# danielzgtg/TTS.cpp

Hardware: AMD Instinct MI355X
Metric: audio-sec/wall-sec (RTF^-1), Parler-TTS-mini v1 Q4_K AR decode + DAC decode (higher is better)
Workload: dtype q4_K weights x q8_K activations (int dot, f32 combine); DAC f16 im2col x f32 weights, f64 accumulate

## Files before the change

include/tts_hip.h:

```cpp
#ifndef TTS_HIP_H
#define TTS_HIP_H

#include <stddef.h>
#include <stdint.h>

#ifdef __cplusplus
extern "C" {
#endif

#define TTS_MAX_DIMS 4
#define TTS_MAX_SRC 4
#define TTS_MAX_OP_PARAMS 16
#define TTS_MAX_NAME 64

enum tts_type {
    TTS_TYPE_F32 = 0,
    TTS_TYPE_F16 = 1,
    TTS_TYPE_Q4_0 = 2,
    TTS_TYPE_Q4_1 = 3,
    TTS_TYPE_Q5_0 = 6,
    TTS_TYPE_Q5_1 = 7,
    TTS_TYPE_Q8_0 = 8,
    TTS_TYPE_Q8_1 = 9,
    TTS_TYPE_Q4_K = 12,
// ... 49 lines not shown
    TTS_OP_COUNT
};

enum tts_custom_op {
    TTS_CUSTOM_NONE = 0,
    TTS_CUSTOM_UV_NOISE = 1,
    TTS_CUSTOM_CFG_SCALE = 2
};

enum tts_unary_op {
    TTS_UNARY_ABS = 0,
    TTS_UNARY_NEG,
    TTS_UNARY_TANH,
    TTS_UNARY_RELU,
    TTS_UNARY_SIGMOID,
    TTS_UNARY_GELU,
    TTS_UNARY_SILU,
    TTS_UNARY_EXP,
    TTS_UNARY_COUNT
};

enum tts_status {
    TTS_STATUS_SUCCESS = 0,
    TTS_STATUS_FAILED = -1,
    TTS_STATUS_ALLOC_FAILED = -2,
    TTS_STATUS_UNSUPPORTED = -3,
    TTS_STATUS_BAD_ARG = -4,
    TTS_STATUS_NO_DEVICE = -5
};

#define TTS_PROF_ATTN 39

#define TTS_FLAG_INPUT 1
#define TTS_FLAG_HOSTDATA 2
#define TTS_FLAG_OUTPUT 4
#define TTS_FLAG_PERSIST 8
#define TTS_FLAG_REPACKED 16
#define TTS_FLAG_TILED_COPY 64
#define TTS_FLAG_TILED 32

typedef struct tts_tensor {
    int32_t type;
    int32_t op;
    int64_t ne[TTS_MAX_DIMS];
    size_t nb[TTS_MAX_DIMS];
    int32_t op_params[TTS_MAX_OP_PARAMS];
    struct tts_tensor * src[TTS_MAX_SRC];
    struct tts_tensor * view_src;
    size_t view_offs;
    void * data;
    int32_t flags;
    int32_t pad_;
    char name[TTS_MAX_NAME];
} tts_tensor;

size_t tts_type_size(int type);
int64_t tts_blck_size(int type);
size_t tts_row_size(int type, int64_t ne0);
const char * tts_type_name(int type);
const char * tts_op_name(int op);

typedef struct tts_hip_backend * tts_hip_backend_t;

int tts_hip_device_count(void);
int tts_hip_device_memory(int device, size_t * free_bytes, size_t * total_bytes);
void * tts_hip_event_new(int device);
void tts_hip_event_free(void * event);
int tts_hip_event_record(tts_hip_backend_t backend, void * event);
int tts_hip_event_wait(tts_hip_backend_t backend, void * event);
int tts_hip_event_synchronize(void * event);
int tts_hip_is_device_pointer(const void * p);
tts_hip_backend_t tts_hip_backend_init(int device);
void tts_hip_backend_free(tts_hip_backend_t backend);
const char * tts_hip_backend_name(tts_hip_backend_t backend);

void * tts_hip_buffer_alloc(tts_hip_backend_t backend, size_t size);
void tts_hip_buffer_free(tts_hip_backend_t backend, void * ptr);
size_t tts_hip_buffer_alignment(void);

int tts_hip_tensor_set(tts_hip_backend_t backend, void * dst_dev, const void * src_host, size_t size);
int tts_hip_tensor_get(tts_hip_backend_t backend, void * dst_host, const void * src_dev, size_t size);
int tts_hip_tensor_copy(tts_hip_backend_t backend, void * dst_dev, const void * src_dev, size_t size);
int tts_hip_copy_stream(tts_hip_backend_t backend, void * dst_dev, const void * src_dev, size_t size);
int tts_hip_plan_stats(tts_tensor * const * nodes, int n_nodes, int mask, int32_t * counts);
int tts_hip_tensor_set_async(tts_hip_backend_t backend, void * dst_dev, const void * src_host, size_t size);
int tts_hip_memset(tts_hip_backend_t backend, void * dst_dev, int value, size_t size);
int tts_hip_synchronize(tts_hip_backend_t backend);

int tts_hip_weight_set(tts_hip_backend_t backend, tts_tensor * t, const void * src_host);
int tts_hip_weight_get(tts_hip_backend_t backend, const tts_tensor * t, void * dst_host);
int tts_hip_quantize(tts_hip_backend_t backend, int type, const float * x_dev, void * dst_dev, int64_t rows, int64_t K);
void tts_repack_q4_K(const void * src, void * dst, int64_t nblocks, int inverse);
void tts_repack_q4_K_tiled(const void * src, void * dst, int64_t nrows, int64_t nb, int inverse);

int tts_hip_supports_op(const tts_tensor * node);
int tts_hip_graph_compute(tts_hip_backend_t backend, tts_tensor * const * nodes, int n_nodes);
int tts_hip_graph_prepare(tts_hip_backend_t backend, tts_tensor * const * nodes, int n_nodes, int slot);
int tts_hip_graph_launch(tts_hip_backend_t backend, int slot);

enum tts_hip_option {
    TTS_HIP_OPT_FUSION = 0,
    TTS_HIP_OPT_PROFILE_GEMV = 1,
    TTS_HIP_OPT_GRAPHS = 2,
    TTS_HIP_OPT_CONV_F32ACC = 3,
    TTS_HIP_OPT_CONVT_LDS = 4,
    TTS_HIP_OPT_ATTN_SPLIT = 5,
    TTS_HIP_OPT_KV_PREFETCH = 6,
    TTS_HIP_OPT_KV_PREFETCH_BLOCKS = 7,
    TTS_HIP_OPT_Q4K_TILE_BYTES = 8,
    TTS_HIP_OPT_GEMV_DEBUG = 10,
    TTS_HIP_OPT_CONV_SPLIT = 12,
    TTS_HIP_OPT_GEMV_UNIQUE = 11,
    TTS_HIP_OPT_GEMV_KS = 13,
    TTS_HIP_OPT_ATTN_FUSED = 14,
    TTS_HIP_OPT_GEMM_Q8 = 18,
    TTS_HIP_OPT_BGEMM_F32 = 19,
    TTS_HIP_OPT_CU_PARTITION = 20,
    TTS_HIP_OPT_Q4K_DUAL_BYTES = 16,
    TTS_HIP_OPT_GEMV_RSPLIT = 17,
    TTS_HIP_OPT_ATTN_PV16 = 15,
    TTS_HIP_OPT_GEMV_PREQUANT = 21,
    TTS_HIP_OPT_GEMV_KRELAY = 22,
    TTS_HIP_OPT_ATTN_KS = 23,
    TTS_HIP_OPT_ATTN_PV8 = 24,
    TTS_HIP_OPT_GEMV_KRELAY_LOOP = 26,
    TTS_HIP_OPT_GEMV_Q80_PRO = 27,
    TTS_HIP_OPT_GEMV_Q80_SLAB = 28,
    TTS_HIP_OPT_GEMV_Q80_RW = 29,
    TTS_HIP_OPT_GEMM_Q8_STAGED = 30,
    TTS_HIP_OPT_GEMV_KR_INKERNEL = 31,
    TTS_HIP_OPT_GEMV_F32_WIDE = 32,
    TTS_HIP_OPT_ATTN_PV_MP = 33,
    TTS_HIP_OPT_GEMM_KR_INKERNEL = 35,
    TTS_HIP_OPT_GEMM_KR_CT2 = 36,
    TTS_HIP_OPT_GEMM_KR_NW = 34,
    TTS_HIP_OPT_GEMV_NW_MIN = 25,
    TTS_HIP_OPT_GEMM_KR_XCD = 38,
    TTS_HIP_OPT_GEMM_KR_CP = 39,
    TTS_HIP_OPT_GEMM_KR_WALK = 40,
    TTS_HIP_OPT_GEMM_PF = 41,
    TTS_HIP_OPT_GEMM_PF_NW = 42,
    TTS_HIP_OPT_ATTN_ONE = 43,
    TTS_HIP_OPT_GEMV_KR_TAIL = 44,
    TTS_HIP_OPT_GEMV_Q50_SLAB = 45,
    TTS_HIP_OPT_GEMV_Q50_RW = 46,
    TTS_HIP_OPT_GEMM_Q5 = 47,
    TTS_HIP_OPT_GEMM_Q5_STAGED = 48,
    TTS_HIP_OPT_GEMV_Q40_SLAB = 49,
    TTS_HIP_OPT_GEMV_Q40_RW = 50,
    TTS_HIP_OPT_GEMM_Q4_0 = 51,
    TTS_HIP_OPT_GEMM_Q4_0_STAGED = 52,
    TTS_HIP_OPT_CONV_VFMA = 53,
    TTS_HIP_OPT_CONV_TILE96 = 54,
    TTS_HIP_OPT_COALESCE = 37,
};
enum tts_fuse_bits {
    TTS_FUSE_LN = 1, TTS_FUSE_GROUP = 2, TTS_FUSE_KV = 4, TTS_FUSE_EPI = 8, TTS_FUSE_HEADS = 16, TTS_FUSE_ATTN = 32,
    TTS_FUSE_LSTM = 64,
    TTS_FUSE_SNAKE = 128,
    TTS_FUSE_EMBED = 256,
    TTS_FUSE_CONV = 512,
    TTS_FUSE_ADAIN = 1024,
    TTS_FUSE_XATTN = 2048,
    TTS_FUSE_MCPY = 4096,
    TTS_FUSE_CONTREAD = 8192
};
int tts_hip_set_option(tts_hip_backend_t backend, int option, int value);
int tts_hip_attn_decode(tts_hip_backend_t backend, const tts_tensor * q, const tts_tensor * k, const tts_tensor * v,
                        const float * mask, int64_t mbs, float scale, float * out, float * out2, const int64_t * koff,
                        const int64_t * voff, const int64_t * moff, const int32_t * pseq);
int tts_hip_coalesce_stats(int device, int64_t * out, int n);
void tts_hip_coalesce_set_wait(int us);
int tts_hip_coalesce_enable(int on);
#define TTS_HIP_HOOK_FAULT_WEIGHT_SET 1
int tts_hip_test_hook(int hook, int value);
int tts_hip_install_crash_handler(void);
int tts_hip_gemv_stats(tts_hip_backend_t backend, int type, double * ms, int64_t * launches, double * bytes, int reset);
int tts_hip_greedy_step(tts_hip_backend_t backend, const float * logits, int32_t B, int32_t NH, int32_t V, int32_t step,
                        int32_t bos, int32_t eos, int32_t * eos_seen, int32_t * hist, int32_t * next);
typedef struct tts_sampling {
    float temperature;
    float top_p;
    float repetition_penalty;
    int32_t top_k;
    int32_t do_sample;
    int32_t pad_;
    uint64_t seed;
} tts_sampling;
void tts_sampling_default(tts_sampling * cfg);
uint32_t tts_sampler_call_seed(uint64_t seed, int32_t stream, int64_t call);
int tts_sampler_sample(const tts_sampling * cfg, const float * logits, int32_t NH, int32_t V, uint32_t call_seed, int32_t * last,
                       int32_t * count, int32_t * out);
int tts_hip_sample_step(tts_hip_backend_t backend, const float * logits, int32_t B, int32_t NH, int32_t V, const tts_sampling * cfg,
                        int64_t call, int32_t * rep_state, int32_t step, int32_t bos, int32_t eos, int32_t * eos_seen, int32_t * hist,
                        int32_t * next);
int tts_sampling_device_ok(const tts_sampling * cfg, int32_t V);
int tts_hip_counters(tts_hip_backend_t backend, int64_t * out, int n);

int tts_hip_gemv(tts_hip_backend_t backend, int type, const void * w, const float * x, float * y,
                 int64_t K, int64_t N, int64_t M);
int tts_hip_gemv_ex(tts_hip_backend_t backend, int type, const void * w, const float * x, float * y,
                    int64_t K, int64_t N, int64_t M, int32_t wflags);
int tts_hip_gemv_res(tts_hip_backend_t backend, int type, const void * w, const float * x, float * y, const float * res,
                     int64_t K, int64_t N, int64_t M, int32_t wflags);

typedef struct tts_backend_iface {
    void * ctx;
    const char * name;
    void * (*alloc)(void * ctx, size_t size);
    void (*free)(void * ctx, void * ptr);
    int (*set)(void * ctx, void * dst, const void * src, size_t size);
    int (*set_tensor)(void * ctx, tts_tensor * t, const void * src);
    int (*get)(void * ctx, void * dst, const void * src, size_t size);
    int (*memset)(void * ctx, void * dst, int value, size_t size);
    int (*compute)(void * ctx, tts_tensor * const * nodes, int n_nodes);
    int (*synchronize)(void * ctx);
    int (*prepare)(void * ctx, tts_tensor * const * nodes, int n_nodes, int slot);
    int (*launch)(void * ctx, int slot);
    int (*set_async)(void * ctx, void * dst, const void * src, size_t size);
    int (*copy)(void * ctx, void * dst, const void * src, size_t size);
    int (*greedy_step)(void * ctx, const float * logits, int B, int NH, int V, int step, int bos, int eos, int32_t * eos_seen,
                       int32_t * hist, int32_t * next);
    int (*sample_step)(void * ctx, const float * logits, int B, int NH, int V, const tts_sampling * cfg, int64_t call, int32_t * rep_state,
                       int step, int bos, int eos, int32_t * eos_seen, int32_t * hist, int32_t * next);
} tts_backend_iface;

int tts_hip_backend_iface(tts_hip_backend_t backend, tts_backend_iface * out);

#ifdef __cplusplus
}
#endif

#endif
```

tts.cpp_amd/csrc/backend.hip:

```cpp
#include <cmath>
#include <atomic>
#include <cstring>
#include <map>
#include <mutex>
#include <thread>

#include "hip_internal.h"
#include <hip/hip_ext.h>

#include <dlfcn.h>
#include <execinfo.h>
#include <fcntl.h>
#include <signal.h>
#include <unistd.h>

using namespace tts;


static void build_gelu_table(uint16_t * t) {
    const float GELU_COEF_A = 0.044715f;
    const float SQRT_2_OVER_PI = 0.79788456080286535587989211986876f;
    for (int i = 0; i < 65536; ++i) {
        const float x = fp16_to_fp32_host((uint16_t)i);
        const float g = 0.5f * x * (1.0f + tanhf(SQRT_2_OVER_PI * x * (1.0f + GELU_COEF_A * x * x)));
        t[i] = fp32_to_fp16_host(g);
    }
}

static const size_t kScratchBytes = 64u << 20;
static const size_t kShadowBytes = 4u << 20;
static const size_t kLstmFloats = 4u << 20;
static const size_t kAttnFloats = 4u << 20;
static const size_t kVecScratchFloats = 1u << 18;
static const size_t kPinBytes = 16u << 20;

namespace {
std::mutex g_reg_mu;
struct BufRec {
    size_t size = 0;
};
std::map<const char *, BufRec> g_buffers;
std::unordered_map<const void *, uint8_t *> g_tiled;
std::atomic<size_t> g_tiled_n{0};
}

namespace tts {
const uint8_t * tiled_copy_find(const void * w) {
    std::lock_guard<std::mutex> lk(g_reg_mu);
    auto it = g_tiled.find(w);
    return it == g_tiled.end() ? nullptr : it->second;
}
static std::atomic<int> g_coalesce_on{[] {
    const char * e = getenv("TTS_HIP_COALESCE");
    return e && e[0] == '0' ? 0 : 1;
}()};
bool coalesce_enabled() { return g_coalesce_on.load(std::memory_order_relaxed) != 0; }
bool buffer_lookup(const void * p, const char ** base, size_t * size) {
    std::lock_guard<std::mutex> lk(g_reg_mu);
    auto it = g_buffers.upper_bound((const char *)p);
    if (it == g_buffers.begin()) return false;
    --it;
    if ((const char *)p >= it->first + it->second.size) return false;
    if (base) *base = it->first;
    if (size) *size = it->second.size;
    return true;
}
}

extern "C" {

int tts_hip_coalesce_enable(int on) { return tts::g_coalesce_on.exchange(on ? 1 : 0); }

int tts_hip_device_count(void) {
    int n = 0;
    if (hipGetDeviceCount(&n) != hipSuccess) return 0;
    return n;
}

tts_hip_backend_t tts_hip_backend_init(int device) {
    int n = tts_hip_device_count();
    if (device < 0 || device >= n) return nullptr;
    if (hipSetDevice(device) != hipSuccess) return nullptr;
    auto * be = new tts_hip_backend();
    be->device = device;
    TTS_HIP_CHECK(hipStreamCreateWithFlags(&be->stream, hipStreamNonBlocking));
    TTS_HIP_CHECK(hipStreamCreateWithFlags(&be->cap_stream, hipStreamNonBlocking));
    TTS_HIP_CHECK(hipStreamCreateWithFlags(&be->pf_stream, hipStreamNonBlocking));
    TTS_HIP_CHECK(hipEventCreateWithFlags(&be->co_ev, hipEventDisableTiming));
    TTS_HIP_CHECK(hipEventCreateWithFlags(&be->pf_fork, hipEventDisableTiming));
    TTS_HIP_CHECK(hipEventCreateWithFlags(&be->pf_join, hipEventDisableTiming));
    hipDeviceProp_t prop;
    TTS_HIP_CHECK(hipGetDeviceProperties(&prop, device));
    snprintf(be->name, sizeof(be->name), "HIP%d(%s)", device, prop.gcnArchName);
    be->cu_total = prop.multiProcessorCount > 0 ? prop.multiProcessorCount : 256;
    be->cus = be->cu_total;
    TTS_HIP_CHECK(hipMalloc((void **)&be->scratch, kScratchBytes));
    be->scratch_size = kScratchBytes;
    TTS_HIP_CHECK(hipMalloc((void **)&be->shadow, kShadowBytes));
    be->shadow_size = kShadowBytes;
    be->hoist_size = (size_t)8 << 20;
    TTS_HIP_CHECK(hipMalloc(&be->hoist, be->hoist_size));
    TTS_HIP_CHECK(hipMalloc((void **)&be->lstm_buf, kLstmFloats * sizeof(float)));
    TTS_HIP_CHECK(hipMalloc((void **)&be->attn_buf, kAttnFloats * sizeof(float)));
    be->attn_floats = kAttnFloats;
    TTS_HIP_CHECK(hipMalloc((void **)&be->vec_scratch, kVecScratchFloats * sizeof(float)));
    be->conv_stage_floats = (size_t)8 << 20;
    TTS_HIP_CHECK(hipMalloc((void **)&be->conv_stage, be->conv_stage_floats * sizeof(float)));
    if (const char * e = getenv("TTS_HIP_OPT_CONV_VFMA"))
        if (e[0] >= '0' && e[0] <= '2' && !e[1]) be->conv_vfma = e[0] - '0';
    be->conv_part_doubles = (size_t)8 << 20;
    TTS_HIP_CHECK(hipMalloc((void **)&be->conv_part, be->conv_part_doubles * sizeof(double)));
    be->lstm_floats = kLstmFloats;
    TTS_HIP_CHECK(hipMalloc((void **)&be->argmax_keys, kArgmaxRows * sizeof(unsigned long long)));
    TTS_HIP_CHECK(hipMalloc((void **)&be->argmax_counts, kArgmaxRows * sizeof(unsigned)));
    TTS_HIP_CHECK(hipMemset(be->argmax_keys, 0, kArgmaxRows * sizeof(unsigned long long)));
    TTS_HIP_CHECK(hipMemset(be->argmax_counts, 0, kArgmaxRows * sizeof(unsigned)));
    TTS_HIP_CHECK(hipHostMalloc((void **)&be->pin, kPinBytes, hipHostMallocDefault));
    be->pin_size = kPinBytes;
    for (auto & e : be->plan_ev) TTS_HIP_CHECK(hipEventCreateWithFlags(&e, hipEventDisableTiming));
    std::vector<uint16_t> tab(65536);
    build_gelu_table(tab.data());
    TTS_HIP_CHECK(hipMalloc((void **)&be->gelu_table, 65536 * sizeof(uint16_t)));
    TTS_HIP_CHECK(hipMemcpy(be->gelu_table, tab.data(), 65536 * sizeof(uint16_t), hipMemcpyHostToDevice));
    return be;
}

void tts_hip_backend_free(tts_hip_backend_t be) {
    if (!be) return;
    tts::coalesce_backend_gone(be);
    hipSetDevice(be->device);
    hipStreamSynchronize(be->stream);
    for (auto & p : be->ev_pending) {
        hipEventDestroy(p.first);
        hipEventDestroy(p.second);
    }
    for (auto e : be->ev_free) hipEventDestroy(e);
    for (auto & r : be->pin_pending) hipEventDestroy(r.ev);
    for (auto e : be->pin_events) hipEventDestroy(e);
    for (auto e : be->plan_ev) hipEventDestroy(e);
    hipHostFree(be->pin);
    if (be->rb_host) hipHostFree(be->rb_host);
    hipFree(be->scratch);
    hipFree(be->shadow);
    hipFree(be->argmax_keys);
    hipFree(be->argmax_counts);
    hipFree(be->lstm_buf);
    hipFree(be->hoist);
    hipFree(be->attn_buf);
    hipFree(be->vec_scratch);
    hipFree(be->conv_stage);
    hipFree(be->conv_part);
    hipFree(be->gelu_table);
    if (be->sample_cand) hipFree(be->sample_cand);
    if (be->repack_tmp) hipFree(be->repack_tmp);
    for (char * r : be->repack_retired) hipFree(r);
    if (be->attn_stage) hipFree(be->attn_stage);
    for (auto & ex : be->gsig_exec)
        if (ex) hipGraphExecDestroy(ex);
    for (auto & ex : be->pexec)
        if (ex) hipGraphExecDestroy(ex);
    hipStreamDestroy(be->stream);
    hipStreamDestroy(be->cap_stream);
    hipStreamDestroy(be->pf_stream);
    hipEventDestroy(be->pf_fork);
    hipEventDestroy(be->pf_join);
    hipEventDestroy(be->co_ev);
    delete be;
}

const char * tts_hip_backend_name(tts_hip_backend_t be) { return be ? be->name : "HIP(null)"; }

int tts_hip_device_memory(int device, size_t * free_bytes, size_t * total_bytes) {
    if (device < 0 || device >= tts_hip_device_count()) return TTS_STATUS_NO_DEVICE;
    int prev = 0;
    hipGetDevice(&prev);
    hipSetDevice(device);
    size_t f = 0, t = 0;
    const hipError_t e = hipMemGetInfo(&f, &t);
    hipSetDevice(prev);
    if (e != hipSuccess) return TTS_STATUS_FAILED;
    if (free_bytes) *free_bytes = f;
    if (total_bytes) *total_bytes = t;
    return 0;
}

void * tts_hip_event_new(int device) {
    if (device < 0 || device >= tts_hip_device_count()) return nullptr;
    hipSetDevice(device);
    hipEvent_t ev = nullptr;
    if (hipEventCreateWithFlags(&ev, hipEventDisableTiming) != hipSuccess) return nullptr;
    return (void *)ev;
}
void tts_hip_event_free(void * event) {
    if (event) hipEventDestroy((hipEvent_t)event);
}
int tts_hip_event_record(tts_hip_backend_t be, void * event) {
    if (!be || !event) return TTS_STATUS_BAD_ARG;
    hipSetDevice(be->device);
    return hipEventRecord((hipEvent_t)event, be->stream) == hipSuccess ? 0 : TTS_STATUS_FAILED;
}
int tts_hip_event_wait(tts_hip_backend_t be, void * event) {
    if (!be || !event) return TTS_STATUS_BAD_ARG;
    hipSetDevice(be->device);
    return hipStreamWaitEvent(be->stream, (hipEvent_t)event, 0) == hipSuccess ? 0 : TTS_STATUS_FAILED;
}
int tts_hip_event_synchronize(void * event) {
    if (!event) return TTS_STATUS_BAD_ARG;
    return hipEventSynchronize((hipEvent_t)event) == hipSuccess ? 0 : TTS_STATUS_FAILED;
}
int tts_hip_is_device_pointer(const void * p) {
    if (!p) return 0;
    hipPointerAttribute_t a;
    if (hipPointerGetAttributes(&a, p) != hipSuccess) {
        (void)hipGetLastError();
        return 0;
    }
    return a.type == hipMemoryTypeDevice ? 1 : 0;
}

size_t tts_hip_buffer_alignment(void) { return 256; }

void * tts_hip_buffer_alloc(tts_hip_backend_t be, size_t size) {
    if (!be) return nullptr;
    hipSetDevice(be->device);
    void * p = nullptr;
    BufRec r;
    r.size = size ? size : 256;
    if (hipMalloc(&p, r.size) != hipSuccess) return nullptr;
    std::lock_guard<std::mutex> lk(g_reg_mu);
    g_buffers[(const char *)p] = r;
    return p;
}

static void drop_tiled_copies(const void * p, size_t n) {
    if (g_tiled_n.load(std::memory_order_acquire) == 0) return;
    const char * a = (const char *)p;
    std::vector<uint8_t *> dead;
    {
        std::lock_guard<std::mutex> lk(g_reg_mu);
        for (auto it = g_tiled.begin(); it != g_tiled.end();) {
            const char * k = (const char *)it->first;
            if (k >= a && k < a + n) {
                dead.push_back(it->second);
                it = g_tiled.erase(it);
            } else {
                ++it;
            }
        }
        g_tiled_n.store(g_tiled.size(), std::memory_order_release);
    }
    if (dead.empty()) return;
    hipDeviceSynchronize();
    for (uint8_t * c : dead) hipFree(c);
}

void tts_hip_buffer_free(tts_hip_backend_t be, void * ptr) {
    if (!be || !ptr) return;
    hipSetDevice(be->device);
    hipStreamSynchronize(be->stream);
    BufRec r;
    bool known = false;
    {
        std::lock_guard<std::mutex> lk(g_reg_mu);
        auto b = g_buffers.find((const char *)ptr);
        if (b != g_buffers.end()) {
            r = b->second;
            known = true;
            g_buffers.erase(b);
        }
    }
    if (known) {
        drop_tiled_copies(ptr, r.size);
        tts::coalesce_written(ptr, r.size);
    }
    hipFree(ptr);
}

int tts_hip_tensor_set(tts_hip_backend_t be, void * dst, const void * src, size_t size) {
    if (!be) return TTS_STATUS_BAD_ARG;
    hipSetDevice(be->device);
    be->rb_clear();
    drop_tiled_copies(dst, size);
    tts::coalesce_written(dst, size);
    if (size > 0 && size <= be->pin_size / 4) {
        const int st = tts_hip_tensor_set_async(be, dst, src, size);
        if (st != 0) return st;
    } else if (hipMemcpyAsync(dst, src, size, hipMemcpyHostToDevice, be->stream) != hipSuccess) {
        return TTS_STATUS_FAILED;
    }
    if (hipStreamSynchronize(be->stream) != hipSuccess) return TTS_STATUS_FAILED;
    return 0;
}

int tts_hip_tensor_set_async(tts_hip_backend_t be, void * dst, const void * src, size_t size) {
    if (!be) return TTS_STATUS_BAD_ARG;
    if (size == 0) return 0;
    hipSetDevice(be->device);
    be->rb_clear();
    if (size > be->pin_size / 2) return tts_hip_tensor_set(be, dst, src, size);
    tts::coalesce_written(dst, size);
    std::lock_guard<std::mutex> pl(be->pin_mu);
    while (!be->pin_pending.empty() && hipEventQuery(be->pin_pending.front().ev) == hipSuccess) {
        be->pin_events.push_back(be->pin_pending.front().ev);
        be->pin_pending.pop_front();
    }
    size_t off = (be->pin_head + 255) & ~(size_t)255;
    if (off + size > be->pin_size) off = 0;
    int last = -1;
    for (int i = 0; i < (int)be->pin_pending.size(); ++i) {
        const auto & r = be->pin_pending[i];
        if (r.off < off + size && off < r.off + r.size) last = i;
    }
    if (last >= 0) {
        if (hipEventSynchronize(be->pin_pending[last].ev) != hipSuccess) return TTS_STATUS_FAILED;
        for (int i = 0; i <= last; ++i) {
            be->pin_events.push_back(be->pin_pending.front().ev);
            be->pin_pending.pop_front();
        }
    }
    memcpy(be->pin + off, src, size);
    if (hipMemcpyAsync(dst, be->pin + off, size, hipMemcpyHostToDevice, be->stream) != hipSuccess) return TTS_STATUS_FAILED;
    hipEvent_t ev;
    if (be->pin_events.empty()) {
        if (hipEventCreateWithFlags(&ev, hipEventDisableTiming) != hipSuccess) return TTS_STATUS_FAILED;
    } else {
        ev = be->pin_events.back();
        be->pin_events.pop_back();
    }
    if (hipEventRecord(ev, be->stream) != hipSuccess) return TTS_STATUS_FAILED;
    be->pin_pending.push_back({off, size, ev});
    be->pin_head = off + size;
    return 0;
}

int tts_hip_greedy_step(tts_hip_backend_t be, const float * logits, int32_t B, int32_t NH, int32_t V, int32_t step, int32_t bos,
                        int32_t eos, int32_t * eos_seen, int32_t * hist, int32_t * next) {
    if (!be || !logits || B <= 0 || NH <= 0 || V <= 0) return TTS_STATUS_BAD_ARG;
    hipSetDevice(be->device);
    be->rb_clear();
    launch_greedy_step(be, logits, B, NH, V, step, bos, eos, eos_seen, hist, next);
    return 0;
}

int tts_hip_sample_step(tts_hip_backend_t be, const float * logits, int32_t B, int32_t NH, int32_t V, const tts_sampling * cfg, int64_t call,
                        int32_t * rep_state, int32_t step, int32_t bos, int32_t eos, int32_t * eos_seen, int32_t * hist, int32_t * next) {
    if (!be || !logits || !cfg || B <= 0 || NH <= 0 || V <= 0) return TTS_STATUS_BAD_ARG;
    hipSetDevice(be->device);
    be->rb_clear();
    return launch_sample_step(be, logits, B, NH, V, cfg, call, rep_state, step, bos, eos, eos_seen, hist, next);
}

int tts_hip_tensor_get(tts_hip_backend_t be, void * dst, const void * src, size_t size) {
    if (!be) return TTS_STATUS_BAD_ARG;
    hipSetDevice(be->device);
    if (be->rb_any.load(std::memory_order_acquire)) {
        std::lock_guard<std::mutex> l(be->rb_mu);
        for (const auto & r : be->rb) {
            const char * s = (const char *)src;
            if (s >= r.dev && s + size <= r.dev + r.bytes) {
                if (hipStreamSynchronize(be->stream) != hipSuccess) return TTS_STATUS_FAILED;
                memcpy(dst, be->rb_host + r.off + (s - r.dev), size);
                return 0;
            }
        }
    }
    if (hipMemcpyAsync(dst, src, size, hipMemcpyDeviceToHost, be->stream) != hipSuccess) return TTS_STATUS_FAILED;
    if (hipStreamSynchronize(be->stream) != hipSuccess) return TTS_STATUS_FAILED;
    return 0;
}

int tts_hip_copy_stream(tts_hip_backend_t be, void * dst, const void * src, size_t size) {
    if (!be || !dst || !src || size % 16 || ((uintptr_t)dst | (uintptr_t)src) % 16) return TTS_STATUS_BAD_ARG;
    if (size == 0) return 0;
    hipSetDevice(be->device);
    be->rb_clear();
    tts::launch_copy_stream(be, dst, src, (int64_t)(size / 16));
    return hipGetLastError() == hipSuccess ? 0 : TTS_STATUS_FAILED;
}

int tts_hip_tensor_copy(tts_hip_backend_t be, void * dst, const void * src, size_t size) {
    if (!be) return TTS_STATUS_BAD_ARG;
    hipSetDevice(be->device);
    be->rb_clear();
    tts::coalesce_written(dst, size);
    tts::launch_copy_bytes(be, dst, src, size);
    return hipGetLastError() == hipSuccess ? 0 : TTS_STATUS_FAILED;
}

int tts_hip_memset(tts_hip_backend_t be, void * dst, int value, size_t size) {
    if (!be) return TTS_STATUS_BAD_ARG;
    hipSetDevice(be->device);
    be->rb_clear();
    tts::coalesce_written(dst, size);
    return hipMemsetAsync(dst, value, size, be->stream) == hipSuccess ? 0 : TTS_STATUS_FAILED;
}

int tts_hip_synchronize(tts_hip_backend_t be) {
    if (!be) return TTS_STATUS_BAD_ARG;
    hipSetDevice(be->device);
    return hipStreamSynchronize(be->stream) == hipSuccess ? 0 : TTS_STATUS_FAILED;
}

void tts_repack_q4_K(const void * src, void * dst, int64_t nblocks, int inverse) {
    const uint8_t * s = (const uint8_t *)src;
    uint8_t * d = (uint8_t *)dst;
    for (int64_t b = 0; b < nblocks; ++b) {
        const uint8_t * sb = s + b * 144;
        uint8_t * db = d + b * 144;
        memcpy(db, sb, 16);
        for (int i = 0; i < 128; ++i) {
            const int l = i >> 4, c = (i >> 2) & 3, k = i & 3;
            const int nat = 32 * c + 8 * k + l;
            if (!inverse) db[16 + i] = sb[16 + nat];
            else db[16 + nat] = sb[16 + i];
        }
    }
}

static void repack_tiled_rows(const uint8_t * s, uint8_t * d, int64_t r0, int64_t r1, int64_t nb, int inverse) {
    const int64_t rb = nb * 144;
    for (int64_t row = r0; row < r1; ++row) {
        const int64_t t = row >> 2, i = row & 3;
        for (int64_t b = 0; b < nb; ++b) {
            const int64_t nat = row * rb + b * 144;
            const int64_t til = (t * nb + b) * 576;
            const uint8_t * a = inverse ? s + til : s + nat;
            uint8_t * o = inverse ? d + nat : d + til;
            if (!inverse) memcpy(o + i * 16, a, 16);
            else memcpy(o, a + i * 16, 16);
            for (int c = 0; c < 4; ++c)
                for (int h = 0; h < 2; ++h)
                    for (int lp = 0; lp < 4; ++lp)
                        for (int kk = 0; kk < 4; ++kk) {
                            const int64_t tpos = 64 + ((c * 2 + h) * 4 + i) * 16 + lp * 4 + kk;
                            const int64_t npos = 16 + 32 * c + 8 * kk + 4 * h + lp;
                            if (!inverse) o[tpos] = a[npos];
                            else o[npos] = a[tpos];
                        }
        }
    }
}

void tts_repack_q4_K_tiled(const void * src, void * dst, int64_t nrows, int64_t nb, int inverse) {
    const uint8_t * s = (const uint8_t *)src;
    uint8_t * d = (uint8_t *)dst;
    unsigned nt = std::thread::hardware_concurrency();
    nt = nt < 1 ? 1 : nt > 16 ? 16 : nt;
    if (nrows * nb < 4096 || nt == 1) {
        repack_tiled_rows(s, d, 0, nrows, nb, inverse);
        return;
    }
    std::vector<std::thread> th;
    const int64_t chunk = ((nrows + nt - 1) / nt + 3) & ~(int64_t)3;
    for (int64_t r0 = 0; r0 < nrows; r0 += chunk)
        th.emplace_back(repack_tiled_rows, s, d, r0, r0 + chunk < nrows ? r0 + chunk : nrows, nb, inverse);
    for (auto & t : th) t.join();
}

static size_t tensor_bytes(const tts_tensor * t) {
    size_t n = tts_row_size(t->type, t->ne[0]);
    for (int i = 1; i < 4; ++i) n *= (size_t)t->ne[i];
    return n;
}

static int weight_set_impl(tts_hip_backend_t be, tts_tensor * t, const void * src);
static std::atomic<bool> g_fault_weight_set{false};

static struct sigaction g_prev_segv, g_prev_bus;
static void crash_write(const char * s, int n) {
    while (n > 0) {
        const ssize_t w = write(2, s, (size_t)n);
        if (w <= 0) return;
        s += w, n -= (int)w;
    }
}
static char g_crash_maps[1 << 20];
static int crash_hex(char * o, unsigned long v) {
    char t[16];
    int n = 0;
    do t[n++] = "0123456789abcdef"[v & 15], v >>= 4; while (v);
    o[0] = '0', o[1] = 'x';
    for (int i = 0; i < n; ++i) o[2 + i] = t[n - 1 - i];
    return n + 2;
}
static int crash_dec(char * o, int v) {
    char t[12];
    int n = 0;
    do t[n++] = (char)('0' + v % 10), v /= 10; while (v);
    for (int i = 0; i < n; ++i) o[i] = t[n - 1 - i];
    return n;
}
static const char * crash_parse_hex(const char * p, unsigned long * v) {
    unsigned long x = 0;
    for (;; ++p) {
        const char c = *p;
        const int d = c >= '0' && c <= '9' ? c - '0' : c >= 'a' && c <= 'f' ? c - 'a' + 10 : -1;
        if (d < 0) break;
        x = x * 16 + (unsigned long)d;
    }
    *v = x;
    return p;
}
static bool crash_map_line(const char * l, const char * e, unsigned long * a, unsigned long * b, unsigned long * off, const char ** path, int * plen) {
    const char * p = crash_parse_hex(l, a);
    if (*p != '-') return false;
    p = crash_parse_hex(p + 1, b);
    while (p < e && *p == ' ') ++p;
    while (p < e && *p != ' ') ++p;
    while (p < e && *p == ' ') ++p;
    p = crash_parse_hex(p, off);
    for (int f = 0; f < 2; ++f) {
        while (p < e && *p == ' ') ++p;
        while (p < e && *p != ' ') ++p;
    }
    while (p < e && *p == ' ') ++p;
    *path = p, *plen = (int)(e - p);
    return true;
}
static void crash_handler(int sig, siginfo_t * si, void * uc) {
    char buf[640];
    int n = 0;
    const char h1[] = "tts_hip: signal ";
    for (const char * c = h1; *c; ++c) buf[n++] = *c;
    n += crash_dec(buf + n, sig);
    const char h2[] = ", fault address ";
    for (const char * c = h2; *c; ++c) buf[n++] = *c;
    const uintptr_t fa = si ? (uintptr_t)si->si_addr : 0;
    n += crash_hex(buf + n, fa);
    buf[n++] = '\n';
    crash_write(buf, n);
    int mlen = 0;
    {
        const int fd = open("/proc/self/maps", O_RDONLY);
        if (fd >= 0) {
            ssize_t r;
            while (mlen < (int)sizeof g_crash_maps - 1 && (r = read(fd, g_crash_maps + mlen, sizeof g_crash_maps - 1 - mlen)) > 0) mlen += (int)r;
            close(fd);
        }
    }
    void * fr[64];
    const int nf = backtrace(fr, 64);
    for (int i = 0; i < nf; ++i) {
        n = 0;
        buf[n++] = ' ', buf[n++] = ' ', buf[n++] = '#';
        n += crash_dec(buf + n, i);
        buf[n++] = ' ';
        n += crash_hex(buf + n, (unsigned long)(uintptr_t)fr[i]);
// ... 28 lines not shown
        if (crash_map_line(g_crash_maps + l0, g_crash_maps + l1, &a, &b, &off, &path, &plen) && fa + (64ul << 20) >= a && fa <= b + (64ul << 20))
            crash_write(g_crash_maps + l0, l1 - l0 + (l1 < mlen ? 1 : 0));
        l0 = l1 + 1;
    }
    const struct sigaction & prev = sig == SIGBUS ? g_prev_bus : g_prev_segv;
    if (prev.sa_flags & SA_SIGINFO) {
        if (prev.sa_sigaction) prev.sa_sigaction(sig, si, uc);
    } else if (prev.sa_handler != SIG_DFL && prev.sa_handler != SIG_IGN && prev.sa_handler) {
        prev.sa_handler(sig);
    }
    signal(sig, SIG_DFL);
    raise(sig);
}

int tts_hip_install_crash_handler(void) {
    void * warm[2];
    (void)backtrace(warm, 2);
    struct sigaction sa;
    memset(&sa, 0, sizeof sa);
    sa.sa_sigaction = crash_handler;
    sa.sa_flags = SA_SIGINFO | SA_RESETHAND;
    sigemptyset(&sa.sa_mask);
    if (sigaction(SIGSEGV, &sa, &g_prev_segv) != 0 || sigaction(SIGBUS, &sa, &g_prev_bus) != 0) return TTS_STATUS_FAILED;
    return 0;
}

int tts_hip_test_hook(int hook, int value) {
    if (hook == TTS_HIP_HOOK_FAULT_WEIGHT_SET) {
        g_fault_weight_set.store(value != 0);
        return 0;
    }
    return TTS_STATUS_BAD_ARG;
}

int tts_hip_weight_set(tts_hip_backend_t be, tts_tensor * t, const void * src) {
    if (!be || !t) return TTS_STATUS_BAD_ARG;
    if (t->type == TTS_TYPE_Q4_K && g_fault_weight_set.load(std::memory_order_relaxed)) return TTS_STATUS_ALLOC_FAILED;
    return weight_set_impl(be, t, src);
}

static int weight_set_impl(tts_hip_backend_t be, tts_tensor * t, const void * src) {
    const size_t n = tensor_bytes(t);
    if (t->type == TTS_TYPE_Q4_K && t->ne[0] % 256 == 0 && t->ne[1] % 4 == 0 && t->ne[2] == 1 && t->ne[3] == 1 &&
        be->q4k_tile_bytes > 0 && (int64_t)n >= be->q4k_tile_bytes) {
        std::vector<uint8_t> tmp(n);
        tts_repack_q4_K_tiled(src, tmp.data(), t->ne[1], t->ne[0] / 256, 0);
        int st = tts_hip_tensor_set(be, t->data, tmp.data(), n);
        if (st == 0) t->flags |= TTS_FLAG_REPACKED | TTS_FLAG_TILED;
        return st;
    }
    if (t->type == TTS_TYPE_Q4_K && t->ne[0] % 256 == 0) {
        std::vector<uint8_t> tmp(n);
        tts_repack_q4_K(src, tmp.data(), (int64_t)(n / 144), 0);
        t->flags &= ~TTS_FLAG_TILED_COPY;
        int st = tts_hip_tensor_set(be, t->data, tmp.data(), n);
        if (st == 0) t->flags |= TTS_FLAG_REPACKED;
        if (st == 0 && be->q4k_dual_bytes > 0 && (int64_t)n >= be->q4k_dual_bytes && t->ne[0] >= 2048 && t->ne[1] % 16 == 0 &&
            t->ne[2] == 1 && t->ne[3] == 1) {
            tts_repack_q4_K_tiled(src, tmp.data(), t->ne[1], t->ne[0] / 256, 0);
            uint8_t * cp = nullptr;
            if (hipMalloc((void **)&cp, n) != hipSuccess) return TTS_STATUS_ALLOC_FAILED;
            if (hipMemcpy(cp, tmp.data(), n, hipMemcpyHostToDevice) != hipSuccess) {
                hipFree(cp);
                return TTS_STATUS_FAILED;
            }
            {
                std::lock_guard<std::mutex> lk(g_reg_mu);
                g_tiled[t->data] = cp;
                g_tiled_n.store(g_tiled.size(), std::memory_order_release);
            }
            t->flags |= TTS_FLAG_TILED_COPY;
        }
        return st;
    }
    return tts_hip_tensor_set(be, t->data, src, n);
}

int tts_hip_weight_get(tts_hip_backend_t be, const tts_tensor * t, void * dst) {
    if (!be || !t) return TTS_STATUS_BAD_ARG;
    const size_t n = tensor_bytes(t);
    if (t->type == TTS_TYPE_Q4_K && (t->flags & TTS_FLAG_TILED)) {
        std::vector<uint8_t> tmp(n);
        int st = tts_hip_tensor_get(be, tmp.data(), t->data, n);
        if (st == 0) tts_repack_q4_K_tiled(tmp.data(), dst, t->ne[1], t->ne[0] / 256, 1);
        return st;
    }
    if (t->type == TTS_TYPE_Q4_K && (t->flags & TTS_FLAG_REPACKED)) {
        std::vector<uint8_t> tmp(n);
        int st = tts_hip_tensor_get(be, tmp.data(), t->data, n);
        if (st == 0) tts_repack_q4_K(tmp.data(), dst, (int64_t)(n / 144), 1);
        return st;
    }
    return tts_hip_tensor_get(be, dst, t->data, n);
}

static bool is_f32(const tts_tensor * t) { return t && t->type == TTS_TYPE_F32; }

int tts_hip_supports_op(const tts_tensor * n) {
    if (!n) return 0;
    for (int i = 0; i < TTS_MAX_SRC; ++i)
        if (n->src[i] && (n->src[i]->flags & 2)) return 0;
    switch (n->op) {
        case TTS_OP_NONE: case TTS_OP_VIEW: case TTS_OP_RESHAPE: case TTS_OP_PERMUTE: case TTS_OP_TRANSPOSE:
            return 1;
        case TTS_OP_DUP: case TTS_OP_CONT: case TTS_OP_CPY:
            return (n->type == TTS_TYPE_F32 || n->type == TTS_TYPE_F16 || n->type == TTS_TYPE_I32) &&
                   (n->src[0]->type == TTS_TYPE_F32 || n->src[0]->type == TTS_TYPE_F16 || n->src[0]->type == TTS_TYPE_I32);
        case TTS_OP_ADD: case TTS_OP_SUB: case TTS_OP_MUL: case TTS_OP_DIV:
        case TTS_OP_SQR: case TTS_OP_SQRT: case TTS_OP_SIN: case TTS_OP_COS: case TTS_OP_SCALE: case TTS_OP_CLAMP:
        case TTS_OP_LEAKY_RELU: case TTS_OP_ROUND: case TTS_OP_MOD: case TTS_OP_UNARY: case TTS_OP_CONCAT:
        case TTS_OP_REPEAT: case TTS_OP_SUM_ROWS:
            return 1;
        case TTS_OP_NORM: case TTS_OP_RMS_NORM:
            return is_f32(n->src[0]) && n->src[0]->nb[0] == 4;
        case TTS_OP_SOFT_MAX:
            return is_f32(n->src[0]);
        case TTS_OP_ROPE:
            return is_f32(n->src[0]);
        case TTS_OP_IM2COL:
            return is_f32(n->src[1]) && n->op_params[6] == 0 && (n->type == TTS_TYPE_F16 || n->type == TTS_TYPE_F32);
        case TTS_OP_CONV_TRANSPOSE_1D:
            return is_f32(n->src[0]) && is_f32(n->src[1]) && n->op_params[4] >= 1;
        case TTS_OP_CUMSUM: case TTS_OP_UPSCALE: case TTS_OP_STFT: case TTS_OP_ISTFT: case TTS_OP_MAP_CUSTOM3: case TTS_OP_MAP_CUSTOM2:
            return tts::audio_op_supported(n);
        case TTS_OP_GET_ROWS:
            return n->src[1]->type == TTS_TYPE_I32 &&
                   (n->src[0]->type == TTS_TYPE_F32 || n->src[0]->type == TTS_TYPE_F16 || n->src[0]->type == TTS_TYPE_Q4_K ||
                    n->src[0]->type == TTS_TYPE_Q8_0 || n->src[0]->type == TTS_TYPE_Q5_0 || n->src[0]->type == TTS_TYPE_Q4_0);
        case TTS_OP_MUL_MAT: {
            const tts_tensor * a = n->src[0];
            const tts_tensor * b = n->src[1];
            if (!is_f32(b)) return 0;
            if (a->ne[0] != b->ne[0] || b->ne[2] % a->ne[2] || b->ne[3] % a->ne[3]) return 0;
            if (a->type == TTS_TYPE_F32 || a->type == TTS_TYPE_F16) return 1;
            if (a->type == TTS_TYPE_Q4_K) return a->ne[0] % 256 == 0;
            if (a->type == TTS_TYPE_Q8_0 || a->type == TTS_TYPE_Q5_0 || a->type == TTS_TYPE_Q4_0) return a->ne[0] % 32 == 0;
            return 0;
        }
        default:
            return 0;
    }
}

}

extern "C" int tts_hip_set_option(tts_hip_backend_t be, int option, int value) {
    if (!be) return TTS_STATUS_BAD_ARG;
    switch (option) {
        case TTS_HIP_OPT_FUSION: be->fusion = value; return 0;
        case TTS_HIP_OPT_CONVT_LDS: be->convt_lds = value != 0; return 0;
        case TTS_HIP_OPT_CONV_SPLIT: be->conv_split = value < 0 ? 1 : value; return 0;
        case TTS_HIP_OPT_CONV_VFMA: be->conv_vfma = value < 0 || value > 2 ? 1 : value; return 0;
        case TTS_HIP_OPT_CONV_TILE96: be->conv_tile96 = value != 0; return 0;
        case TTS_HIP_OPT_PROFILE_GEMV: be->profile_gemv = value != 0; return 0;
        case TTS_HIP_OPT_GRAPHS: be->use_graphs = value != 0; return 0;
        case TTS_HIP_OPT_CONV_F32ACC:
            be->conv_f32acc = value == 1;
            be->conv_acc_mode = value == 2 ? 2 : 0;
            return 0;
        case TTS_HIP_OPT_ATTN_SPLIT: be->attn_split_minp = value; return 0;
        case TTS_HIP_OPT_ATTN_FUSED: be->attn_fused_minp = value; return 0;
        case TTS_HIP_OPT_ATTN_PV16: be->attn_pv_uv16 = value != 0; return 0;
        case TTS_HIP_OPT_KV_PREFETCH: be->kv_prefetch_minp = value; return 0;
        case TTS_HIP_OPT_Q4K_TILE_BYTES: be->q4k_tile_bytes = value; return 0;
        case TTS_HIP_OPT_Q4K_DUAL_BYTES: be->q4k_dual_bytes = value; return 0;
        case TTS_HIP_OPT_GEMV_RSPLIT: be->gemv_mf_rsplit = value != 0; return 0;
        case TTS_HIP_OPT_GEMV_PREQUANT: be->gemv_mf_prequant = value != 0; return 0;
        case TTS_HIP_OPT_GEMV_KRELAY: be->gemv_kr = value != 0; return 0;
        case TTS_HIP_OPT_GEMV_KRELAY_LOOP: be->gemv_kr_loop = value != 0; return 0;
        case TTS_HIP_OPT_GEMV_Q80_PRO: be->gemv_q80_pro = value != 0; return 0;
        case TTS_HIP_OPT_GEMV_Q80_SLAB: be->gemv_q80_slab = value != 0; return 0;
        case TTS_HIP_OPT_GEMV_KR_INKERNEL:
            if (value < 0) return TTS_STATUS_BAD_ARG;
            be->gemv_kr_ink = value;
            return 0;
        case TTS_HIP_OPT_GEMM_Q8_STAGED:
            if (value < 0 || value > 2) return TTS_STATUS_BAD_ARG;
            be->gemm_q8_staged = value;
            return 0;
        case TTS_HIP_OPT_GEMV_Q80_RW:
            if (value < 0 || value > 32 || (value & (value - 1))) return TTS_STATUS_BAD_ARG;
            be->gemv_q80_rw = value;
            return 0;
        case TTS_HIP_OPT_GEMV_Q50_SLAB: be->gemv_q50_slab = value != 0; return 0;
        case TTS_HIP_OPT_GEMV_Q50_RW:
            if (value < 0 || value > 32 || (value & (value - 1))) return TTS_STATUS_BAD_ARG;
            be->gemv_q50_rw = value;
            return 0;
        case TTS_HIP_OPT_GEMM_Q5: be->gemm_q5 = value != 0; return 0;
        case TTS_HIP_OPT_GEMM_Q5_STAGED:
            if (value < 0 || value > 2) return TTS_STATUS_BAD_ARG;
            be->gemm_q5_staged = value;
            return 0;
        case TTS_HIP_OPT_GEMV_Q40_SLAB: be->gemv_q40_slab = value != 0; return 0;
        case TTS_HIP_OPT_GEMV_Q40_RW:
            if (value < 0 || value > 32 || (value & (value - 1))) return TTS_STATUS_BAD_ARG;
            be->gemv_q40_rw = value;
            return 0;
        case TTS_HIP_OPT_GEMM_Q4_0: be->gemm_q4_0 = value != 0; return 0;
        case TTS_HIP_OPT_GEMM_Q4_0_STAGED:
            if (value < 0 || value > 2) return TTS_STATUS_BAD_ARG;
            be->gemm_q4_0_staged = value;
            return 0;
        case TTS_HIP_OPT_ATTN_KS: be->attn_ks = value; return 0;
        case TTS_HIP_OPT_GEMV_NW_MIN: be->gemv_nw_min = value; return 0;
        case TTS_HIP_OPT_ATTN_PV8: be->attn_pv8 = value != 0; return 0;
        case TTS_HIP_OPT_GEMM_KR_CT2: be->gemm_kr_ct2 = value != 0; return 0;
        case TTS_HIP_OPT_GEMM_KR_INKERNEL: be->gemm_kr_ink = value < 0 ? 0 : value; return 0;
        case TTS_HIP_OPT_ATTN_PV_MP: be->attn_pv_mp = value == 2 ? 2 : value != 0; return 0;
        case TTS_HIP_OPT_ATTN_ONE:
            if (value < 0 || value > 2) return TTS_STATUS_BAD_ARG;
            be->attn_one = value;
            return 0;
        case TTS_HIP_OPT_GEMV_KR_TAIL:
            if (value < 0 || value > 4) return TTS_STATUS_BAD_ARG;
            be->gemv_kr_tail = value;
            return 0;
        case TTS_HIP_OPT_GEMM_KR_NW: be->gemm_kr_nw = value == 8 ? 8 : 4; return 0;
        case TTS_HIP_OPT_GEMM_Q8: be->gemm_q8 = value != 0; return 0;
        case TTS_HIP_OPT_CU_PARTITION: {
            const int count = value & 0xFF, index = (value >> 8) & 0xFF;
            const bool inter = (value >> 16) & 1;
            hipSetDevice(be->device);
            TTS_HIP_CHECK(hipStreamSynchronize(be->stream));
            hipStream_t ns = nullptr;
            if (count <= 1) {
                TTS_HIP_CHECK(hipStreamCreateWithFlags(&ns, hipStreamNonBlocking));
                be->cus = be->cu_total;
            } else {
                if (index >= count) return TTS_STATUS_BAD_ARG;
                std::vector<uint32_t> mask((be->cu_total + 31) / 32, 0u);
                const int per = be->cu_total / count;
                int n = 0;
                for (int c = 0; c < be->cu_total; ++c) {
                    const bool on = inter ? (c % count == index) : (c / per == index && c < per * count);
                    if (on) mask[c / 32] |= 1u << (c % 32), ++n;
                }
                if (hipExtStreamCreateWithCUMask(&ns, (uint32_t)mask.size(), mask.data()) != hipSuccess) return TTS_STATUS_FAILED;
                be->cus = n;
            }
            TTS_HIP_CHECK(hipStreamDestroy(be->stream));
            be->stream = ns;
            for (auto & ex : be->gsig_exec)
                if (ex) hipGraphExecDestroy(ex), ex = nullptr;
            for (auto & g : be->gsig) g = 0;
            return 0;
        }
        case TTS_HIP_OPT_BGEMM_F32: be->bgemm_f32 = value != 0; return 0;
        case TTS_HIP_OPT_GEMV_F32_WIDE: be->gemv_f32_wide = value != 0; return 0;
        case TTS_HIP_OPT_GEMV_DEBUG: be->gemv_dbg = value; return 0;
        case TTS_HIP_OPT_GEMV_UNIQUE: be->gemv_unique = value != 0; return 0;
        case TTS_HIP_OPT_GEMV_KS: be->gemv_ks_tiles = value > 0 ? value : 0; return 0;
        case TTS_HIP_OPT_COALESCE: be->co_member = value != 0; return 0;
        case TTS_HIP_OPT_GEMM_KR_XCD: be->gemm_kr_xcd = value != 0; return 0;
        case TTS_HIP_OPT_GEMM_KR_CP: be->gemm_kr_cp = value != 0; return 0;
        case TTS_HIP_OPT_GEMM_KR_WALK: be->gemm_kr_walk = value < 0 ? 0 : value; return 0;
        case TTS_HIP_OPT_GEMM_PF: be->gemm_pf = value < 0 ? 0 : value; return 0;
        case TTS_HIP_OPT_GEMM_PF_NW: be->gemm_pf_nw = value == 8 ? 8 : 4; return 0;
        case TTS_HIP_OPT_KV_PREFETCH_BLOCKS: be->kv_prefetch_blocks = value > 0 ? value : 1; return 0;
        default: return TTS_STATUS_BAD_ARG;
    }
}

extern "C" int tts_hip_counters(tts_hip_backend_t be, int64_t * out, int n) {
    if (!be || !out) return TTS_STATUS_BAD_ARG;
    const int64_t v[8] = {be->graph_updates, be->graph_instantiations, be->lstm_chains, be->lstm_steps, be->plan_wait_ns,
                          be->cap_plan_ns, be->cap_launch_ns, be->cap_update_ns};
    int k = 0;
    for (; k < n && k < 8; ++k) out[k] = v[k];
    return k;
}

extern "C" int tts_hip_gemv_stats(tts_hip_backend_t be, int type, double * ms, int64_t * launches, double * bytes, int reset) {
    if (!be) return TTS_STATUS_BAD_ARG;
    hipSetDevice(be->device);
    TTS_HIP_CHECK(hipStreamSynchronize(be->stream));
    for (size_t i = 0; i < be->ev_pending.size(); ++i) {
        float t = 0;
        TTS_HIP_CHECK(hipEventElapsedTime(&t, be->ev_pending[i].first, be->ev_pending[i].second));
        const int ty = be->ev_type[i];
        be->gemv_ms[ty] += t;
        be->gemv_launches[ty] += 1;
        be->gemv_bytes[ty] += be->ev_bytes[i];
        be->ev_free.push_back(be->ev_pending[i].first);
        be->ev_free.push_back(be->ev_pending[i].second);
    }
    be->ev_pending.clear();
    be->ev_bytes.clear();
    be->ev_type.clear();
    double a = 0, c = 0;
    int64_t b = 0;
    for (int ty = 0; ty < TTS_TYPE_COUNT; ++ty) {
        if (type >= 0 && ty != type) continue;
        a += be->gemv_ms[ty];
        b += be->gemv_launches[ty];
        c += be->gemv_bytes[ty];
    }
    if (ms) *ms = a;
    if (launches) *launches = b;
    if (bytes) *bytes = c;
    if (reset) {
        for (int ty = 0; ty < TTS_TYPE_COUNT; ++ty) {
            be->gemv_ms[ty] = 0;
            be->gemv_launches[ty] = 0;
            be->gemv_bytes[ty] = 0;
        }
    }
    return 0;
}

static void * hb_alloc(void * c, size_t n) { return tts_hip_buffer_alloc((tts_hip_backend_t)c, n); }
static void hb_free(void * c, void * p) { tts_hip_buffer_free((tts_hip_backend_t)c, p); }
static int hb_set(void * c, void * d, const void * s, size_t n) { return tts_hip_tensor_set((tts_hip_backend_t)c, d, s, n); }
static int hb_set_tensor(void * c, tts_tensor * t, const void * s) { return tts_hip_weight_set((tts_hip_backend_t)c, t, s); }
static int hb_get(void * c, void * d, const void * s, size_t n) { return tts_hip_tensor_get((tts_hip_backend_t)c, d, s, n); }
static int hb_memset(void * c, void * d, int v, size_t n) { return tts_hip_memset((tts_hip_backend_t)c, d, v, n); }
static int hb_compute(void * c, tts_tensor * const * nodes, int n) { return tts_hip_graph_compute((tts_hip_backend_t)c, nodes, n); }
static int hb_sync(void * c) { return tts_hip_synchronize((tts_hip_backend_t)c); }
static int hb_prepare(void * c, tts_tensor * const * nodes, int n, int slot) {
    return tts_hip_graph_prepare((tts_hip_backend_t)c, nodes, n, slot);
}
static int hb_launch(void * c, int slot) { return tts_hip_graph_launch((tts_hip_backend_t)c, slot); }
static int hb_set_async(void * c, void * d, const void * s, size_t n) { return tts_hip_tensor_set_async((tts_hip_backend_t)c, d, s, n); }
static int hb_copy(void * c, void * d, const void * s, size_t n) { return tts_hip_tensor_copy((tts_hip_backend_t)c, d, s, n); }
static int hb_greedy(void * c, const float * l, int B, int NH, int V, int step, int bos, int eos, int32_t * seen, int32_t * hist, int32_t * next) {
    return tts_hip_greedy_step((tts_hip_backend_t)c, l, B, NH, V, step, bos, eos, seen, hist, next);
}
static int hb_sample(void * c, const float * l, int B, int NH, int V, const tts_sampling * cfg, int64_t call, int32_t * rep, int step, int bos,
                     int eos, int32_t * seen, int32_t * hist, int32_t * next) {
    return tts_hip_sample_step((tts_hip_backend_t)c, l, B, NH, V, cfg, call, rep, step, bos, eos, seen, hist, next);
}

extern "C" int tts_hip_backend_iface(tts_hip_backend_t be, tts_backend_iface * out) {
    if (!be || !out) return TTS_STATUS_BAD_ARG;
    out->ctx = be;
    out->name = be->name;
    out->alloc = hb_alloc;
    out->free = hb_free;
    out->set = hb_set;
    out->set_tensor = hb_set_tensor;
    out->get = hb_get;
    out->memset = hb_memset;
    out->compute = hb_compute;
    out->synchronize = hb_sync;
    out->prepare = hb_prepare;
    out->launch = hb_launch;
    out->set_async = hb_set_async;
    out->copy = hb_copy;
    out->greedy_step = hb_greedy;
    out->sample_step = hb_sample;
    return 0;
}
```

tts.cpp_amd/csrc/graph_exec.hip:

```cpp
#include <algorithm>
#include <cstring>
#include <deque>
#include <unordered_map>
#include <vector>

#include <array>

#include "hip_internal.h"
#include <chrono>

using namespace tts;

namespace tts {
void launch_kv_prefetch(tts_hip_backend * be, hipStream_t st, const TD & t, int pdim, int blocks);
void launch_gemv_q4K_xattn(tts_hip_backend * be, const GemvJob & j, const XAttnArgs & a);
void launch_attn_decode(tts_hip_backend * be, const TD & q, const TD & k, const TD & v, const float * mask, float scale,
                        float * out, int hd, int P, int H, int n, int B, float * out2, int64_t obs = -1, int64_t mbs = 0,
                        const int64_t * koff = nullptr, const int64_t * voff = nullptr, const int64_t * moff = nullptr,
                        const int * pseq = nullptr);
void launch_attn_bias(tts_hip_backend * be, const TD & q, const TD & k, const TD & v, const float * bias, const float * mask,
                      float scale, float * out, int P, int H, int n);
void launch_layernorm(tts_hip_backend * be, const tts_tensor * dst, const tts_tensor * x, const float * w, const float * b,
                      float eps, bool rms);
}
// ... 1156 lines not shown
                m->ne[1] * m->ne[2] * m->ne[3] == 1 && !overlap(A, m) && !(overlap(A, x0) && A->data != x0->data)) {
                it.x = x0;
                it.snake_mask = m;
                act[index[x]] = -1;
            }
        }
        act[index[M1]] = act[index[S]] = act[index[Q]] = act[index[M2]] = -1;
        if (rfuse) {
            it.b = nullptr;
            it.snake_one = O;
            act[index[R]] = -1;
        }
        act[i] = add_item(std::move(it));
    }

    static bool vec_c(const tts_tensor * t, int64_t C) {
        if (!t || t->type != TTS_TYPE_F32 || t->ne[2] * t->ne[3] != 1 || t->nb[0] != 4) return false;
        return (t->ne[0] == C && t->ne[1] == 1) || (t->ne[0] == 1 && t->ne[1] == C && t->nb[1] == 4);
    }
    static bool same_shape(const tts_tensor * a, int64_t n0, int64_t n1) {
        return a->type == TTS_TYPE_F32 && a->ne[0] == n0 && a->ne[1] == n1 && a->ne[2] * a->ne[3] == 1;
    }
    static bool plan_debug() {
        static const bool dbg = getenv("TTS_PLAN_DEBUG") != nullptr;
        return dbg;
    }
    static void plan_reject(const char * what, int code) {
        if (plan_debug()) fprintf(stderr, "plan: %s not fused (check %d)\n", what, code);
    }
    static bool adain_fail(int code) {
        plan_reject("adain", code);
        return false;
    }
    bool try_adain(int i) {
        const tts_tensor * N = nodes[i];
        const tts_tensor * X = N->src[0];
        if (!X || X->type != TTS_TYPE_F32 || N->type != TTS_TYPE_F32 || X->nb[0] != 4 || N->ne[2] * N->ne[3] != 1) return adain_fail(1);
        const int64_t T = N->ne[0], C = N->ne[1];
        if (!adain_supported(T)) return adain_fail(2);
        const tts_tensor * T1 = sole_consumer(N);
        if (!T1 || T1->op != TTS_OP_TRANSPOSE) return adain_fail(3);
        const tts_tensor * C1 = sole_consumer(T1);
        if (!C1 || C1->op != TTS_OP_CONT || !same_shape(C1, C, T) || uses[C1] != 2) return adain_fail(4);
        const auto & cc = consumers[C1];
        if (cc.size() != 2) return adain_fail(5);
        const tts_tensor *M = nodes[cc[0]], *A1 = nodes[cc[1]];
        if (M->op != TTS_OP_MUL || M->src[0] != C1 || !vec_c(M->src[1], C) || sole_consumer(M) != A1) return adain_fail(6);
        if (A1->op != TTS_OP_ADD || A1->src[0] != C1 || A1->src[1] != M || !same_shape(A1, C, T)) return adain_fail(7);
        const tts_tensor * A2 = sole_consumer(A1);
        if (!A2 || A2->op != TTS_OP_ADD || A2->src[0] != A1 || !vec_c(A2->src[1], C) || !same_shape(A2, C, T)) return adain_fail(8);
        const tts_tensor * T2 = sole_consumer(A2);
        if (!T2 || T2->op != TTS_OP_TRANSPOSE) return adain_fail(9);
        const tts_tensor * C2 = sole_consumer(T2);
        if (!C2 || C2->op != TTS_OP_CONT || !same_shape(C2, T, C) || !contiguous(C2)) return adain_fail(10);
        const tts_tensor *gamma = M->src[1], *beta = A2->src[1];
        std::vector<int> absorbed = {i, index[C1], index[M], index[A1], index[A2], index[C2]};
        auto affine_src = [&](const tts_tensor * v, const tts_tensor * user, const tts_tensor *& W, const tts_tensor *& B,
                              const tts_tensor *& st) {
            if (!v || v->op != TTS_OP_ADD || sole_consumer(v) != user) return false;
            const tts_tensor * mm = v->src[0];
            if (!mm || mm->op != TTS_OP_MUL_MAT || sole_consumer(mm) != v || !vec_c(v->src[1], C) || v->src[1]->ne[0] != C) return false;
            W = mm->src[0], st = mm->src[1], B = v->src[1];
            const int64_t S = W->ne[0];
            return W->type == TTS_TYPE_F32 && contiguous(W) && W->ne[1] == C && W->ne[2] * W->ne[3] == 1 && S % 4 == 0 &&
                   ((uintptr_t)W->data % 16) == 0 && st->type == TTS_TYPE_F32 && contiguous(st) && st->ne[0] == S &&
                   st->ne[1] * st->ne[2] * st->ne[3] == 1 && ((uintptr_t)st->data % 16) == 0;
        };
        const tts_tensor *gW = nullptr, *gB = nullptr, *gS = nullptr, *bW = nullptr, *bB = nullptr, *bS = nullptr;
        const bool inline_gb = affine_src(gamma, M, gW, gB, gS) && affine_src(beta, A2, bW, bB, bS) && gS == bS;
        if (inline_gb) {
            for (const tts_tensor * t : {gamma, (const tts_tensor *)gamma->src[0], beta, (const tts_tensor *)beta->src[0]}) absorbed.push_back(index[t]);
            gamma = beta = nullptr;
        }
        const tts_tensor * out = C2;
        const tts_tensor *alpha = nullptr, *recip = nullptr, *one = nullptr;
        if ((mask & TTS_FUSE_SNAKE) && uses[C2] == 2) {
            const auto & sc = consumers[C2];
            const tts_tensor *M1 = nodes[sc[0]], *SA = nodes[sc[1]];
            const tts_tensor *S = sole_consumer(M1), *Q = S ? sole_consumer(S) : nullptr, *M2 = Q ? sole_consumer(Q) : nullptr;
            const tts_tensor * R = M2 ? M2->src[1] : nullptr;
            const tts_tensor * O = R ? R->src[0] : nullptr;
            const bool r_inline = R && R->op == TTS_OP_DIV && O && R->src[1] == M1->src[1] && sole_consumer(R) == M2 &&
                                  O->type == TTS_TYPE_F32 && O->nb[1] == 0 && O->ne[0] == 1 && O->ne[2] * O->ne[3] == 1 &&
                                  same_shape(R, 1, C);
            if (M1->op == TTS_OP_MUL && M1->src[0] == C2 && S && S->op == TTS_OP_SIN && Q && Q->op == TTS_OP_SQR && M2 &&
                M2->op == TTS_OP_MUL && M2->src[0] == Q && sole_consumer(M2) == SA && SA->op == TTS_OP_ADD && SA->src[0] == C2 &&
                SA->src[1] == M2 && vec_c(M1->src[1], C) && vec_c(M2->src[1], C) && same_shape(SA, T, C) && contiguous(SA) &&
                same_shape(M1, T, C) && same_shape(S, T, C) && same_shape(Q, T, C) && same_shape(M2, T, C)) {
                alpha = M1->src[1];
                recip = M2->src[1];
                out = SA;
                for (const tts_tensor * t : {M1, S, Q, M2, SA}) absorbed.push_back(index[t]);
                if (r_inline) {
                    absorbed.push_back(index[R]);
                    recip = nullptr;
                    one = O;
                }
            }
        }
        const bool in_place = out->data == X->data && out->nb[1] == X->nb[1];
        if (overlap(out, X) && !in_place) return adain_fail(11);
        bool stage = false;
        for (const tts_tensor * t : {gamma, beta, alpha, recip, one})
            if (t && overlap(out, t)) stage = true;
        if (inline_gb)
            for (const tts_tensor * t : {gW, gB, bW, bB, gS})
                if (overlap(out, t)) return adain_fail(14);
        if (stage && 4 * C + 1 > (int64_t)vec_cap) return adain_fail(12);
        const int last = *std::max_element(absorbed.begin(), absorbed.end());
        std::vector<bool> is_abs(n, false);
        for (int k : absorbed) is_abs[k] = true;
        for (int k = i + 1; k < last; ++k) {
            if (is_abs[k] || is_view(nodes[k]->op)) continue;
            const tts_tensor * w = nodes[k];
            for (const tts_tensor * t : {X, gamma, beta, alpha, recip, one, gW, gB, bW, bB, gS})
                if (t && t != w && overlap(w, t)) {
                    if (plan_debug()) fprintf(stderr, "plan: adain node %d (%s) between %d..%d overlaps an input\n", k, tts_op_name(w->op), i, last);
                    return adain_fail(13);
                }
        }
        AdainArgs a;
        a.x = (const float *)X->data;
        a.xcs = (int64_t)(X->nb[1] / 4);
        a.y = (float *)out->data;
        a.ycs = (int64_t)(out->nb[1] / 4);
        auto vstride = [](const tts_tensor * t) { return t->ne[0] == 1 ? (int64_t)(t->nb[1] / 4) : (int64_t)1; };
        if (inline_gb) {
            a.gw = (const float *)gW->data, a.gb = (const float *)gB->data;
            a.bw = (const float *)bW->data, a.bb = (const float *)bB->data;
            a.style = (const float *)gS->data, a.S = gW->ne[0];
        } else {
            a.gamma = (const float *)gamma->data, a.gcs = vstride(gamma);
            a.beta = (const float *)beta->data, a.bcs = vstride(beta);
        }
        if (alpha) {
            a.alpha = (const float *)alpha->data, a.acs = vstride(alpha);
            if (recip) a.recip = (const float *)recip->data, a.rcs = vstride(recip);
            else a.one = (const float *)one->data;
        }
        a.T = T, a.C = C;
        a.stage = stage;
        memcpy(&a.eps, &N->op_params[0], 4);
        Item it;
        it.kind = Item::ADAIN;
        it.adain = a;
        it.dst = out;
        for (int k : absorbed)
            if (k != last) act[k] = -1;
        act[last] = add_item(std::move(it));
        return true;
    }

    static const tts_tensor * through_view(const tts_tensor * t) { return t && t->op == TTS_OP_RESHAPE ? t->src[0] : t; }
    void try_conv(int i) {
        const tts_tensor * col = nodes[i];
        const tts_tensor *kern = col->src[0], *x = col->src[1];
        if (col->type != TTS_TYPE_F16 || col->op_params[6] != 0 || col->ne[2] * col->ne[3] != 1) return plan_reject("conv", 1);
        if (!x || x->type != TTS_TYPE_F32 || x->ne[2] * x->ne[3] != 1) return plan_reject("conv", 2);
        if (!kern || (kern->type != TTS_TYPE_F32 && kern->type != TTS_TYPE_F16) || kern->ne[3] != 1) return plan_reject("conv", 3);
        const tts_tensor * cv = sole_consumer(col);
        if (!cv || cv->op != TTS_OP_RESHAPE || !contiguous(col)) return plan_reject("conv", 4);
        const tts_tensor * mm = sole_consumer(cv);
        if (!mm || mm->op != TTS_OP_MUL_MAT || mm->src[0] != cv || mm->type != TTS_TYPE_F32) return plan_reject("conv", 5);
        const tts_tensor * wv = mm->src[1];
        if (!wv || through_view(wv) != kern) return plan_reject("conv", 6);
        const int K = (int)kern->ne[0];
        const int64_t IC = kern->ne[1], OC = kern->ne[2], L = x->ne[0], OL = col->ne[1];
        if (x->ne[1] != IC || mm->ne[0] != OL || mm->ne[1] != OC || !contiguous(mm)) return plan_reject("conv", 7);
        const int s = col->op_params[0], p = col->op_params[2], d = col->op_params[4];
        if (!conv1d_fused_ok(IC, K, s, d, nullptr)) return plan_reject("conv", 8);
        if (kern->nb[0] != tts_type_size(kern->type)) return plan_reject("conv", 9);
        const tts_tensor * out = mm;
        std::vector<int> absorbed = {i, (int)index[mm]};
        const tts_tensor * r3 = sole_consumer(mm);
        const tts_tensor * cur = mm;
        if (r3 && r3->op == TTS_OP_RESHAPE && r3->ne[0] == OL && r3->ne[1] == OC) cur = r3;
        Conv1dArgs a;
        const tts_tensor * bias = nullptr;
        const tts_tensor * res = nullptr;
        const tts_tensor * nb = sole_consumer(cur);
        if (nb && nb->op == TTS_OP_ADD && nb->src[0] == cur && nb->type == TTS_TYPE_F32 && contiguous(nb) && nb->ne[0] == OL &&
            nb->ne[1] == OC && nb->ne[2] * nb->ne[3] == 1 && chan_vec(nb->src[1], OC) && nb->src[1]->ne[1] == OC) {
            bias = nb->src[1];
            out = nb;
            absorbed.push_back(index[nb]);
            const tts_tensor * nr = sole_consumer(nb);
            if (nr && nr->op == TTS_OP_ADD && nr->type == TTS_TYPE_F32 && contiguous(nr) && nr->ne[0] == OL && nr->ne[1] == OC &&
                nr->ne[2] * nr->ne[3] == 1) {
                const tts_tensor * other = nr->src[0] == nb ? nr->src[1] : nr->src[0];
                if (other && other != nb && other->type == TTS_TYPE_F32 && contiguous(other) && other->ne[0] == OL && other->ne[1] == OC &&
                    other->ne[2] * other->ne[3] == 1 && (!overlap(nr, other) || nr->data == other->data)) {
                    res = other;
                    out = nr;
                    absorbed.push_back(index[nr]);
                }
            }
        }
        float * stage = nullptr;
        for (;;) {
            if (overlap(out, kern) || (bias && overlap(out, bias))) return plan_reject("conv", 10);
            stage = nullptr;
            bool ok = true;
            bool in_col = false;
            if (overlap(out, x)) {
                const size_t need = (size_t)OL * (size_t)OC * 4;
                if (tbytes(col) >= need && !overlap(col, x) && !overlap(col, out) && !(res && overlap(col, res)) && !overlap(col, kern) &&
                    !(bias && overlap(col, bias))) {
                    stage = (float *)col->data;
                    in_col = true;
                } else if (conv_stage && need <= 4 * conv_stage_cap) {
                    stage = conv_stage;
                } else {
                    ok = false;
                }
            }
            for (int j = i + 1; ok && j < absorbed.back(); ++j) {
                if (std::find(absorbed.begin(), absorbed.end(), j) != absorbed.end() || is_view(nodes[j]->op)) continue;
                if (overlap(nodes[j], x) || (in_col && overlap(nodes[j], col))) ok = false;
            }
            if (ok) break;
            if (!res) return plan_reject("conv", 11);
            res = nullptr;
            absorbed.pop_back();
            out = bias ? nb : mm;
        }
        a.x = make_td(x);
        a.w = kern->data;
        a.w16 = kern->type == TTS_TYPE_F16;
        const size_t es = tts_type_size(kern->type);
        a.wk = (int64_t)(kern->nb[0] / es), a.wic = (int64_t)(kern->nb[1] / es), a.woc = (int64_t)(kern->nb[2] / es);
        a.y = (float *)out->data;
        a.ycs = (int64_t)(out->nb[1] / 4);
        if (stage) {
            a.copy_dst = a.y;
            a.y = stage;
            a.ycs = OL;
        }
        if (bias) a.bias = (const float *)bias->data, a.bcs = bias->ne[1] == 1 ? 0 : (int64_t)(bias->nb[1] / 4);
        if (res) a.res = (const float *)res->data, a.rcs = (int64_t)(res->nb[1] / 4);
        a.L = L, a.IC = IC, a.OL = OL, a.OC = OC;
        a.K = K, a.s = s, a.p = p, a.d = d;
        const size_t xb = (size_t)((x->ne[0] - 1) * x->nb[0] + (x->ne[1] - 1) * x->nb[1]) + 4;
        const size_t wb = tbytes(kern);
        if (xb >= 0x80000000u || wb >= 0x80000000u) return plan_reject("conv", 12);
        a.x_bytes = (uint32_t)xb, a.w_bytes = (uint32_t)wb;
        Item it;
        it.kind = Item::CONV;
        it.conv = a;
        it.dst = out;
        for (size_t k = 0; k + 1 < absorbed.size(); ++k) act[absorbed[k]] = -1;
        act[absorbed.back()] = add_item(std::move(it));
    }

    bool embed_terms(const tts_tensor * a, const tts_tensor * root, std::vector<const tts_tensor *> & terms, std::vector<int> & members) {
        if (a->op != TTS_OP_ADD || a->type != TTS_TYPE_F32) return false;
        for (int d = 0; d < 4; ++d)
            if (a->ne[d] != root->ne[d]) return false;
        const tts_tensor *l = a->src[0], *r = a->src[1];
        if (!l || !r) return false;
        const bool la = l->op == TTS_OP_ADD, ra = r->op == TTS_OP_ADD;
        if (la && ra) return false;
        auto leaf_ok = [&](const tts_tensor * g) {
            if (g->op != TTS_OP_GET_ROWS || sole_consumer(g) != a || g->type != TTS_TYPE_F32) return false;
            const tts_tensor *tab = g->src[0], *idx = g->src[1];
            if (tab->type != TTS_TYPE_F32 && tab->type != TTS_TYPE_F16 && tab->type != TTS_TYPE_Q8_0 && tab->type != TTS_TYPE_Q5_0 && tab->type != TTS_TYPE_Q4_0 && tab->type != TTS_TYPE_Q4_K) return false;
            if (idx->type != TTS_TYPE_I32 || idx->ne[1] * idx->ne[2] * idx->ne[3] != 1 || (idx->nb[0] % 4)) return false;
            if (tab->ne[0] != root->ne[0] || g->ne[0] != root->ne[0] || tab->ne[2] * tab->ne[3] != 1) return false;
            const int64_t rows = g->ne[1] * g->ne[2] * g->ne[3], M = root->ne[1] * root->ne[2] * root->ne[3];
            return idx->ne[0] == rows && (rows == 1 || rows == M);
        };
        if (la || ra) {
            const tts_tensor * inner = la ? l : r;
            const tts_tensor * leaf = la ? r : l;
            if (sole_consumer(inner) != a || !leaf_ok(leaf)) return false;
            if (!embed_terms(inner, root, terms, members)) return false;
            terms.push_back(leaf);
            members.push_back(index[leaf]);
            members.push_back(index[inner]);
            return true;
        }
        if (!leaf_ok(l) || !leaf_ok(r)) return false;
        terms.push_back(l);
        terms.push_back(r);
        members.push_back(index[l]);
        members.push_back(index[r]);
        return true;
    }
    void try_rint(int i) {
        const tts_tensor * R = nodes[i];
        if (R->type != TTS_TYPE_F32 || R->op_params[0] != 1 || !contiguous(R)) return;
        std::vector<const tts_tensor *> leaves;
        std::vector<int> members{i};
        const tts_tensor * t = R;
        while (t->op == TTS_OP_CONCAT && t->op_params[0] == 1) {
            leaves.push_back(t->src[1]);
            t = t->src[0];
            if (t->op == TTS_OP_CONCAT) {
                if (uses[t] != 1 || !index.count(t)) return;
                members.push_back(index[t]);
            }
        }
        leaves.push_back(t);
        std::reverse(leaves.begin(), leaves.end());
        const tts_tensor * a = nullptr;
        int64_t r = 0;
        for (size_t k = 0; k < leaves.size(); ++k) {
            const tts_tensor * rp = leaves[k];
            if (rp->op != TTS_OP_REPEAT || uses[rp] != 1 || !index.count(rp)) return;
            const tts_tensor * c = rp->src[0];
            if (!c || c->op != TTS_OP_CONT || uses[c] != 1 || !index.count(c)) return;
            const tts_tensor * v = c->src[0];
            if (!v || v->op != TTS_OP_VIEW || !v->view_src || v->ne[1] != 1) return;
            const tts_tensor * base = v->view_src;
            if (k == 0) {
                a = base;
                r = rp->ne[1];
                if (a->type != TTS_TYPE_F32 || (int64_t)leaves.size() != a->ne[1]) return;
            }
            if (base != a || rp->ne[1] != r || (const char *)v->data != (const char *)a->data + k * a->nb[1]) return;
            for (int d = 0; d < 4; ++d)
                if (d != 1 && (v->ne[d] != a->ne[d] || v->nb[d] != a->nb[d] || rp->ne[d] != a->ne[d])) return;
            members.push_back(index[rp]);
            members.push_back(index[c]);
        }
        if (!a || R->ne[1] != a->ne[1] * r || overlap(R, a)) return;
        for (int m : members)
            if (act[m] != 0) return;
        const int first = *std::min_element(members.begin(), members.end());
        for (int j = first + 1; j < i; ++j) {
            if (is_view(nodes[j]->op) || std::find(members.begin(), members.end(), j) != members.end()) continue;
            if (overlap(nodes[j], a)) return;
        }
        Item it;
        it.kind = Item::RINT;
        it.x = a;
        it.dst = R;
        it.rint = (int)r;
        for (int m : members) act[m] = -1;
        if (a->op == TTS_OP_CONT && a->src[0] && index.count(a) && act[index[a]] == 0) {
            const tts_tensor * s0 = a->src[0];
            bool ok = s0->type == TTS_TYPE_F32 && !overlap(R, s0);
            for (int d = 0; d < 4; ++d) ok &= s0->ne[d] == a->ne[d];
            auto ca = consumers.find(a);
            ok &= ca != consumers.end();
            if (ok)
                for (int k : ca->second) {
                    const tts_tensor * v = nodes[k];
                    const tts_tensor * u = sole_consumer(v);
                    ok &= v->op == TTS_OP_VIEW && u && std::find(members.begin(), members.end(), index[u]) != members.end();
                }
            const int ia = ok ? index[a] : 0;
            for (int j = ia + 1; ok && j < i; ++j) {
                if (is_view(nodes[j]->op) || std::find(members.begin(), members.end(), j) != members.end()) continue;
                if (overlap(nodes[j], s0)) ok = false;
            }
            if (ok) {
                it.x = s0;
                act[ia] = -1;
            }
        }
        rint_to_cpy(i, R, it);
        act[i] = add_item(std::move(it));
    }

    void rint_to_cpy(int i, const tts_tensor * R, Item & it) {
        const tts_tensor * X = sole_consumer(R);
        std::vector<int> skip;
        while (X && X->op == TTS_OP_RESHAPE && X->src[0] && contiguous(X)) X = sole_consumer(X);
        if (X && X->op == TTS_OP_CONT && contiguous(X) && index.count(X) && act[index[X]] == 0) {
            skip.push_back(index[X]);
            X = sole_consumer(X);
        }
        if (!X || X->op != TTS_OP_CPY || !index.count(X) || act[index[X]] != 0) return;
        const int iP = index[X];
        skip.push_back(iP);
        const tts_tensor * D = X;
        if (D->type != TTS_TYPE_F32 || D->nb[0] != 4 || D->ne[0] != R->ne[0] * R->ne[1] * R->ne[2] || D->ne[1] != R->ne[3] ||
            D->ne[2] != 1 || D->ne[3] != 1 || overlap(D, it.x))
            return;
        for (int j = i + 1; j < iP; ++j)
            if (!is_view(nodes[j]->op) && std::find(skip.begin(), skip.end(), j) == skip.end()) return;
        tts_tensor t = *R;
        t.data = D->data;
        t.nb[0] = 4;
        t.nb[1] = 4 * R->ne[0];
        t.nb[2] = t.nb[1] * R->ne[1];
        t.nb[3] = D->nb[1];
        it.node = t;
        it.rint_cpy = true;
        for (int k : skip) act[k] = -1;
    }

    void try_gather_t(int i) {
        const tts_tensor * C2 = nodes[i];
        const tts_tensor * Tv = C2->src[0];
        if (!Tv || Tv->op != TTS_OP_TRANSPOSE || C2->type != TTS_TYPE_F32 || !contiguous(C2) || uses[Tv] != 1) return;
        const tts_tensor * G = Tv->view_src ? Tv->view_src : Tv->src[0];
        if (!G || G->op != TTS_OP_GET_ROWS || !index.count(G) || act[index[G]] != 0 || uses[G] != 1 || G->type != TTS_TYPE_F32 ||
// ... 925 lines not shown
                    if (!mk || !mv || mk->ne[0] != it.k->ne[0] || mk->ne[2] != it.k->ne[2] || mk->ne[3] != 1 || mv->ne[1] != it.v->ne[1] ||
                        mv->ne[2] != it.v->ne[2] || mv->ne[3] != 1 || mv->ne[0] != mk->ne[1] || mk->nb[1] != it.k->nb[1] ||
                        mk->nb[2] != it.k->nb[2] || mv->nb[1] != it.v->nb[1] || mv->nb[2] != it.v->nb[2] || mk->nb[0] != it.k->nb[0] ||
                        mv->nb[0] != it.v->nb[0])
                        CO_NO();
                    pseq = (int *)&tab[of[3]];
                    pseq[k] = (int)mk->ne[1];
                    pmax = std::max(pmax, (int)mk->ne[1]);
                    ragged |= mk->ne[1] != it.k->ne[1];
                    if (it.mask) {
                        const tts_tensor * mm = cm.member(bc, it.mask, k);
                        if (!mm || mm->ne[0] != mk->ne[1] || mm->ne[1] < it.q->ne[1]) CO_NO();
                    }
                }
                tb.pmax = pmax;
                bc.ragged |= ragged;
                for (int w = 0; w < 2; ++w) {
                    const tts_tensor * kv = w ? it.v : it.k;
                    if (inter(kv)) {
                        if (ragged) CO_NO();
                        continue;
                    }
                    if (bc.stride(kv->data)) CO_NO();
                    of[1 + w] = alloc(N);
                    if (!offsets(kv, of[1 + w], 16)) CO_NO();
                    for (int k = 0; k < N; ++k) tab[of[1 + w] + k] *= 16;
                }
                if (it.mask) {
                    if (inter(it.mask)) {
                        if (ragged) CO_NO();
                    } else {
                        of[4] = alloc(N);
                        if (!offsets(it.mask, of[4], 4)) CO_NO();
                    }
                }
                break;
            }
            case Item::LN:
                if (it.dst->ne[3] != 1 || it.x->ne[3] != 1 || !inter(it.dst) || !inter(it.x) || !equal_all(it.dst) || !equal_all(it.x)) CO_NO();
                if (!share(it.w) || !share(it.b)) CO_NO();
                break;
            case Item::EMBED:
                if (it.gather_t || it.dst->ne[1] * it.dst->ne[2] * it.dst->ne[3] != 1 || !inter(it.dst) || !equal_all(it.dst)) CO_NO();
                if (it.terms.size() > (size_t)EMBED_MAX_TERMS) CO_NO();
                for (size_t t = 0; t < it.terms.size(); ++t) {
                    const tts_tensor * g = it.terms[t];
                    if (g->ne[1] * g->ne[2] * g->ne[3] != 1 || !equal_all(g) || !share(g->src[0])) CO_NO();
                    const tts_tensor * idx = g->src[1];
                    if (inter(idx)) continue;
                    if (!input_mem(idx) || !equal_all(idx)) CO_NO();
                    ioffs[a - 1][t] = alloc(N);
                    if (!offsets(idx, ioffs[a - 1][t], 4)) CO_NO();
                }
                break;
            case Item::NODE: {
                auto * e = cm.pos.find(nd);
                if (!e) CO_NO();
                cm.pos[&it.node] = e->second;
                if (!equal_all(nd)) CO_NO();
                for (int s2 = 0; s2 < TTS_MAX_SRC; ++s2) {
                    const tts_tensor * x = it.node.src[s2];
                    if (!x) continue;
                    if (!cm.pos.find(x) && owned_mem(x)) CO_NO();
                    if (cm.pos.find(x) && !equal_all(x)) CO_NO();
                }
                if (co_per_slice(bc, &it.node))
                    for (int s2 = 0; s2 < TTS_MAX_SRC; ++s2)
                        if (it.node.src[s2] && owned_mem(it.node.src[s2]) && !share(it.node.src[s2])) CO_NO();
                break;
            }
            default: CO_NO();
        }
    }
    *n_scatter = 0;
    std::vector<const tts_tensor *> outs;
    for (int i = 0; i < n_nodes; ++i)
        if ((nodes[i]->flags & TTS_FLAG_OUTPUT) || i == n_nodes - 1) outs.push_back(nodes[i]);
    std::vector<std::array<int64_t, 3>> sc;
    for (const tts_tensor * o : outs) {
        if (owned_mem(o) || is_view(o->op)) continue;
        if (!inter(o) || !contiguous(o) || (tbytes(o) & 3) || !equal_all(o)) CO_NO();
        for (int k = 0; k < N; ++k) {
            const tts_tensor * m = cm.member(bc, o, k);
            if (!m || !m->data || !contiguous(m)) CO_NO();
            sc.push_back({(int64_t)(uintptr_t)bc.reloc(o->data, k), (int64_t)(uintptr_t)m->data, (int64_t)tbytes(o)});
        }
    }
    if (!sc.empty()) {
        *scatter = alloc(3 * sc.size());
        for (size_t e = 0; e < sc.size(); ++e)
            for (int c = 0; c < 3; ++c) tab[*scatter + 3 * (int64_t)e + c] = sc[e][c];
        *n_scatter = (int)sc.size();
    }
    for (size_t a = 0; a < pl.items.size(); ++a)
        for (int t = 0; t < EMBED_MAX_TERMS; ++t)
            if (ioffs[a][t] >= 0) bc.tabs[a].ioff[t] = (const int64_t *)(intptr_t)(ioffs[a][t] + 1);
    return true;
}

static void co_readback(tts_hip_backend * be, const std::vector<int64_t> & sc, int n_sc) {
    BatchCtx & bc = *be->bat;
    const int N = bc.N;
    if ((int)bc.mbe.size() != N) return;
    std::vector<size_t> need(N, 0), off(N, 0);
    for (int e = 0; e < n_sc; ++e) need[e % N] += ((size_t)sc[3 * e + 2] + 255) & ~(size_t)255;
    for (int k = 0; k < N; ++k) {
        tts_hip_backend * m = bc.mbe[k];
        m->rb_clear();
        if (need[k] <= m->rb_cap) continue;
        if (m->rb_host) {
            TTS_HIP_CHECK(hipStreamSynchronize(be->stream));
            TTS_HIP_CHECK(hipHostFree(m->rb_host));
            m->rb_host = nullptr;
            m->rb_cap = 0;
        }
        if (hipHostMalloc((void **)&m->rb_host, need[k], hipHostMallocDefault) != hipSuccess) {
            (void)hipGetLastError();
            m->rb_host = nullptr;
            continue;
        }
        m->rb_cap = need[k];
    }
    for (int e = 0; e < n_sc; ++e) {
        const int k = e % N;
        tts_hip_backend * m = bc.mbe[k];
        if (!m->rb_host) continue;
        const size_t bytes = (size_t)sc[3 * e + 2];
        TTS_HIP_CHECK(hipMemcpyAsync(m->rb_host + off[k], (const void *)(uintptr_t)sc[3 * e], bytes, hipMemcpyDeviceToHost, be->stream));
        std::lock_guard<std::mutex> l(m->rb_mu);
        m->rb.push_back({(const char *)(uintptr_t)sc[3 * e + 1], bytes, off[k]});
        m->rb_any.store(true, std::memory_order_release);
        off[k] += (bytes + 255) & ~(size_t)255;
    }
}

__global__ void k_co_scatter(const int64_t * __restrict__ tab, int n) {
    const int e = blockIdx.y;
    if (e >= n) return;
    const uint32_t * src = (const uint32_t *)(uintptr_t)tab[3 * e];
    uint32_t * dst = (uint32_t *)(uintptr_t)tab[3 * e + 1];
    const int64_t w = tab[3 * e + 2] / 4;
    for (int64_t i = (int64_t)blockIdx.x * blockDim.x + threadIdx.x; i < w; i += (int64_t)gridDim.x * blockDim.x) dst[i] = src[i];
}

static bool capture_worthy(tts_hip_backend * be, tts_tensor * const * nodes, int n_nodes) {
    if (!be->use_graphs || be->profile_gemv) return false;
    for (int i = 0; i < n_nodes; ++i) {
        const tts_tensor * t = nodes[i];
        if (t->op == TTS_OP_MUL_MAT && t->src[1] && t->src[1]->ne[1] > 64) return false;
    }
    return true;
}

static int capture_into(tts_hip_backend * be, tts_tensor * const * nodes, int n_nodes, hipGraphExec_t & ex) {
    hipStream_t run = be->stream;
    be->stream = be->cap_stream;
    const auto t0 = std::chrono::steady_clock::now();
    TTS_HIP_CHECK(hipStreamBeginCapture(be->stream, hipStreamCaptureModeThreadLocal));
    const int st = graph_compute_launches(be, nodes, n_nodes);
    hipGraph_t graph = nullptr;
    TTS_HIP_CHECK(hipStreamEndCapture(be->stream, &graph));
    be->stream = run;
    const auto t1 = std::chrono::steady_clock::now();
    be->cap_launch_ns += std::chrono::duration_cast<std::chrono::nanoseconds>(t1 - t0).count();
    if (st != 0) {
        if (graph) hipGraphDestroy(graph);
        return st;
    }
    bool ok = false;
    if (ex) {
        hipGraphNode_t err_node = nullptr;
        hipGraphExecUpdateResult res;
        ok = hipGraphExecUpdate(ex, graph, &err_node, &res) == hipSuccess && res == hipGraphExecUpdateSuccess;
        if (ok) be->graph_updates++;
        else {
            (void)hipGetLastError();
            TTS_HIP_CHECK(hipGraphExecDestroy(ex));
            ex = nullptr;
        }
    }
    if (!ok) {
        TTS_HIP_CHECK(hipGraphInstantiate(&ex, graph, nullptr, nullptr, 0));
        be->graph_instantiations++;
    }
    TTS_HIP_CHECK(hipGraphDestroy(graph));
    be->cap_update_ns += std::chrono::duration_cast<std::chrono::nanoseconds>(std::chrono::steady_clock::now() - t1).count();
    return 0;
}

extern "C" int tts_hip_graph_compute(tts_hip_backend_t be, tts_tensor * const * nodes, int n_nodes) {
    if (!be) return TTS_STATUS_BAD_ARG;
    hipSetDevice(be->device);
    be->rb_clear();
    const int cs = coalesce_submit(be, nodes, n_nodes);
    if (cs != kCoalesceNotTaken) return cs;
    uint64_t sig = 0x9E3779B97F4A7C15ull ^ (uint64_t)n_nodes;
    for (int i = 0; i < n_nodes; ++i) sig = (sig ^ (uint64_t)nodes[i]->op) * 0x100000001B3ull;
    if (n_nodes > 0)
        for (int d = 0; d < 4; ++d)
            sig = (sig ^ (uint64_t)nodes[0]->ne[d] ^ ((uint64_t)nodes[n_nodes - 1]->ne[d] << 32)) * 0x100000001B3ull;
    sig |= 1;
    int slot = -1;
    for (int k = 0; k < tts_hip_backend::N_GSIG; ++k)
        if (be->gsig[k] == sig) slot = k;
    if (slot < 0) {
        slot = be->gsig_next;
        be->gsig_next = (be->gsig_next + 1) % tts_hip_backend::N_GSIG;
        be->gsig[slot] = sig;
        if (be->gsig_exec[slot]) {
            TTS_HIP_CHECK(hipGraphExecDestroy(be->gsig_exec[slot]));
            be->gsig_exec[slot] = nullptr;
        }
        return graph_compute_launches(be, nodes, n_nodes);
    }
    if (!capture_worthy(be, nodes, n_nodes)) return graph_compute_launches(be, nodes, n_nodes);
    const int st = capture_into(be, nodes, n_nodes, be->gsig_exec[slot]);
    if (st != 0) return st;
    TTS_HIP_CHECK(hipGraphLaunch(be->gsig_exec[slot], be->stream));
    return 0;
}

extern "C" int tts_hip_graph_prepare(tts_hip_backend_t be, tts_tensor * const * nodes, int n_nodes, int slot) {
    if (!be || slot < 0 || slot > 1) return TTS_STATUS_BAD_ARG;
    hipSetDevice(be->device);
    be->rb_clear();
    if (be->plan_ev_pending[slot]) {
        const auto t0 = std::chrono::steady_clock::now();
        TTS_HIP_CHECK(hipEventSynchronize(be->plan_ev[slot]));
        be->plan_wait_ns += std::chrono::duration_cast<std::chrono::nanoseconds>(std::chrono::steady_clock::now() - t0).count();
        be->plan_ev_pending[slot] = false;
    }
    be->plan_nodes[slot] = nodes;
    be->plan_n[slot] = n_nodes;
    be->plan_eager[slot] = !capture_worthy(be, nodes, n_nodes);
    if (be->plan_eager[slot]) return 0;
    const int st = capture_into(be, nodes, n_nodes, be->pexec[slot]);
    be->plan_prepared[slot] = st == 0;
    return st;
}

extern "C" int tts_hip_graph_launch(tts_hip_backend_t be, int slot) {
    if (!be || slot < 0 || slot > 1) return TTS_STATUS_BAD_ARG;
    hipSetDevice(be->device);
    be->rb_clear();
    if (be->plan_eager[slot]) {
        const int st = graph_compute_launches(be, be->plan_nodes[slot], be->plan_n[slot]);
        if (st != 0) return st;
    } else {
        if (!be->pexec[slot]) return TTS_STATUS_BAD_ARG;
        TTS_HIP_CHECK(hipGraphLaunch(be->pexec[slot], be->stream));
        be->plan_prepared[slot] = false;
    }
    TTS_HIP_CHECK(hipEventRecord(be->plan_ev[slot], be->stream));
    be->plan_ev_pending[slot] = true;
    return 0;
}

extern "C" int tts_hip_plan_stats(tts_tensor * const * nodes, int n_nodes, int mask, int32_t * counts) {
    Planner pl;
    pl.mask = mask;
    pl.vec_cap = 1u << 18;
    static float lstm_stand_in alignas(256);
    pl.lstm_buf = &lstm_stand_in;
    pl.lstm_cap = (size_t)4 << 20;
    static float conv_stand_in alignas(256);
    pl.conv_stage = &conv_stand_in;
    pl.conv_stage_cap = (size_t)8 << 20;
    static char hoist_stand_in alignas(256);
    pl.hoist_buf = &hoist_stand_in;
    pl.hoist_cap = (size_t)8 << 20;
    if (mask) pl.build(nodes, n_nodes);
    else pl.act.assign(n_nodes, 0);
    for (int k = 0; k < 16; ++k) counts[k] = 0;
    for (const Item & it : pl.items) {
        counts[(int)it.kind]++;
        if (it.xattn >= 0) counts[14]++;
        if (it.kind == Item::GEMV) {
            counts[12] += (int32_t)it.mms.size();
            if ((int32_t)it.mms.size() > counts[13]) counts[13] = (int32_t)it.mms.size();
        }
    }
    static const bool dump = getenv("TTS_PLAN_DUMP") != nullptr;
    if (dump)
        for (int i = 0; i < n_nodes; ++i)
            if (pl.act[i] > 0) {
                const Item & it = pl.items[pl.act[i] - 1];
                fprintf(stderr, "item %d kind %d", i, (int)it.kind);
                if (it.kind == Item::GEMV)
                    fprintf(stderr, " mms %d K %lld N %lld M %lld epi %d ln %d", (int)it.mms.size(), (long long)it.mms[0]->src[0]->ne[0],
                            (long long)it.mms[0]->src[0]->ne[1], (long long)(nel(it.mms[0]->src[1]) / it.mms[0]->src[1]->ne[0]), it.epi, (int)it.ln);
                if (it.kind == Item::COPY) fprintf(stderr, " bytes %zu", it.cp_bytes);
                fprintf(stderr, "\n");
            }
    for (int i = 0; i < n_nodes; ++i)
        if (pl.act[i] == 0 && !is_view(nodes[i]->op)) {
            counts[15]++;
            if (dump)
                fprintf(stderr, "unfused %d op %d [%lld %lld %lld %lld] %s <- %s\n", i, (int)nodes[i]->op, (long long)nodes[i]->ne[0],
                        (long long)nodes[i]->ne[1], (long long)nodes[i]->ne[2], (long long)nodes[i]->ne[3], nodes[i]->name,
                        nodes[i]->src[0] ? nodes[i]->src[0]->name : "");
        }
    return (int)pl.items.size();
}

namespace tts {
static void plan_setup(Planner & pl, const tts_hip_backend * be) {
    pl.mask = be->fusion;
    pl.q80pro = be->gemv_q80_pro != 0;
    pl.lstm_buf = be->lstm_buf;
    pl.lstm_cap = be->lstm_floats;
    pl.vec_cap = be->vec_scratch ? (1u << 18) : 0;
    pl.conv_stage = be->conv_stage;
    pl.conv_stage_cap = be->conv_stage_floats;
    pl.hoist_buf = (char *)be->hoist;
    pl.hoist_cap = be->hoist_size;
// ... 198 lines not shown
```

tts.cpp_amd/csrc/hip_internal.h:

```cpp
#pragma once

#include <hip/hip_fp16.h>
#include <hip/hip_runtime.h>

#include <cstdio>
#include <cstdlib>
#include <atomic>
#include <deque>
#include <mutex>
#include <unordered_map>
#include <tuple>
#include <vector>

#include "common.h"

#define TTS_HIP_CHECK(expr)                                                                          \
    do {                                                                                             \
        hipError_t err_ = (expr);                                                                    \
        if (err_ != hipSuccess) {                                                                    \
            fprintf(stderr, "%s:%d: HIP error %s: %s\n", __FILE__, __LINE__, #expr, hipGetErrorString(err_)); \
            abort();                                                                                 \
        }                                                                                            \
    } while (0)

// ... 252 lines not shown
    const int64_t * koff = nullptr;
    const int64_t * voff = nullptr;
    const int64_t * moff = nullptr;
    const int * pseq = nullptr;
};

constexpr int EMBED_MAX_TERMS = 16;
struct BatchCls {
    const char * b0 = nullptr;
    size_t size = 0;
    char * win = nullptr;
    int64_t stride = 0;
};
struct ItemTab {
    const int64_t * yoff = nullptr;
    int32_t yoff_mats = 0;
    const int64_t *koff = nullptr, *voff = nullptr;
    const int64_t * moff = nullptr;
    const int * pseq = nullptr;
    int pmax = 0;
    const int64_t * ioff[EMBED_MAX_TERMS] = {};
};
struct BatchCtx {
    int N = 0;
    uint64_t key = 0;
    std::vector<BatchCls> cls;
    std::vector<tts_tensor * const *> mnodes;
    std::vector<tts_hip_backend *> mbe;
    int n_nodes = 0;
    bool checked = false;
    int canon = 0;
    bool ragged = false;
    bool differs = false;
    std::vector<ItemTab> tabs;
    void * comap = nullptr;
    const BatchCls * find(const void * p) const {
        const char * c = (const char *)p;
        size_t lo = 0, hi = cls.size();
        while (lo < hi) {
            const size_t m = (lo + hi) / 2;
            if (cls[m].b0 <= c) lo = m + 1;
            else hi = m;
        }
        if (lo == 0) return nullptr;
        const BatchCls & b = cls[lo - 1];
        return c < b.b0 + b.size ? &b : nullptr;
    }
    template <typename T>
    T * win(T * p) const {
        const BatchCls * b = p ? find(p) : nullptr;
        return b ? (T *)(b->win + ((const char *)p - b->b0)) : p;
    }
    int64_t stride(const void * p) const {
        const BatchCls * b = p ? find(p) : nullptr;
        return b ? b->stride : 0;
    }
    template <typename T>
    T * reloc(T * p, int k) const {
        const BatchCls * b = p ? find(p) : nullptr;
        return b ? (T *)(b->win + k * b->stride + ((const char *)p - b->b0)) : p;
    }
};

}

struct tts_hip_backend {
    int device = 0;
    hipStream_t stream = nullptr;
    char name[64] = {0};
    char * scratch = nullptr;
    size_t scratch_size = 0;
    float * shadow = nullptr;
    size_t shadow_size = 0;
    void * hoist = nullptr;
    size_t hoist_size = 0;
    float * attn_buf = nullptr;
    size_t attn_floats = 0;
    int attn_split_minp = 128;
    int attn_ks = 2;
    int attn_pv_mp = 1;
    int attn_one = 1;
    int attn_pv8 = 0;
    int attn_pv_uv16 = 0;
    int attn_fused_minp = 0;
    unsigned long long * argmax_keys = nullptr;
    unsigned * argmax_counts = nullptr;
    int64_t q4k_tile_bytes = 4 << 20;
    int gemv_dbg = 0;
    int gemv_unique = 1;
    int gemm_q8 = 1;
    int64_t cus = 256;
    int cu_total = 256;
    int bgemm_f32 = 1;
    int gemv_f32_wide = 1;
    int gemm_kr_nw = 4;
    int64_t gemv_ks_tiles = 256;
    int gemv_mf_prequant = 1;
    int gemv_kr = 1;
    int gemv_kr_loop = 1;
    int gemv_kr_tail = 1;
    int gemv_q80_pro = 1;
    int gemv_q80_slab = 1;
    int gemv_q80_rw = 0;
    int gemm_q8_staged = 2;
    int gemv_q50_slab = 1;
    int gemv_q50_rw = 0;
    int gemm_q5 = 1;
    int gemm_q5_staged = 2;
    int gemv_q40_slab = 1;
    int gemv_q40_rw = 0;
    int gemm_q4_0 = 1;
    int gemm_q4_0_staged = 2;
    int64_t gemv_kr_ink = 0;
    int gemm_kr_walk = 0;
    int gemm_pf = 64;
    int gemm_pf_nw = 4;
    int gemm_kr_cp = 0;
    int gemm_kr_xcd = 0;
    int gemm_kr_ct2 = 0;
    int64_t gemm_kr_ink = 0;
    int gemv_nw_min = 0;
    int gemv_mf_rsplit = 1;
    int64_t q4k_dual_bytes = 1 << 20;
    void * sample_cand = nullptr;
    size_t sample_cand_size = 0;
    int kv_prefetch_minp = 0;
    int kv_prefetch_blocks = 128;
    hipStream_t pf_stream = nullptr;
    hipEvent_t pf_fork = nullptr, pf_join = nullptr;
    uint8_t * pin = nullptr;
    size_t pin_size = 0, pin_head = 0;
    struct PinRec {
        size_t off, size;
        hipEvent_t ev;
    };
    std::deque<PinRec> pin_pending;
    std::vector<hipEvent_t> pin_events;
    std::mutex pin_mu;
    hipEvent_t plan_ev[2] = {nullptr, nullptr};
    bool plan_ev_pending[2] = {false, false};
    float * lstm_buf = nullptr;
    float * conv_stage = nullptr;
    size_t conv_stage_floats = 0;
    float * vec_scratch = nullptr;
    size_t lstm_floats = 0;
    tts::ActQuant aq;
    int64_t graph_epoch = 0;
    uint16_t * gelu_table = nullptr;
    bool convt_lds = true;
    double * conv_part = nullptr;
    size_t conv_part_doubles = 0;
    int conv_vfma = 1;
    int conv_tile96 = 1;
    int conv_split = 1;
    int fusion = 0x3FFF;
    bool profile_gemv = false;
    double gemv_ms[TTS_TYPE_COUNT] = {0};
    int64_t gemv_launches[TTS_TYPE_COUNT] = {0};
    double gemv_bytes[TTS_TYPE_COUNT] = {0};
    std::vector<std::pair<hipEvent_t, hipEvent_t>> ev_pending;
    std::vector<double> ev_bytes;
    std::vector<int> ev_type;
    std::vector<hipEvent_t> ev_free;
    char * repack_tmp = nullptr;
    size_t repack_tmp_size = 0;
    std::vector<char *> repack_retired;
    float * attn_stage = nullptr;
    size_t attn_stage_size = 0;
    bool use_graphs = false;
    static constexpr int N_GSIG = 4;
    uint64_t gsig[N_GSIG] = {};
    hipGraphExec_t gsig_exec[N_GSIG] = {};
    int gsig_next = 0;
    bool conv_f32acc = false;
    int conv_acc_mode = 0;
    hipStream_t cap_stream = nullptr;
    int64_t graph_updates = 0, graph_instantiations = 0;
    int64_t lstm_chains = 0, lstm_steps = 0;
    int64_t plan_wait_ns = 0;
    int64_t cap_plan_ns = 0, cap_launch_ns = 0, cap_update_ns = 0;
    hipGraphExec_t pexec[2] = {nullptr, nullptr};
    tts_tensor * const * plan_nodes[2] = {nullptr, nullptr};
    int plan_n[2] = {0, 0};
    bool plan_eager[2] = {true, true};
    bool plan_prepared[2] = {false, false};
    tts::BatchCtx * bat = nullptr;
    hipEvent_t co_ev = nullptr;
    int64_t * co_tab = nullptr;
    size_t co_tab_bytes = 0;
    int64_t co_prep_ns = 0;
    bool co_member = true;
    struct RbEnt {
        const char * dev;
        size_t bytes, off;
    };
    char * rb_host = nullptr;
    size_t rb_cap = 0;
    std::vector<RbEnt> rb;
    std::mutex rb_mu;
    std::atomic<bool> rb_any{false};
    void rb_clear() {
        if (!rb_any.load(std::memory_order_acquire)) return;
        std::lock_guard<std::mutex> l(rb_mu);
        rb.clear();
        rb_any.store(false, std::memory_order_release);
    }
};

namespace tts {

const uint8_t * tiled_copy_find(const void * weight);

void profile_pair(tts_hip_backend * be, hipEvent_t & e0, hipEvent_t & e1);
void profile_push(tts_hip_backend * be, hipEvent_t e0, hipEvent_t e1, double bytes, int type);

void launch_quantize_act(tts_hip_backend * be, int wtype, const float * x, int64_t xcs, int64_t K, int64_t M, ActQuant & aq);
void launch_gemv_job(tts_hip_backend * be, const GemvJob & job);
bool launch_bgemm_f32(tts_hip_backend * be, const tts_tensor * node);
bool gemm_f32_ok(const GemvJob & j);
void launch_gemm_f32(tts_hip_backend * be, const GemvJob & j);
void launch_copy_cols(tts_hip_backend * be, float * dst, const float * src, int64_t K, int64_t scs, int64_t M);
void launch_profile_spin(tts_hip_backend * be, double us);
void launch_im2col(tts_hip_backend * be, const tts_tensor * node);
constexpr int kLstmQMaxK = 512;
struct LstmStepArgs {
    const float * pre[4];
    const void * w[4];
    int64_t w_rs[4];
    const float * bias[4];
    const float * hprev;
    const float * cprev;
    float * h;
    float * c;
    int Hd, K, wtype;
};
void launch_lstm_step(tts_hip_backend * be, const LstmStepArgs & a, const LstmStepArgs * b = nullptr);
void launch_repeat_interleave1(tts_hip_backend * be, const tts_tensor * dst, const tts_tensor * a, int r);
void launch_copy_bytes(tts_hip_backend * be, void * dst, const void * src, size_t bytes);
void launch_cpy_multi(tts_hip_backend * be, const tts_tensor * src, const tts_tensor * const * dsts, int nd);
void launch_rope_multi(tts_hip_backend * be, const tts_tensor * rope, const tts_tensor * src, const tts_tensor * const * dsts, int nd);
void launch_greedy_step(tts_hip_backend * be, const float * logits, int B, int NH, int V, int step, int bos, int eos, int32_t * eos_seen,
                        int32_t * hist, int32_t * next);
int launch_sample_step(tts_hip_backend * be, const float * logits, int B, int NH, int V, const tts_sampling * c, int64_t call,
                       int32_t * rep_state, int step, int bos, int eos, int32_t * eos_seen, int32_t * hist, int32_t * next);
struct BatchCtx;
void launch_embed_sum(tts_hip_backend * be, const tts_tensor * out, const tts_tensor * const * gr, int n, const BatchCtx * bat = nullptr,
                      const ItemTab * tab = nullptr);
void launch_snake(tts_hip_backend * be, const tts_tensor * dst, const tts_tensor * x, const tts_tensor * alpha, const tts_tensor * recip,
                  const tts_tensor * one = nullptr, const tts_tensor * mask = nullptr);
void launch_lstm_finish(tts_hip_backend * be, const tts_tensor * final_out, const float * hist, int64_t Hd, int64_t T);
bool audio_op_supported(const tts_tensor * n);
int launch_audio_op(tts_hip_backend * be, const tts_tensor * n);
void launch_conv_transpose_1d(tts_hip_backend * be, const tts_tensor * node);
constexpr int CONV1D_MAX_R = 128;
struct Conv1dArgs {
    TD x;
    const void * w = nullptr;
    int w16 = 0;
    int64_t wk = 0, wic = 0, woc = 0;
    float * y = nullptr;
    int64_t ycs = 0;
    const float * bias = nullptr;
    int64_t bcs = 0;
    const float * res = nullptr;
    int64_t rcs = 0;
    int64_t L = 0, IC = 0, OL = 0, OC = 0;
    int K = 1, s = 1, p = 0, d = 1;
    int icc = 0, xw = 0, rs = 0;
    float * copy_dst = nullptr;
    uint32_t x_bytes = 0, w_bytes = 0;
    double * part = nullptr;
    int ic_per_split = 0;
};
constexpr int CONV1D_XN = 16, CONV1D_WN = 16;
inline int conv1d_icc(int64_t IC, int K, int xw) {
    int best = 0;
    double best_eff = -1.0;
    const int top = (int)(IC < 64 ? IC : 64);
    for (int c = 1; c <= top; ++c) {
        const int r = c * K, rp = (r + 31) & ~31;
        if (rp > 64 || c * xw > 256 * CONV1D_XN) break;
        const double eff = (double)r / rp + 1e-4 * c;
        if (eff > best_eff) best_eff = eff, best = c;
    }
    return best;
}
bool conv1d_fused_ok(int64_t IC, int K, int s, int d, size_t * lds);
struct AdainArgs {
    const float * x = nullptr;
    int64_t xcs = 0;
    float * y = nullptr;
    int64_t ycs = 0;
    const float *gamma = nullptr, *beta = nullptr, *alpha = nullptr, *recip = nullptr;
    const float * one = nullptr;
    int stage = 0;
    const float *gw = nullptr, *gb = nullptr, *bw = nullptr, *bb = nullptr, *style = nullptr;
    int64_t S = 0;
    int64_t gcs = 1, bcs = 1, acs = 1, rcs = 1;
    int64_t T = 0, C = 0;
    float eps = 0.f;
};
bool adain_supported(int64_t T);
void launch_adain_snake(tts_hip_backend * be, const AdainArgs & a);
void launch_conv1d_fused(tts_hip_backend * be, Conv1dArgs a);
bool launch_gemm_f16(tts_hip_backend * be, const tts_tensor * node);
size_t act_quant_bytes(int wtype, int64_t K, int64_t M);
void act_quant_layout(int wtype, char * base, int64_t K, int64_t M, ActQuant & aq);

void launch_repack_q4_K(tts_hip_backend * be, const void * src, void * dst, int64_t nblocks, int inverse);

int launch_op(tts_hip_backend * be, const tts_tensor * node);
void launch_copy_stream(tts_hip_backend * be, void * dst, const void * src, int64_t n16);

int graph_compute_launches(tts_hip_backend * be, tts_tensor * const * nodes, int n_nodes);
constexpr int kCoalesceNotTaken = 1 << 20;
int coalesce_submit(tts_hip_backend * be, tts_tensor * const * nodes, int n_nodes);
bool buffer_lookup(const void * p, const char ** base, size_t * size);
bool coalesce_check_shared(tts_hip_backend * ex, const std::vector<std::tuple<const void *, const void *, size_t>> & pairs);
void coalesce_backend_gone(const tts_hip_backend * be);
void coalesce_written(const void * p, size_t size);
bool coalesce_enabled();
bool co_debug();

}
```

tts.cpp_amd/csrc/k_conv.hip:

```cpp
#include "hip_internal.h"

namespace tts {

template <bool F16OUT>
__global__ void k_im2col(TD dst, TD x, int K, int s0, int p0, int d0, int64_t n) {
    const int64_t KW = dst.ne[0];
    const int64_t OL = dst.ne[1];
    const int64_t L = x.ne[0];
    for (int64_t e = (int64_t)blockIdx.x * blockDim.x + threadIdx.x; e < n; e += (int64_t)gridDim.x * blockDim.x) {
        const int64_t kk = e % KW;
        const int64_t ol = (e / KW) % OL;
        const int64_t nn = e / (KW * OL);
        const int64_t ic = kk / K, k = kk % K;
        const int64_t il = ol * s0 + k * d0 - p0;
        float v = 0.f;
        if (il >= 0 && il < L) v = *(const float *)(x.data + il * x.nb[0] + ic * x.nb[1] + nn * x.nb[2]);
        char * o = dst.data + kk * dst.nb[0] + ol * dst.nb[1] + nn * dst.nb[2];
        if (F16OUT) *(__half *)o = __float2half_rn(v);
        else *(float *)o = v;
    }
}

void launch_im2col(tts_hip_backend * be, const tts_tensor * node) {
    const tts_tensor * a = node->src[0];
// ... 75 lines not shown
            if (j >= N) continue;
            float * dp = D + j * ldd + i;
#pragma unroll
            for (int e = 0; e < 4; ++e)
                if (i + e < M) dp[e] = acc[ti][tj][e];
        }
    }
}

typedef double f64x4_t __attribute__((ext_vector_type(4)));

template <bool BF16>
__global__ __launch_bounds__(256) void k_gemm_f16_f64acc(const __half * __restrict__ A, int64_t lda, const void * __restrict__ B, int64_t ldb,
                                                         float * __restrict__ D, int64_t ldd, int64_t M, int64_t N, int64_t K,
                                                         double * __restrict__ part = nullptr, int64_t kps = 0) {
    const int64_t kb = part ? (int64_t)blockIdx.z * kps : 0;
    const int64_t ke = part ? min(K, kb + kps) : K;
    const int lane = threadIdx.x & 63, wave = threadIdx.x >> 6;
    const int64_t i0 = (int64_t)blockIdx.x * 64 + (wave & 1) * 32;
    const int64_t j0 = (int64_t)blockIdx.y * 64 + (wave >> 1) * 32;
    const int r16 = lane & 15, kq = lane >> 4;
    int64_t ia[2], jb[2];
#pragma unroll
    for (int t = 0; t < 2; ++t) {
        ia[t] = min(i0 + 16 * t + r16, M - 1);
        jb[t] = min(j0 + 16 * t + r16, N - 1);
    }
    f64x4_t acc[2][2] = {};
    half8_t a[2], b[2], an[2], bn[2];
    auto load = [&](int64_t k0, half8_t (&fa)[2], half8_t (&fb)[2]) {
        const int64_t k = k0 + 8 * kq;
        const bool kin = k < ke;
        const int64_t kc = kin ? k : 0;
#pragma unroll
        for (int t = 0; t < 2; ++t) {
            half8_t va = __builtin_bit_cast(half8_t, *(const uint4 *)(A + ia[t] * lda + kc));
            half8_t vb = load_b_frag<BF16>(B, ldb, jb[t], kc);
            const half8_t z = {};
            fa[t] = kin ? va : z;
            fb[t] = kin ? vb : z;
        }
    };
    load(kb, a, b);
    for (int64_t k0 = kb; k0 < ke; k0 += 32) {
        if (k0 + 32 < ke) load(k0 + 32, an, bn);
#pragma unroll
        for (int t = 0; t < 8; ++t) {
            double ad[2], bd[2];
#pragma unroll
            for (int u = 0; u < 2; ++u) ad[u] = (double)(float)a[u][t], bd[u] = (double)(float)b[u][t];
#pragma unroll
            for (int ti = 0; ti < 2; ++ti)
#pragma unroll
                for (int tj = 0; tj < 2; ++tj) acc[ti][tj] = __builtin_amdgcn_mfma_f64_16x16x4f64(ad[ti], bd[tj], acc[ti][tj], 0, 0, 0);
        }
#pragma unroll
        for (int t = 0; t < 2; ++t) a[t] = an[t], b[t] = bn[t];
    }
#pragma unroll
    for (int ti = 0; ti < 2; ++ti) {
#pragma unroll
        for (int tj = 0; tj < 2; ++tj) {
            const int64_t j = j0 + 16 * tj + r16;
            if (j >= N) continue;
#pragma unroll
            for (int e = 0; e < 4; ++e) {
                const int64_t i = i0 + 16 * ti + kq + 4 * e;
                if (i >= M) continue;
                if (part) part[((int64_t)blockIdx.z * N + j) * M + i] = acc[ti][tj][e];
                else D[j * ldd + i] = (float)acc[ti][tj][e];
            }
        }
    }
}

__global__ __launch_bounds__(256) void k_split_reduce(const double * __restrict__ part, int nz, int64_t M, int64_t N, float * __restrict__ y,
                                                      int64_t ldy, const float * __restrict__ bias, int64_t bcs, const float * __restrict__ res,
                                                      int64_t rcs) {
    const int64_t e = (int64_t)blockIdx.x * 256 + threadIdx.x;
    if (e >= M * N) return;
    const int64_t j = e / M, i = e - j * M;
    double s = 0.0;
    for (int z = 0; z < nz; ++z) s += part[((int64_t)z * N + j) * M + i];
    float v = (float)s;
    if (bias) v = v + bias[j * bcs];
    if (res) v = res[i + j * rcs] + v;
    y[i + j * ldy] = v;
}

static int split_count(const tts_hip_backend * be, int64_t tiles, int64_t K, int64_t minlen, int64_t outs) {
    const int64_t target = be->conv_split > 1 ? be->conv_split : 512;
    if (!be->conv_split || 2 * tiles >= target) return 1;
    int64_t z = (target + tiles - 1) / tiles;
    const int64_t zk = K / minlen;
    if (z > zk) z = zk;
    const int64_t zm = outs > 0 ? (int64_t)(be->conv_part_doubles / (size_t)outs) : 1;
    if (z > zm) z = zm;
    return z < 2 ? 1 : (int)z;
}

static void launch_split_reduce(tts_hip_backend * be, int nz, int64_t M, int64_t N, float * y, int64_t ldy, const float * bias, int64_t bcs,
                                const float * res, int64_t rcs) {
    const int64_t n = M * N;
    hipLaunchKernelGGL(k_split_reduce, dim3((unsigned)((n + 255) / 256)), dim3(256), 0, be->stream, (const double *)be->conv_part, nz, M, N, y, ldy,
                       bias, bcs, res, rcs);
}

bool launch_gemm_f16(tts_hip_backend * be, const tts_tensor * node) {
    const tts_tensor * a = node->src[0];
    const tts_tensor * b = node->src[1];
    if (a->type != TTS_TYPE_F16 || (b->type != TTS_TYPE_F32 && b->type != TTS_TYPE_F16)) return false;
    if (a->ne[2] * a->ne[3] != 1 || b->ne[2] * b->ne[3] != 1 || node->type != TTS_TYPE_F32) return false;
    const int64_t K = a->ne[0], M = a->ne[1], N = b->ne[1];
    const size_t bes = tts_type_size(b->type);
    if (K % 8 || a->nb[0] != 2 || b->nb[0] != bes || node->nb[0] != 4) return false;
    if (a->nb[1] % 16 || b->nb[1] % 16 || ((uintptr_t)a->data % 16) || ((uintptr_t)b->data % 16)) return false;
    dim3 grid((unsigned)((M + 63) / 64), (unsigned)((N + 63) / 64));
    if (!be->conv_f32acc) {
        const int nz = split_count(be, (int64_t)grid.x * grid.y, K, 256, M * N);
        const int64_t kps = nz > 1 ? (((K + nz - 1) / nz + 31) & ~(int64_t)31) : K;
        const int nzr = nz > 1 ? (int)((K + kps - 1) / kps) : 1;
        double * part = nzr > 1 ? be->conv_part : nullptr;
        grid.z = (unsigned)nzr;
        if (b->type == TTS_TYPE_F16)
            hipLaunchKernelGGL(k_gemm_f16_f64acc<true>, grid, dim3(256), 0, be->stream, (const __half *)a->data, (int64_t)(a->nb[1] / 2), b->data,
                               (int64_t)(b->nb[1] / 2), (float *)node->data, (int64_t)(node->nb[1] / 4), M, N, K, part, kps);
        else
            hipLaunchKernelGGL(k_gemm_f16_f64acc<false>, grid, dim3(256), 0, be->stream, (const __half *)a->data, (int64_t)(a->nb[1] / 2), b->data,
                               (int64_t)(b->nb[1] / 4), (float *)node->data, (int64_t)(node->nb[1] / 4), M, N, K, part, kps);
        TTS_HIP_CHECK(hipGetLastError());
        if (part) launch_split_reduce(be, nzr, M, N, (float *)node->data, (int64_t)(node->nb[1] / 4), nullptr, 0, nullptr, 0);
        return true;
    }
    if (b->type == TTS_TYPE_F16)
        hipLaunchKernelGGL(k_gemm_f16_mfma<true>, grid, dim3(256), 0, be->stream, (const __half *)a->data, (int64_t)(a->nb[1] / 2), b->data,
                           (int64_t)(b->nb[1] / 2), (float *)node->data, (int64_t)(node->nb[1] / 4), M, N, K);
    else
        hipLaunchKernelGGL(k_gemm_f16_mfma<false>, grid, dim3(256), 0, be->stream, (const __half *)a->data, (int64_t)(a->nb[1] / 2), b->data,
                           (int64_t)(b->nb[1] / 4), (float *)node->data, (int64_t)(node->nb[1] / 4), M, N, K);
    TTS_HIP_CHECK(hipGetLastError());
    return true;
}

typedef _Float16 h16x8_t __attribute__((ext_vector_type(8)));

template <bool BIAS, bool RES>
__device__ __forceinline__ float conv1d_epilogue(double acc, float bias, float res) {
    float v = (float)acc;
    if (BIAS) v = v + bias;
    if (RES) v = res + v;
    return v;
}

template <bool W16, bool BIAS, bool RES, bool H32 = false, int MT = 2>
__global__ __launch_bounds__(256) __attribute__((amdgpu_waves_per_eu(MT == 2 ? 1 : 2))) void k_conv1d_f64(Conv1dArgs a) {
    constexpr int OCT = 32 * MT, WN = CONV1D_WN * MT / 2;
    extern __shared__ float sm[];
    __shared__ int xoff[CONV1D_MAX_R];
    __shared__ int wofs[CONV1D_MAX_R];
    const int lane = threadIdx.x & 63, wave = threadIdx.x >> 6;
    const int c16 = lane & 15, kq = lane >> 4;
    const int64_t ol0 = (int64_t)blockIdx.x * 64;
    const int oc0 = blockIdx.y * OCT;
    const int K = a.K, s = a.s, icc = a.icc, xw = a.xw, rs = a.rs;
    const int R = icc * K, Rp = (R + 31) & ~31;
    float * xs = sm;
    float * ws = sm + icc * xw + 1;
    const int zslot = icc * xw;
    for (int r = threadIdx.x; r < Rp; r += 256) {
        const int ic = r / K, k = r - ic * K;
        xoff[r] = r < R ? ic * xw + k * a.d : zslot;
        wofs[r] = r < R ? (int)(k * a.wk + ic * a.wic) : -1;
    }
    if (threadIdx.x == 0) xs[zslot] = 0.f;
    __syncthreads();
    const int wr0 = (wave >> 1) * 16 * MT, wc0 = (wave & 1) * 32;
    const bool wave_live = oc0 + wr0 < a.OC && ol0 + wc0 < a.OL;
    f64x4_t acc[MT][2] = {};
    const int64_t base = ol0 * s - a.p;
    const int EX = icc * xw, EW = OCT * Rp;
    constexpr int esz = W16 ? 2 : 4;
    const uint32_t OOB = 0x80000000u;
    const auto xr = __builtin_amdgcn_make_buffer_rsrc(a.x.data, 0, a.x_bytes, 0x00020000);
    const auto wr = __builtin_amdgcn_make_buffer_rsrc(const_cast<void *>(a.w), 0, a.w_bytes, 0x00020000);
    const int rsh = Rp == 64 ? 6 : 5;
    uint32_t xrel[CONV1D_XN], wrel[WN];
#pragma unroll
    for (int u = 0; u < CONV1D_XN; ++u) {
        const int e = (int)threadIdx.x + 256 * u;
        const int ic = e / xw, q = e - ic * xw;
        const int64_t pos = base + q;
        const bool ok = e < EX && pos >= 0 && pos < a.L;
        xrel[u] = ok ? (uint32_t)(pos * a.x.nb[0] + (int64_t)ic * a.x.nb[1]) : OOB;
    }
#pragma unroll
    for (int u = 0; u < WN; ++u) {
        const int e = (int)threadIdx.x + 256 * u;
        const int oc = e >> rsh, r = e & (Rp - 1);
        const int wo = e < EW ? wofs[r] : -1;
        const bool ok = wo >= 0 && oc0 + oc < a.OC;
        wrel[u] = ok ? (uint32_t)(((int64_t)(oc0 + oc) * a.woc + wo) * esz) : OOB;
    }
    float xv[CONV1D_XN], wv[WN];
    auto fetch = [&](int ic0) {
        const int nic = min(icc, (int)(a.IC - ic0));
        const uint32_t xc = (uint32_t)((int64_t)ic0 * a.x.nb[1]);
        const uint32_t wc = (uint32_t)((int64_t)ic0 * a.wic * esz);
#pragma unroll
        for (int u = 0; u < CONV1D_XN; ++u) {
            const uint32_t off = (xrel[u] == OOB || (int)threadIdx.x + 256 * u >= nic * xw) ? OOB : xrel[u] + xc;
            xv[u] = __builtin_bit_cast(float, __builtin_amdgcn_raw_buffer_load_b32(xr, off, 0, 0));
        }
#pragma unroll
        for (int u = 0; u < WN; ++u) {
            const uint32_t off = (wrel[u] == OOB || (((int)threadIdx.x + 256 * u) & (Rp - 1)) >= nic * K) ? OOB : wrel[u] + wc;
            if (W16) wv[u] = __half2float(__builtin_bit_cast(__half, __builtin_amdgcn_raw_buffer_load_b16(wr, off, 0, 0)));
            else wv[u] = __builtin_bit_cast(float, __builtin_amdgcn_raw_buffer_load_b32(wr, off, 0, 0));
        }
    };
    const int ic_lo = a.part ? (int)blockIdx.z * a.ic_per_split : 0;
    const int ic_hi = a.part ? (int)min((int64_t)(ic_lo + a.ic_per_split), a.IC) : (int)a.IC;
    fetch(ic_lo);
    for (int ic0 = ic_lo; ic0 < ic_hi; ic0 += icc) {
#pragma unroll
        for (int u = 0; u < CONV1D_XN; ++u)
            if ((int)threadIdx.x + 256 * u < EX) xs[(int)threadIdx.x + 256 * u] = __half2float(__float2half_rn(xv[u]));
#pragma unroll
        for (int u = 0; u < WN; ++u) {
            const int e = (int)threadIdx.x + 256 * u;
            if (e < EW) ws[e + (e >> rsh)] = W16 ? wv[u] : __half2float(__float2half_rn(wv[u]));
        }
        __syncthreads();
        if (ic0 + icc < ic_hi) fetch(ic0 + icc);
        if (!wave_live) {
            __syncthreads();
            continue;
        }
        if (H32) {
            for (int r0 = 0; r0 < Rp; r0 += 32) {
                int xo[8];
#pragma unroll
                for (int u = 0; u < 8; ++u) xo[u] = xoff[r0 + 8 * kq + u];
                h16x8_t A[MT], B[2];
#pragma unroll
                for (int u = 0; u < 8; ++u) {
                    const bool z = xo[u] == zslot;
#pragma unroll
                    for (int t = 0; t < MT; ++t) A[t][u] = (_Float16)ws[(wr0 + 16 * t + c16) * rs + r0 + 8 * kq + u];
#pragma unroll
                    for (int t = 0; t < 2; ++t) B[t][u] = (_Float16)xs[z ? zslot : xo[u] + (wc0 + 16 * t + c16) * s];
                }
#pragma unroll
                for (int ti = 0; ti < MT; ++ti)
#pragma unroll
                    for (int tj = 0; tj < 2; ++tj) {
                        const f32x4 pr = __builtin_amdgcn_mfma_f32_16x16x32_f16(A[ti], B[tj], f32x4{0.f, 0.f, 0.f, 0.f}, 0, 0, 0);
#pragma unroll
                        for (int e = 0; e < 4; ++e) acc[ti][tj][e] += (double)pr[e];
                    }
            }
        } else
        for (int r0 = 0; r0 < Rp; r0 += 32) {
            int xo[8];
#pragma unroll
            for (int u = 0; u < 8; ++u) xo[u] = xoff[r0 + 4 * u + kq];
            float af[8][MT], bf[8][2];
#pragma unroll
            for (int u = 0; u < 8; ++u) {
                const int r = r0 + 4 * u + kq;
                const bool z = xo[u] == zslot;
#pragma unroll
                for (int t = 0; t < MT; ++t) af[u][t] = ws[(wr0 + 16 * t + c16) * rs + r];
#pragma unroll
                for (int t = 0; t < 2; ++t) bf[u][t] = xs[z ? zslot : xo[u] + (wc0 + 16 * t + c16) * s];
            }
#pragma unroll
            for (int u = 0; u < 8; ++u)
#pragma unroll
                for (int ti = 0; ti < MT; ++ti)
#pragma unroll
                    for (int tj = 0; tj < 2; ++tj)
                        acc[ti][tj] = __builtin_amdgcn_mfma_f64_16x16x4f64((double)af[u][ti], (double)bf[u][tj], acc[ti][tj], 0, 0, 0);
        }
        __syncthreads();
    }
    if (a.part) {
#pragma unroll
        for (int tj = 0; tj < 2; ++tj) {
            const int64_t ol = ol0 + wc0 + 16 * tj + c16;
            if (ol >= a.OL) continue;
#pragma unroll
            for (int ti = 0; ti < MT; ++ti)
#pragma unroll
                for (int e = 0; e < 4; ++e) {
                    const int oc = oc0 + wr0 + 16 * ti + (H32 ? 4 * kq + e : kq + 4 * e);
                    if (oc < a.OC) a.part[((int64_t)blockIdx.z * a.OC + oc) * a.OL + ol] = acc[ti][tj][e];
                }
        }
        return;
    }
    float bv[MT][4], rv[2][MT][4];
#pragma unroll
    for (int ti = 0; ti < MT; ++ti)
#pragma unroll
        for (int e = 0; e < 4; ++e) {
            const int oc = min(oc0 + wr0 + 16 * ti + (H32 ? 4 * kq + e : kq + 4 * e), (int)a.OC - 1);
            bv[ti][e] = BIAS ? a.bias[(int64_t)oc * a.bcs] : 0.f;
#pragma unroll
            for (int tj = 0; tj < 2; ++tj) {
                const int64_t ol = min(ol0 + wc0 + 16 * tj + c16, a.OL - 1);
                rv[tj][ti][e] = RES ? a.res[ol + (int64_t)oc * a.rcs] : 0.f;
            }
        }
#pragma unroll
    for (int tj = 0; tj < 2; ++tj) {
        const int64_t ol = ol0 + wc0 + 16 * tj + c16;
        if (ol >= a.OL) continue;
#pragma unroll
        for (int ti = 0; ti < MT; ++ti)
#pragma unroll
            for (int e = 0; e < 4; ++e) {
                const int oc = oc0 + wr0 + 16 * ti + (H32 ? 4 * kq + e : kq + 4 * e);
                if (oc >= a.OC) continue;
                a.y[ol + (int64_t)oc * a.ycs] = conv1d_epilogue<BIAS, RES>(acc[ti][tj][e], bv[ti][e], rv[tj][ti][e]);
            }
    }
}

constexpr int CONV1DV_NP = 4;
template <bool W16, bool BIAS, bool RES>
__global__ __launch_bounds__(256) void k_conv1d_f64v(Conv1dArgs a) {
    constexpr int NP = CONV1DV_NP;
    extern __shared__ double smd[];
    const int K = a.K, d = a.d, icc = a.icc, xw = a.xw, R = icc * K;
    double * xs = smd;
    double * ws = smd + icc * xw;
    const int tid = threadIdx.x;
    const int64_t ol0 = (int64_t)blockIdx.x * (256 * NP);
    const int oc = blockIdx.y;
    const int64_t base = ol0 - a.p;
    const int EX = icc * xw;
    constexpr int esz = W16 ? 2 : 4;
    const uint32_t OOB = 0x80000000u;
    const auto xr = __builtin_amdgcn_make_buffer_rsrc(a.x.data, 0, a.x_bytes, 0x00020000);
    const auto wr = __builtin_amdgcn_make_buffer_rsrc(const_cast<void *>(a.w), 0, a.w_bytes, 0x00020000);
    uint32_t xrel[CONV1D_XN];
#pragma unroll
    for (int u = 0; u < CONV1D_XN; ++u) {
        const int e = tid + 256 * u;
        const int ic = e / xw, q = e - ic * xw;
        const int64_t pos = base + q;
        const bool ok = e < EX && pos >= 0 && pos < a.L;
        xrel[u] = ok ? (uint32_t)(pos * a.x.nb[0] + (int64_t)ic * a.x.nb[1]) : OOB;
    }
    const int wicl = tid < R ? tid / K : -1;
    const uint32_t wrel = tid < R ? (uint32_t)(((int64_t)oc * a.woc + (int64_t)(tid - wicl * K) * a.wk + (int64_t)wicl * a.wic) * esz) : OOB;
    float xv[CONV1D_XN], wv;
    auto fetch = [&](int ic0) {
        const int nic = min(icc, (int)(a.IC - ic0));
        const uint32_t xc = (uint32_t)((int64_t)ic0 * a.x.nb[1]);
        const uint32_t wc = (uint32_t)((int64_t)ic0 * a.wic * esz);
#pragma unroll
        for (int u = 0; u < CONV1D_XN; ++u) {
            const uint32_t off = (xrel[u] == OOB || tid + 256 * u >= nic * xw) ? OOB : xrel[u] + xc;
            xv[u] = __builtin_bit_cast(float, __builtin_amdgcn_raw_buffer_load_b32(xr, off, 0, 0));
        }
        const uint32_t off = (wrel == OOB || wicl >= nic) ? OOB : wrel + wc;
        if (W16) wv = __half2float(__builtin_bit_cast(__half, __builtin_amdgcn_raw_buffer_load_b16(wr, off, 0, 0)));
        else wv = __builtin_bit_cast(float, __builtin_amdgcn_raw_buffer_load_b32(wr, off, 0, 0));
    };
    double acc[NP];
#pragma unroll
    for (int j = 0; j < NP; ++j) acc[j] = 0.0;
    fetch(0);
    for (int ic0 = 0; ic0 < a.IC; ic0 += icc) {
        const int nic = min(icc, (int)(a.IC - ic0));
#pragma unroll
        for (int u = 0; u < CONV1D_XN; ++u)
            if (tid + 256 * u < EX) xs[tid + 256 * u] = (double)__half2float(__float2half_rn(xv[u]));
        if (wicl >= 0) ws[tid] = (double)(W16 ? wv : __half2float(__float2half_rn(wv)));
        __syncthreads();
        if (ic0 + icc < a.IC) fetch(ic0 + icc);
        const double * xp = xs + tid;
        for (int icl = 0; icl < nic; ++icl, xp += xw)
            for (int k = 0; k < K; ++k) {
                const double w = ws[icl * K + k];
#pragma unroll
                for (int j = 0; j < NP; ++j) acc[j] = __builtin_fma(xp[k * d + 256 * j], w, acc[j]);
            }
        __syncthreads();
    }
    const float bias = BIAS ? a.bias[(int64_t)oc * a.bcs] : 0.f;
#pragma unroll
    for (int j = 0; j < NP; ++j) {
        const int64_t ol = ol0 + tid + 256 * j;
        if (ol >= a.OL) continue;
        const float res = RES ? a.res[ol + (int64_t)oc * a.rcs] : 0.f;
        a.y[ol + (int64_t)oc * a.ycs] = conv1d_epilogue<BIAS, RES>(acc[j], bias, res);
    }
}

static bool conv1d_vfma_geometry(const Conv1dArgs & a, int * xw, int * icc, size_t * lds) {
    if (a.s != 1 || a.K < 1 || a.K > 64 || a.OC > 65535) return false;
    const int64_t w = 256 * CONV1DV_NP + (int64_t)(a.K - 1) * a.d;
    if (w > 256 * CONV1D_XN) return false;
    int c = (int)std::min<int64_t>(std::min<int64_t>(a.IC, 256 * CONV1D_XN / w), 256 / a.K);
    if (c < 1) return false;
    *xw = (int)w, *icc = c, *lds = ((size_t)c * (size_t)w + (size_t)c * a.K) * sizeof(double);
    return true;
}

bool conv1d_fused_ok(int64_t IC, int K, int s, int d, size_t * lds) {
    if (K < 1 || K > 64 || s < 1 || d < 1 || IC < 1) return false;
    const int xw = 63 * s + (K - 1) * d + 1;
    const int icc = conv1d_icc(IC, K, xw);
    if (icc < 1) return false;
    const int rs = ((icc * K + 31) & ~31) + 1;
    const size_t bytes = ((size_t)icc * xw + 1 + 64 * (size_t)rs) * 4;
    if (lds) *lds = bytes;
    return bytes <= 64 * 1024;
}

void launch_conv1d_fused(tts_hip_backend * be, Conv1dArgs a) {
    a.xw = 63 * a.s + (a.K - 1) * a.d + 1;
    a.icc = conv1d_icc(a.IC, a.K, a.xw);
    a.rs = ((a.icc * a.K + 31) & ~31) + 1;
    size_t lds = 0;
    if (!conv1d_fused_ok(a.IC, a.K, a.s, a.d, &lds)) {
        fprintf(stderr, "tts_hip: conv1d_fused shape unsupported\n");
        abort();
    }
    dim3 grid((unsigned)((a.OL + 63) / 64), (unsigned)((a.OC + 63) / 64));
    Conv1dArgs e = a;
    const int64_t nchunk = (a.IC + a.icc - 1) / a.icc;
    const int nz = be->conv_acc_mode == 2 ? 1 : split_count(be, (int64_t)grid.x * grid.y, nchunk, 2, a.OL * a.OC);
    if (nz > 1) {
        a.ic_per_split = (int)(((nchunk + nz - 1) / nz) * a.icc);
        grid.z = (unsigned)((a.IC + a.ic_per_split - 1) / a.ic_per_split);
        a.part = be->conv_part;
        a.bias = nullptr;
        a.res = nullptr;
    }
    const int sel = (a.w16 ? 4 : 0) | (a.bias ? 2 : 0) | (a.res ? 1 : 0);
#define TTS_CONV1D_SEL(KERNEL, GRID, LDS, ...)                                                                           \
    switch (sel) {                                                                                                        \
        case 0: hipLaunchKernelGGL((KERNEL<false, false, false __VA_ARGS__>), GRID, dim3(256), LDS, be->stream, a); break; \
        case 1: hipLaunchKernelGGL((KERNEL<false, false, true __VA_ARGS__>), GRID, dim3(256), LDS, be->stream, a); break;  \
        case 2: hipLaunchKernelGGL((KERNEL<false, true, false __VA_ARGS__>), GRID, dim3(256), LDS, be->stream, a); break;  \
        case 3: hipLaunchKernelGGL((KERNEL<false, true, true __VA_ARGS__>), GRID, dim3(256), LDS, be->stream, a); break;   \
        case 4: hipLaunchKernelGGL((KERNEL<true, false, false __VA_ARGS__>), GRID, dim3(256), LDS, be->stream, a); break;  \
        case 5: hipLaunchKernelGGL((KERNEL<true, false, true __VA_ARGS__>), GRID, dim3(256), LDS, be->stream, a); break;   \
        case 6: hipLaunchKernelGGL((KERNEL<true, true, false __VA_ARGS__>), GRID, dim3(256), LDS, be->stream, a); break;   \
        default: hipLaunchKernelGGL((KERNEL<true, true, true __VA_ARGS__>), GRID, dim3(256), LDS, be->stream, a); break;   \
    }
#define TTS_COMMA ,
    int vxw = 0, vicc = 0;
    size_t vlds = 0;
    if (nz == 1 && be->conv_acc_mode != 2 && be->conv_vfma && (be->conv_vfma == 2 || a.OC < 8) && conv1d_vfma_geometry(a, &vxw, &vicc, &vlds)) {
        a.xw = vxw, a.icc = vicc;
        const dim3 vgrid((unsigned)((a.OL + 256 * CONV1DV_NP - 1) / (256 * CONV1DV_NP)), (unsigned)a.OC);
        TTS_CONV1D_SEL(k_conv1d_f64v, vgrid, vlds)
    } else if (nz == 1 && be->conv_acc_mode != 2 && be->conv_tile96 && a.OC % 96 == 0) {
        grid.y = (unsigned)(a.OC / 96);
        lds += 32 * (size_t)a.rs * 4;
        TTS_CONV1D_SEL(k_conv1d_f64, grid, lds, TTS_COMMA false TTS_COMMA 3)
    } else if (be->conv_acc_mode == 2) {
        TTS_CONV1D_SEL(k_conv1d_f64, grid, lds, TTS_COMMA true)
    } else {
        TTS_CONV1D_SEL(k_conv1d_f64, grid, lds)
    }
#undef TTS_COMMA
#undef TTS_CONV1D_SEL
    TTS_HIP_CHECK(hipGetLastError());
    if (a.part) launch_split_reduce(be, (int)grid.z, a.OL, a.OC, e.y, e.ycs, e.bias, e.bcs, e.res, e.rcs);
    if (a.copy_dst)
        launch_copy_bytes(be, a.copy_dst, a.y, (size_t)a.OL * (size_t)a.OC * 4);
}

__global__ __launch_bounds__(256) void k_conv_transpose_1d(TD y, TD x, TD w, int s, int p, int d, int g) {
    const int64_t OL = y.ne[0];
    const int64_t o = (int64_t)blockIdx.x * blockDim.x + threadIdx.x;
    const int oc = blockIdx.y;
    if (o >= OL) return;
    const int K = (int)w.ne[0], OCg = (int)w.ne[1];
    const int64_t L = x.ne[0];
    const int IC = (int)x.ne[1], ICg = IC / g;
    const int grp = oc / OCg, ocl = oc % OCg;
    double acc = 0.0;
    const int64_t num0 = o + p;
    for (int k = (d == 1 ? (int)(num0 % s) : 0); k < K; k += (d == 1 ? s : 1)) {
        const int64_t num = num0 - (int64_t)k * d;
        if (num < 0) break;
        if (num % s) continue;
        const int64_t i = num / s;
        if (i >= L) continue;
        const char * xp = x.data + i * x.nb[0] + (int64_t)grp * ICg * x.nb[1];
        const char * wp = w.data + (int64_t)k * w.nb[0] + (int64_t)ocl * w.nb[1] + (int64_t)grp * ICg * w.nb[2];
        if (w.type == TTS_TYPE_F16) {
            for (int icl = 0; icl < ICg; ++icl)
                acc = __fma_rn((double)__half2float(__float2half_rn(*(const float *)(xp + icl * x.nb[1]))),
                               (double)__half2float(*(const __half *)(wp + icl * w.nb[2])), acc);
        } else {
            for (int icl = 0; icl < ICg; ++icl)
                acc = __fma_rn((double)*(const float *)(xp + icl * x.nb[1]), (double)*(const float *)(wp + icl * w.nb[2]), acc);
        }
    }
    *(float *)(y.data + o * y.nb[0] + (int64_t)oc * y.nb[1]) = (float)acc;
}

__global__ __launch_bounds__(64) void k_conv_transpose_1d_mfma(TD y, TD x, TD w, int s, int p) {
    const int lane = threadIdx.x, r16 = lane & 15, kq = lane >> 4;
    const int rr = blockIdx.z;
    const int64_t q0 = (int64_t)blockIdx.x * 16;
    const int oc0 = blockIdx.y * 16;
    const int K = (int)w.ne[0], OC = (int)w.ne[1], IC = (int)w.ne[2];
    const int64_t L = x.ne[0], OL = y.ne[0];
    const int J = (K - rr + s - 1) / s;
    const int oca = min(oc0 + r16, OC - 1);
    const int64_t qb = q0 + r16;
    f64x4_t acc = {};
    for (int j = 0; j < J; ++j) {
        const int k = rr + s * j;
        const int64_t i = qb - j;
        const bool iin = i >= 0 && i < L;
        const char * wp = w.data + (int64_t)k * w.nb[0] + (int64_t)oca * w.nb[1];
        const char * xp = x.data + (iin ? i : 0) * x.nb[0];
        for (int ic0 = 0; ic0 < IC; ic0 += 16) {
            double av[4], bv[4];
#pragma unroll
            for (int u = 0; u < 4; ++u) {
                const int ic = ic0 + 4 * u + kq;
                const int icc = min(ic, IC - 1);
                const bool w16 = w.type == TTS_TYPE_F16;
                const float wa = w16 ? __half2float(*(const __half *)(wp + (int64_t)icc * w.nb[2])) : *(const float *)(wp + (int64_t)icc * w.nb[2]);
                float xb = *(const float *)(xp + (int64_t)icc * x.nb[1]);
                if (w16) xb = __half2float(__float2half_rn(xb));
                av[u] = ic < IC ? (double)wa : 0.0;
                bv[u] = (ic < IC && iin) ? (double)xb : 0.0;
            }
#pragma unroll
            for (int u = 0; u < 4; ++u) acc = __builtin_amdgcn_mfma_f64_16x16x4f64(av[u], bv[u], acc, 0, 0, 0);
        }
    }
    const int64_t o = qb * s + rr - p;
    if (o < 0 || o >= OL) return;
#pragma unroll
    for (int e = 0; e < 4; ++e) {
        const int oc = oc0 + kq + 4 * e;
        if (oc < OC) *(float *)(y.data + o * y.nb[0] + (int64_t)oc * y.nb[1]) = (float)acc[e];
    }
}

template <int S, bool W16>
__global__ __launch_bounds__(256) void k_convt_f64_lds(TD y, TD x, TD w, int p, double * __restrict__ part = nullptr, int icps = 0) {
    constexpr int JM = 2, K = 2 * S;
    constexpr int QT = 64, OCT = 32, ICC = 16, XW = QT + JM - 1;
    constexpr int NX = ICC * XW, NW4 = ICC * K * OCT / 4;
    constexpr int XR = (NX + 255) / 256, WR = (NW4 + 255) / 256;
    constexpr int XWP = 80;
    constexpr int WK = S == 8 ? 34 : S == 4 ? 36 : OCT + 1;
    constexpr int WIC0 = K * WK, WIC = WIC0 + ((16 - WIC0 % 32) + 32) % 32;
    __shared__ float xs[ICC][XWP];
    __shared__ float ws[ICC * WIC];
    const int lane = threadIdx.x & 63, qw = threadIdx.x >> 6;
    const int c16 = lane & 15, kq = lane >> 4;
    const int OC = (int)w.ne[1], IC = (int)w.ne[2];
    const int64_t L = x.ne[0], OL = y.ne[0];
    const int64_t q0 = (int64_t)blockIdx.x * QT;
    const int oc0 = blockIdx.y * OCT;
    f64x4_t acc[S][2];
#pragma unroll
    for (int r = 0; r < S; ++r) acc[r][0] = acc[r][1] = (f64x4_t){0.0, 0.0, 0.0, 0.0};
    float xr[XR];
    float4 wr[WR];
    auto fetch = [&](int ic0) {
#pragma unroll
        for (int u = 0; u < XR; ++u) {
            const int t = threadIdx.x + 256 * u;
            const int ic = t / XW, qq = t - ic * XW;
            const int64_t pos = q0 - (JM - 1) + qq;
            const bool ok = t < NX && pos >= 0 && pos < L && ic0 + ic < IC;
            xr[u] = ok ? *(const float *)(x.data + pos * x.nb[0] + (int64_t)(ic0 + ic) * x.nb[1]) : 0.f;
            if (W16) xr[u] = __half2float(__float2half_rn(xr[u]));
        }
#pragma unroll
        for (int u = 0; u < WR; ++u) {
            const int t = threadIdx.x + 256 * u;
            const int ic = t / (K * OCT / 4), rem = (t - ic * (K * OCT / 4)) * 4;
            const int oc = rem / K;
            const bool ok = t < NW4 && oc0 + oc < OC && ic0 + ic < IC;
            const char * src = w.data + (int64_t)(oc0 + oc) * w.nb[1] + (int64_t)(ic0 + ic) * w.nb[2] + (rem - oc * K) * (W16 ? 2 : 4);
            if (W16) {
                const uint2 h = ok ? *(const uint2 *)src : make_uint2(0u, 0u);
                wr[u] = make_float4(__half2float(__ushort_as_half((unsigned short)(h.x & 0xFFFF))), __half2float(__ushort_as_half((unsigned short)(h.x >> 16))),
                                    __half2float(__ushort_as_half((unsigned short)(h.y & 0xFFFF))), __half2float(__ushort_as_half((unsigned short)(h.y >> 16))));
            } else {
                wr[u] = ok ? *(const float4 *)src : make_float4(0.f, 0.f, 0.f, 0.f);
            }
        }
    };
    auto stage = [&]() {
#pragma unroll
        for (int u = 0; u < XR; ++u) {
            const int t = threadIdx.x + 256 * u;
            if (t < NX) xs[t / XW][t % XW] = xr[u];
        }
#pragma unroll
        for (int u = 0; u < WR; ++u) {
            const int t = threadIdx.x + 256 * u;
            if (t >= NW4) continue;
            const int ic = t / (K * OCT / 4), rem = (t - ic * (K * OCT / 4)) * 4;
            const int oc = rem / K, k = rem - oc * K;
            float * o = ws + ic * WIC + k * WK + oc;
            o[0] = wr[u].x, o[WK] = wr[u].y, o[2 * WK] = wr[u].z, o[3 * WK] = wr[u].w;
// ... 97 lines not shown
```

tts.cpp_amd/ttship/__init__.py:

```python
import ctypes
import os
import pathlib

_HERE = pathlib.Path(__file__).resolve().parent
PKG_ROOT = _HERE.parent
REPO_ROOT = PKG_ROOT.parent
LIB_PATH = PKG_ROOT / "lib" / "libtts_hip.so"

F32, F16, Q4_0, Q5_0, Q8_0, Q4_K, Q8_K, I32 = 0, 1, 2, 6, 8, 12, 15, 26
PROF_ATTN = 39

OPS = ["NONE", "DUP", "ADD", "SUB", "MUL", "DIV", "SQR", "SQRT", "SIN", "COS", "SUM_ROWS", "REPEAT",
       "CONCAT", "NORM", "RMS_NORM", "MUL_MAT", "SCALE", "CPY", "CONT", "RESHAPE", "VIEW", "PERMUTE",
       "TRANSPOSE", "GET_ROWS", "SOFT_MAX", "ROPE", "CLAMP", "CONV_TRANSPOSE_1D", "IM2COL", "UPSCALE",
       "PAD", "LEAKY_RELU", "UNARY", "CUMSUM", "MOD", "ROUND", "STFT", "ISTFT", "MAP_CUSTOM3", "MAP_CUSTOM2"]
OP = {n: i for i, n in enumerate(OPS)}
FUSE = {"LN": 1, "GROUP": 2, "KV": 4, "EPI": 8, "HEADS": 16, "ATTN": 32, "LSTM": 64, "SNAKE": 128, "EMBED": 256, "CONV": 512, "ADAIN": 1024, "XATTN": 2048, "MCPY": 4096, "CONTREAD": 8192}
FUSE_ALL = sum(FUSE.values())
UNARY = {"ABS": 0, "NEG": 1, "TANH": 2, "RELU": 3, "SIGMOID": 4, "GELU": 5, "SILU": 6, "EXP": 7}

OPT = {"FUSION": 0, "PROFILE_GEMV": 1, "GRAPHS": 2, "CONV_F32ACC": 3, "CONVT_LDS": 4, "ATTN_SPLIT": 5, "KV_PREFETCH": 6, "KV_PREFETCH_BLOCKS": 7, "Q4K_TILE_BYTES": 8, "GEMV_DEBUG": 10, "GEMV_UNIQUE": 11, "CONV_SPLIT": 12, "GEMV_KS": 13, "ATTN_FUSED": 14, "ATTN_PV16": 15, "Q4K_DUAL_BYTES": 16, "GEMV_RSPLIT": 17, "GEMM_Q8": 18, "BGEMM_F32": 19, "CU_PARTITION": 20, "GEMV_PREQUANT": 21, "GEMV_KRELAY": 22, "ATTN_KS": 23, "ATTN_PV8": 24, "GEMV_NW_MIN": 25, "GEMV_KRELAY_LOOP": 26, "GEMV_Q80_PRO": 27, "GEMV_Q80_SLAB": 28, "GEMV_Q80_RW": 29, "GEMM_Q8_STAGED": 30, "GEMV_KR_INKERNEL": 31, "GEMV_F32_WIDE": 32, "ATTN_PV_MP": 33, "GEMM_KR_NW": 34, "GEMM_KR_INKERNEL": 35, "GEMM_KR_CT2": 36, "COALESCE": 37, "GEMM_KR_XCD": 38, "GEMM_KR_CP": 39, "GEMM_KR_WALK": 40, "GEMM_PF": 41, "GEMM_PF_NW": 42, "ATTN_ONE": 43, "GEMV_KR_TAIL": 44, "GEMV_Q50_SLAB": 45, "GEMV_Q50_RW": 46, "GEMM_Q5": 47, "GEMM_Q5_STAGED": 48, "GEMV_Q40_SLAB": 49, "GEMV_Q40_RW": 50, "GEMM_Q4_0": 51, "GEMM_Q4_0_STAGED": 52, "CONV_VFMA": 53, "CONV_TILE96": 54}
ATTN_SPLIT_DEFAULT = 128
ATTN_ONE_DEFAULT = 1
GEMV_KR_TAIL_DEFAULT = 1
ATTN_FUSED_ON = 128

TYPE_SIZE = {F32: 4, F16: 2, Q4_K: 144, Q8_0: 34, Q5_0: 22, Q4_0: 18, I32: 4}
BLCK_SIZE = {F32: 1, F16: 1, Q4_K: 256, Q8_0: 32, Q5_0: 32, Q4_0: 32, I32: 1}


class TtsTensor(ctypes.Structure):
    pass


TtsTensor._fields_ = [
    ("type", ctypes.c_int32),
    ("op", ctypes.c_int32),
    ("ne", ctypes.c_int64 * 4),
    ("nb", ctypes.c_uint64 * 4),
    ("op_params", ctypes.c_int32 * 16),
    ("src", ctypes.POINTER(TtsTensor) * 4),
    ("view_src", ctypes.POINTER(TtsTensor)),
    ("view_offs", ctypes.c_uint64),
    ("data", ctypes.c_void_p),
    ("flags", ctypes.c_int32),
    ("pad_", ctypes.c_int32),
    ("name", ctypes.c_char * 64),
]


class BackendIface(ctypes.Structure):
    _fields_ = [
        ("ctx", ctypes.c_void_p),
        ("name", ctypes.c_char_p),
        ("alloc", ctypes.c_void_p),
        ("free", ctypes.c_void_p),
        ("set", ctypes.c_void_p),
        ("set_tensor", ctypes.c_void_p),
        ("get", ctypes.c_void_p),
        ("memset", ctypes.c_void_p),
        ("compute", ctypes.c_void_p),
        ("synchronize", ctypes.c_void_p),
        ("prepare", ctypes.c_void_p),
        ("launch", ctypes.c_void_p),
        ("set_async", ctypes.c_void_p),
        ("copy", ctypes.c_void_p),
        ("greedy_step", ctypes.c_void_p),
        ("sample_step", ctypes.c_void_p),
    ]


class Sampling(ctypes.Structure):
    _fields_ = [
        ("temperature", ctypes.c_float),
        ("top_p", ctypes.c_float),
        ("repetition_penalty", ctypes.c_float),
        ("top_k", ctypes.c_int32),
        ("do_sample", ctypes.c_int32),
        ("pad_", ctypes.c_int32),
        ("seed", ctypes.c_uint64),
    ]


def sampling(**kw):
    c = Sampling()
    lib().tts_sampling_default(ctypes.byref(c))
    for k, v in kw.items():
        setattr(c, k, v)
    return c


def call_seed(seed, stream, call):
    return int(lib().tts_sampler_call_seed(seed, stream, call))


def host_sample(cfg, logits, call_seed_, last=None, count=None):
    import numpy as np
    lg = np.ascontiguousarray(logits, dtype=np.float32)
    NH, V = lg.shape
    out = np.zeros(NH, dtype=np.int32)
    if last is None:
        last = np.full(NH, -1, dtype=np.int32)
    if count is None:
        count = np.zeros(NH, dtype=np.int32)
    st = lib().tts_sampler_sample(ctypes.byref(cfg), lg.ctypes.data, NH, V, call_seed_, last.ctypes.data, count.ctypes.data, out.ctypes.data)
    if st != 0:
        raise RuntimeError(f"tts_sampler_sample failed {st}")
    return out


class ParlerConfig(ctypes.Structure):
    _fields_ = [
        ("n_layers", ctypes.c_int32),
        ("hidden_size", ctypes.c_int32),
        ("n_attn_heads", ctypes.c_int32),
        ("ffn_size", ctypes.c_int32),
        ("n_output_heads", ctypes.c_int32),
        ("output_vocab", ctypes.c_int32),
        ("audio_vocab", ctypes.c_int32),
        ("max_ctx", ctypes.c_int32),
        ("n_encode", ctypes.c_int32),
        ("prompt_vocab", ctypes.c_int32),
        ("max_positions", ctypes.c_int32),
        ("weight_type", ctypes.c_int32),
        ("head_type", ctypes.c_int32),
        ("use_cross_attn", ctypes.c_int32),
        ("batch", ctypes.c_int32),
        ("eos_token", ctypes.c_int32),
        ("bos_token", ctypes.c_int32),
        ("seed", ctypes.c_uint64),
        ("arena_bytes", ctypes.c_uint64),
        ("debug_no_reuse", ctypes.c_int32),
        ("pad_", ctypes.c_int32),
    ]


class T5Config(ctypes.Structure):
    _fields_ = [
        ("n_layers", ctypes.c_int32),
        ("hidden_size", ctypes.c_int32),
        ("n_attn_heads", ctypes.c_int32),
        ("head_size", ctypes.c_int32),
        ("ffn_size", ctypes.c_int32),
        ("relative_attn_buckets", ctypes.c_int32),
        ("vocab_size", ctypes.c_int32),
        ("max_context_length", ctypes.c_int32),
        ("output_size", ctypes.c_int32),
        ("has_down_proj", ctypes.c_int32),
        ("weight_type", ctypes.c_int32),
        ("eos_token_id", ctypes.c_int32),
        ("seed", ctypes.c_uint64),
        ("arena_bytes", ctypes.c_uint64),
        ("debug_no_reuse", ctypes.c_int32),
        ("pad_", ctypes.c_int32),
    ]


class OrpheusConfig(ctypes.Structure):
    _fields_ = [
        ("n_layers", ctypes.c_int32),
        ("hidden_size", ctypes.c_int32),
        ("n_attn_heads", ctypes.c_int32),
        ("n_kv_attn_heads", ctypes.c_int32),
        ("head_size", ctypes.c_int32),
        ("ffn_size", ctypes.c_int32),
        ("vocab_size", ctypes.c_int32),
        ("max_ctx", ctypes.c_int32),
        ("weight_type", ctypes.c_int32),
        ("batch", ctypes.c_int32),
        ("seed", ctypes.c_uint64),
        ("arena_bytes", ctypes.c_uint64),
        ("rope_theta", ctypes.c_float),
        ("rope_factor", ctypes.c_float),
        ("rope_low_freq_factor", ctypes.c_float),
# ... 308 lines not shown
        "tts_gguf_arr_n": (i64, [vp, i64]),
        "tts_gguf_arr_data": (vp, [vp, i64]),
        "tts_gguf_arr_str": (ctypes.c_char_p, [vp, i64, i64]),
        "tts_gguf_n_tensors": (i64, [vp]),
        "tts_gguf_find_tensor": (i64, [vp, ctypes.c_char_p]),
        "tts_gguf_tensor_name": (ctypes.c_char_p, [vp, i64]),
        "tts_gguf_tensor_type": (i32, [vp, i64]),
        "tts_gguf_tensor_ndims": (i32, [vp, i64, ctypes.POINTER(i64)]),
        "tts_gguf_tensor_offset": (u64, [vp, i64]),
        "tts_gguf_tensor_size": (u64, [vp, i64]),
        "tts_gguf_tensor_data": (vp, [vp, i64]),
        "tts_gguf_type_size": (sz, [i32]),
        "tts_gguf_blck_size": (i64, [i32]),
        "tts_gguf_writer_new": (vp, []),
        "tts_gguf_writer_free": (None, [vp]),
        "tts_gguf_set_u32": (None, [vp, ctypes.c_char_p, ctypes.c_uint32]),
        "tts_gguf_set_i32": (None, [vp, ctypes.c_char_p, i32]),
        "tts_gguf_set_f32": (None, [vp, ctypes.c_char_p, ctypes.c_float]),
        "tts_gguf_set_u64": (None, [vp, ctypes.c_char_p, u64]),
        "tts_gguf_set_bool": (None, [vp, ctypes.c_char_p, ctypes.c_int]),
        "tts_gguf_set_str": (None, [vp, ctypes.c_char_p, ctypes.c_char_p]),
        "tts_gguf_set_arr": (None, [vp, ctypes.c_char_p, i32, vp, i64]),
        "tts_gguf_set_arr_str": (None, [vp, ctypes.c_char_p, ctypes.POINTER(ctypes.c_char_p), i64]),
        "tts_gguf_copy_kv": (None, [vp, vp]),
        "tts_gguf_add_tensor": (ctypes.c_int, [vp, ctypes.c_char_p, i32, i32, ctypes.POINTER(i64), vp, u64]),
        "tts_gguf_writer_write": (ctypes.c_int, [vp, ctypes.c_char_p]),
        "tts_gguf_tensor_rule": (ctypes.c_int, [ctypes.c_char_p, ctypes.c_char_p, ctypes.POINTER(QuantizeParams)]),
        "tts_gguf_quantize": (ctypes.c_int, [ctypes.c_char_p, ctypes.c_char_p, ctypes.POINTER(QuantizeParams), vp, vp]),
        "tts_hip_gguf_quantize": (ctypes.c_int, [vp, ctypes.c_char_p, ctypes.c_char_p, ctypes.POINTER(QuantizeParams)]),
        "tts_parler_config_from_gguf": (ctypes.c_int, [vp, ctypes.POINTER(ParlerConfig)]),
        "tts_parler_create_from_gguf": (vp, [ctypes.POINTER(BackendIface), ctypes.POINTER(ParlerConfig), vp]),
        "tts_parler_write_synthetic_gguf": (ctypes.c_int, [ctypes.POINTER(ParlerConfig), ctypes.POINTER(DacConfig), ctypes.c_char_p]),
        "tts_dac_config_from_gguf": (ctypes.c_int, [vp, ctypes.POINTER(DacConfig)]),
        "tts_dac_create_from_gguf": (vp, [ctypes.POINTER(BackendIface), ctypes.POINTER(DacConfig), vp]),
        "tts_dia_config_from_gguf": (ctypes.c_int, [vp, ctypes.POINTER(DiaConfig)]),
        "tts_dia_create_from_gguf": (vp, [ctypes.POINTER(BackendIface), ctypes.POINTER(DiaConfig), vp]),
        "tts_dia_write_synthetic_gguf": (ctypes.c_int, [ctypes.POINTER(DiaConfig), ctypes.POINTER(DacConfig), ctypes.c_char_p]),
        "tts_dia_set_weight": (ctypes.c_int, [vp, i32, vp, u64]),
        "tts_orpheus_config_from_gguf": (ctypes.c_int, [vp, ctypes.POINTER(OrpheusConfig)]),
        "tts_orpheus_create_from_gguf": (vp, [ctypes.POINTER(BackendIface), ctypes.POINTER(OrpheusConfig), vp]),
        "tts_orpheus_write_synthetic_gguf": (ctypes.c_int, [ctypes.POINTER(OrpheusConfig), ctypes.POINTER(SnacConfig), ctypes.c_char_p]),
        "tts_orpheus_set_weight": (ctypes.c_int, [vp, i32, vp, u64]),
        "tts_snac_config_from_gguf": (ctypes.c_int, [vp, ctypes.POINTER(SnacConfig)]),
        "tts_snac_create_from_gguf": (vp, [ctypes.POINTER(BackendIface), ctypes.POINTER(SnacConfig), vp]),
    }
    for name, (res, args) in sig.items():
        fn = getattr(L, name)
        fn.restype = res
        fn.argtypes = args
    _lib = L
    if os.environ.get("TTS_HIP_CRASH_HANDLER") == "1":
        L.tts_hip_install_crash_handler()
    return L


class HipBackend:

    def __init__(self, device=0):
        L = lib()
        n = L.tts_hip_device_count()
        if n <= device:
            raise RuntimeError(f"no HIP device {device} (device count {n})")
        self.ptr = L.tts_hip_backend_init(device)
        if not self.ptr:
            raise RuntimeError("tts_hip_backend_init failed")
        self.L = L

    def iface(self, reference_flow=False):
        it = BackendIface()
        if self.L.tts_hip_backend_iface(self.ptr, ctypes.byref(it)) != 0:
            raise RuntimeError("tts_hip_backend_iface failed")
        if reference_flow:
            for f in ("prepare", "launch", "set_async", "copy", "greedy_step", "sample_step"):
                setattr(it, f, None)
        return it

    def alloc(self, nbytes):
        p = self.L.tts_hip_buffer_alloc(self.ptr, nbytes)
        if not p:
            raise MemoryError(f"tts_hip_buffer_alloc({nbytes}) failed")
        return p

    def free(self, p):
        self.L.tts_hip_buffer_free(self.ptr, p)

    def set(self, dev, host_arr):
        st = self.L.tts_hip_tensor_set(self.ptr, dev, host_arr.ctypes.data, host_arr.nbytes)
        if st != 0:
            raise RuntimeError(f"tensor_set failed {st}")

    def get(self, host_arr, dev):
        st = self.L.tts_hip_tensor_get(self.ptr, host_arr.ctypes.data, dev, host_arr.nbytes)
        if st != 0:
            raise RuntimeError(f"tensor_get failed {st}")

    def sample_step(self, logits, cfg, call, rep_state=None, step=100, bos=-2, eos=-3, eos_seen=None):
        import numpy as np
        lg = np.ascontiguousarray(logits, dtype=np.float32)
        B, NH, V = lg.shape
        rs = np.ascontiguousarray(rep_state if rep_state is not None else np.tile(np.array([-1, 0], np.int32), B * NH), dtype=np.int32)
        es = np.ascontiguousarray(eos_seen if eos_seen is not None else np.zeros(B * NH, np.int32), dtype=np.int32)
        bufs = [self.alloc(n) for n in (lg.nbytes, rs.nbytes, es.nbytes, B * NH * 4, B * NH * 4)]
        try:
            self.set(bufs[0], lg)
            self.set(bufs[1], rs)
            self.set(bufs[2], es)
            st = self.L.tts_hip_sample_step(self.ptr, bufs[0], B, NH, V, ctypes.byref(cfg), call, bufs[1], step, bos, eos, bufs[2], bufs[3], bufs[4])
            if st != 0:
                raise RuntimeError(f"tts_hip_sample_step failed {st}")
            hist = np.zeros((B, NH), np.int32)
            nxt = np.zeros((NH, B), np.int32)
            self.get(hist, bufs[3])
            self.get(nxt, bufs[4])
            self.get(rs, bufs[1])
            self.get(es, bufs[2])
            return hist, nxt, es, rs
        finally:
            for b in bufs:
                self.free(b)

    def quantize(self, wtype, x):
        import numpy as np
        x = np.ascontiguousarray(x, dtype=np.float32)
        N, K = x.shape
        rs = K // BLCK_SIZE[wtype] * TYPE_SIZE[wtype]
        dx, dq = self.alloc(x.nbytes), self.alloc(N * rs)
        try:
            self.set(dx, x)
            st = self.L.tts_hip_quantize(self.ptr, wtype, dx, dq, N, K)
            if st != 0:
                raise RuntimeError(f"tts_hip_quantize failed {st}")
            out = np.empty(N * rs, dtype=np.uint8)
            self.get(out, dq)
            return out
        finally:
            self.free(dx)
            self.free(dq)

    def sync(self):
        if self.L.tts_hip_synchronize(self.ptr) != 0:
            raise RuntimeError("synchronize failed")

    def set_option(self, opt, value):
        self.L.tts_hip_set_option(self.ptr, opt, value)

    def gemv_stats(self, wtype=-1, reset=True):
        ms = ctypes.c_double()
        n = ctypes.c_int64()
        b = ctypes.c_double()
        self.L.tts_hip_gemv_stats(self.ptr, wtype, ctypes.byref(ms), ctypes.byref(n), ctypes.byref(b), 1 if reset else 0)
        return ms.value, n.value, b.value

    def counters(self):
        out = (ctypes.c_int64 * 8)()
        n = self.L.tts_hip_counters(self.ptr, out, 8)
        keys = ("graph_updates", "graph_instantiations", "lstm_chains", "lstm_steps", "plan_wait_ns",
                "cap_plan_ns", "cap_launch_ns", "cap_update_ns")
        return {keys[i]: int(out[i]) for i in range(n)}

    def close(self):
        if self.ptr:
            self.L.tts_hip_backend_free(self.ptr)
            self.ptr = None


def runner_weights(n_fn, w_fn, ptr):
    import numpy as np
    out = {}
    for i in range(n_fn(ptr)):
        name = ctypes.create_string_buffer(128)
        ne = (ctypes.c_int64 * 4)()
        ty = ctypes.c_int32()
        n = w_fn(ptr, i, name, 128, ne, ctypes.byref(ty), None, 0)
        if ty.value not in (F32, F16):
            continue
        a = np.empty(n, dtype=np.uint8)
        w_fn(ptr, i, name, 128, ne, ctypes.byref(ty), a.ctypes.data, n)
        a = a.view(np.float32 if ty.value == F32 else np.float16).astype(np.float32)
        shape = [int(v) for v in reversed(list(ne))]
        while len(shape) > 1 and shape[0] == 1:
            shape.pop(0)
        out[name.value.decode()] = a.reshape(shape)
    return out


class _Runner:
    PREFIX = None
    TYPED_WEIGHTS = True

    def _fn(self, name):
        return getattr(self.L, f"{self.PREFIX}_{name}")

    def weight_bytes(self):
        return self._fn("weight_bytes")(self.ptr)

    def weights(self):
        n_fn, w_fn = self._fn("n_weights"), self._fn("weight")
        if self.TYPED_WEIGHTS:
            return runner_weights(n_fn, w_fn, self.ptr)
        return runner_weights(n_fn, lambda ptr, i, name, cap, ne, ty, dst, n: w_fn(ptr, i, name, cap, ne, dst, n), self.ptr)

    def weights_raw(self):
        import numpy as np
        w_fn = self._fn("weight" if self.TYPED_WEIGHTS else "weight_raw")
        out = {}
        for i in range(self._fn("n_weights")(self.ptr)):
            name = ctypes.create_string_buffer(128)
            ne = (ctypes.c_int64 * 4)()
            ty = ctypes.c_int32()
            n = w_fn(self.ptr, i, name, 128, ne, ctypes.byref(ty), None, 0)
            a = np.empty(n, dtype=np.uint8)
            if w_fn(self.ptr, i, name, 128, ne, ctypes.byref(ty), a.ctypes.data, n) != n:
                raise RuntimeError(f"reading weight {name.value.decode()} failed")
            out[name.value.decode()] = (ty.value, tuple(ne), a)
        return out

    def set_weight(self, i, data):
        import numpy as np
        d = np.ascontiguousarray(data).view(np.uint8).reshape(-1)
        if self._fn("set_weight")(self.ptr, i, d.ctypes.data, d.nbytes) != 0:
            raise RuntimeError(f"setting weight {i} failed ({d.nbytes} bytes)")

    def plan_stats(self, mask=None):
        n = ctypes.c_int32()
        p = self._fn("graph")(self.ptr, ctypes.byref(n))
        return plan_stats(p, n.value, FUSE_ALL if mask is None else mask)

    def node(self, i, cap=1 << 26):
        import numpy as np
        op, ty = ctypes.c_int32(), ctypes.c_int32()
        ne = (ctypes.c_int64 * 4)()
        buf = np.empty(cap // 4, dtype=np.float32)
        n = self._fn("node")(self.ptr, i, ctypes.byref(op), ctypes.byref(ty), ne, buf.ctypes.data, cap)
        data = buf[: n // 4].copy() if n else None
        return OPS[op.value], ty.value, tuple(ne), data

    def named(self, name, dtype="float32", lead=()):
        import numpy as np
        get = self._fn("get_node")
        n = get(self.ptr, *lead, name.encode(), None, 0)
        if not n:
            return None
        a = np.empty(n // 4, dtype=dtype)
        get(self.ptr, *lead, name.encode(), a.ctypes.data, n)
        return a

    def close(self):
        if self.ptr:
            self._fn("free")(self.ptr)
            self.ptr = None


def coalesce_stats(device=0):
    out = (ctypes.c_int64 * 11)()
    n = lib().tts_hip_coalesce_stats(device, out, 11)
    keys = ("launches", "member_steps", "alone", "refused", "max_group", "wait_us", "ragged_launches", "exec_us", "layout_us",
            "plan_us", "tables_us")
    return {keys[i]: int(out[i]) for i in range(max(n, 0))}


def coalesce_set_wait(us):
    lib().tts_hip_coalesce_set_wait(int(us))


def coalesce_enable(on=True):
    return bool(lib().tts_hip_coalesce_enable(1 if on else 0))


def dia_config(**kw):
    cfg = DiaConfig()
    lib().tts_dia_default_config(ctypes.byref(cfg))
    for k, v in kw.items():
        setattr(cfg, k, v)
    return cfg


class Dia(_Runner):
    PREFIX = "tts_dia"

    def __init__(self, iface, cfg, gguf=None):
        self.L = lib()
        self.cfg = cfg
        self._iface = iface
        if gguf is None:
            self.ptr = self.L.tts_dia_create(ctypes.byref(iface), ctypes.byref(cfg))
        else:
            self.ptr = self.L.tts_dia_create_from_gguf(ctypes.byref(iface), ctypes.byref(cfg), gguf.ptr)
        if not self.ptr:
            raise RuntimeError("tts_dia_create failed")

    @classmethod
    def from_gguf(cls, iface, g, **kw):
        return cls(iface, dia_config_from_gguf(g, **kw), gguf=g)

    def prefill(self, text_ids, audio):
        import numpy as np
        c = self.cfg
        T = c.max_encoder_context_length
        t = np.zeros((2, T), dtype=np.int32)
        t[0, :len(text_ids)] = text_ids
        a = np.ascontiguousarray(audio, dtype=np.int32)
        out = np.empty((c.n_output_heads, c.output_vocab_size), dtype=np.float32)
        st = self.L.tts_dia_prefill(self.ptr, t.ctypes.data, len(text_ids), a.ctypes.data, out.ctypes.data)
        if st != 0:
            raise RuntimeError(f"prefill failed {st}")
        return out

    def decode(self, audio):
        import numpy as np
        c = self.cfg
# ... 770 lines not shown
```

Baseline: 114.9.

## Cache pre-packed f16-rounded conv weight images in MFMA fragment layout

```diff
diff --git a/include/tts_hip.h b/include/tts_hip.h
--- a/include/tts_hip.h
+++ b/include/tts_hip.h
@@ -225,6 +225,7 @@
     TTS_HIP_OPT_GEMM_Q4_0_STAGED = 52,
     TTS_HIP_OPT_CONV_VFMA = 53,
     TTS_HIP_OPT_CONV_TILE96 = 54,
+    TTS_HIP_OPT_CONV_PACK = 55,
     TTS_HIP_OPT_COALESCE = 37,
 };
 enum tts_fuse_bits {
diff --git a/tts.cpp_amd/csrc/backend.hip b/tts.cpp_amd/csrc/backend.hip
--- a/tts.cpp_amd/csrc/backend.hip
+++ b/tts.cpp_amd/csrc/backend.hip
@@ -42,6 +42,14 @@
 std::map<const char *, BufRec> g_buffers;
 std::unordered_map<const void *, uint8_t *> g_tiled;
 std::atomic<size_t> g_tiled_n{0};
+struct PackRec {
+    float * img = nullptr;
+    size_t src_bytes = 0;
+};
+std::map<tts::ConvPackKey, PackRec> g_packs;
+std::atomic<size_t> g_packs_n{0};
+std::atomic<size_t> g_packs_bytes{0};
+std::atomic<uintptr_t> g_packs_lo{UINTPTR_MAX}, g_packs_hi{0};
 }
 
 namespace tts {
@@ -55,6 +63,69 @@
     return e && e[0] == '0' ? 0 : 1;
 }()};
 bool coalesce_enabled() { return g_coalesce_on.load(std::memory_order_relaxed) != 0; }
+const float * conv_pack_get(tts_hip_backend * be, const ConvPackKey & k) {
+    std::lock_guard<std::mutex> lk(g_reg_mu);
+    auto it = g_packs.find(k);
+    if (it != g_packs.end()) return it->second.img;
+    if (be->capturing) return nullptr;
+    PackRec r;
+    const size_t es = k.w16 ? 2 : 4;
+    r.src_bytes = (size_t)((k.K - 1) * k.wk + (k.IC - 1) * k.wic + (k.OC - 1) * k.woc + 1) * es;
+    const size_t bytes = k.floats() * sizeof(float);
+    if (hipMalloc((void **)&r.img, bytes) != hipSuccess) {
+        (void)hipGetLastError();
+        return nullptr;
+    }
+    launch_conv1d_pack(be->stream, k, r.img);
+    g_packs[k] = r;
+    g_packs_lo.store(std::min(g_packs_lo.load(), (uintptr_t)k.w));
+    g_packs_hi.store(std::max(g_packs_hi.load(), (uintptr_t)k.w + r.src_bytes));
+    g_packs_n.store(g_packs.size(), std::memory_order_release);
+    g_packs_bytes.fetch_add(bytes, std::memory_order_relaxed);
+    return r.img;
+}
+void conv_pack_written(tts_hip_backend * be, const void * p, size_t n) {
+    if (g_packs_n.load(std::memory_order_acquire) == 0) return;
+    const char * a = (const char *)p;
+    if ((uintptr_t)a >= g_packs_hi.load() || (uintptr_t)a + n <= g_packs_lo.load()) return;
+    std::lock_guard<std::mutex> lk(g_reg_mu);
+    for (auto & e : g_packs) {
+        const char * w = (const char *)e.first.w;
+        if (!(w < a + n && a < w + e.second.src_bytes)) continue;
+        const tts_hip_backend * ob = e.first.be;
+        if (ob->device == be->device) {
+            launch_conv1d_pack(be->stream, e.first, e.second.img);
+        } else {
+            hipStreamSynchronize(be->stream);
+            hipSetDevice(ob->device);
+            launch_conv1d_pack(ob->stream, e.first, e.second.img);
+            hipSetDevice(be->device);
+        }
+    }
+}
+void conv_pack_freed(const tts_hip_backend * be, const void * p, size_t n) {
+    if (g_packs_n.load(std::memory_order_acquire) == 0) return;
+    const char * a = (const char *)p;
+    std::vector<float *> dead;
+    {
+        std::lock_guard<std::mutex> lk(g_reg_mu);
+        for (auto it = g_packs.begin(); it != g_packs.end();) {
+            const char * w = (const char *)it->first.w;
+            if (be ? it->first.be == be : (w >= a && w < a + n)) {
+                dead.push_back(it->second.img);
+                g_packs_bytes.fetch_sub(it->first.floats() * sizeof(float), std::memory_order_relaxed);
+                it = g_packs.erase(it);
+            } else {
+                ++it;
+            }
+        }
+        if (g_packs.empty()) g_packs_lo.store(UINTPTR_MAX), g_packs_hi.store(0);
+        g_packs_n.store(g_packs.size(), std::memory_order_release);
+    }
+    if (dead.empty()) return;
+    hipDeviceSynchronize();
+    for (float * c : dead) hipFree(c);
+}
 bool buffer_lookup(const void * p, const char ** base, size_t * size) {
     std::lock_guard<std::mutex> lk(g_reg_mu);
     auto it = g_buffers.upper_bound((const char *)p);
@@ -108,6 +179,8 @@
     TTS_HIP_CHECK(hipMalloc((void **)&be->conv_stage, be->conv_stage_floats * sizeof(float)));
     if (const char * e = getenv("TTS_HIP_OPT_CONV_VFMA"))
         if (e[0] >= '0' && e[0] <= '2' && !e[1]) be->conv_vfma = e[0] - '0';
+    if (const char * e = getenv("TTS_HIP_OPT_CONV_PACK"))
+        if (e[0] >= '0' && e[0] <= '1' && !e[1]) be->conv_pack = e[0] - '0';
     be->conv_part_doubles = (size_t)8 << 20;
     TTS_HIP_CHECK(hipMalloc((void **)&be->conv_part, be->conv_part_doubles * sizeof(double)));
     be->lstm_floats = kLstmFloats;
@@ -130,6 +203,7 @@
     tts::coalesce_backend_gone(be);
     hipSetDevice(be->device);
     hipStreamSynchronize(be->stream);
+    tts::conv_pack_freed(be, nullptr, 0);
     for (auto & p : be->ev_pending) {
         hipEventDestroy(p.first);
         hipEventDestroy(p.second);
@@ -271,6 +345,7 @@
     }
     if (known) {
         drop_tiled_copies(ptr, r.size);
+        tts::conv_pack_freed(nullptr, ptr, r.size);
         tts::coalesce_written(ptr, r.size);
     }
     hipFree(ptr);
@@ -287,6 +362,8 @@
         if (st != 0) return st;
     } else if (hipMemcpyAsync(dst, src, size, hipMemcpyHostToDevice, be->stream) != hipSuccess) {
         return TTS_STATUS_FAILED;
+    } else {
+        tts::conv_pack_written(be, dst, size);
     }
     if (hipStreamSynchronize(be->stream) != hipSuccess) return TTS_STATUS_FAILED;
     return 0;
@@ -320,6 +397,7 @@
     }
     memcpy(be->pin + off, src, size);
     if (hipMemcpyAsync(dst, be->pin + off, size, hipMemcpyHostToDevice, be->stream) != hipSuccess) return TTS_STATUS_FAILED;
+    tts::conv_pack_written(be, dst, size);
     hipEvent_t ev;
     if (be->pin_events.empty()) {
         if (hipEventCreateWithFlags(&ev, hipEventDisableTiming) != hipSuccess) return TTS_STATUS_FAILED;
@@ -375,6 +453,7 @@
     hipSetDevice(be->device);
     be->rb_clear();
     tts::launch_copy_stream(be, dst, src, (int64_t)(size / 16));
+    tts::conv_pack_written(be, dst, size);
     return hipGetLastError() == hipSuccess ? 0 : TTS_STATUS_FAILED;
 }
 
@@ -384,6 +463,7 @@
     be->rb_clear();
     tts::coalesce_written(dst, size);
     tts::launch_copy_bytes(be, dst, src, size);
+    tts::conv_pack_written(be, dst, size);
     return hipGetLastError() == hipSuccess ? 0 : TTS_STATUS_FAILED;
 }
 
@@ -392,7 +472,9 @@
     hipSetDevice(be->device);
     be->rb_clear();
     tts::coalesce_written(dst, size);
-    return hipMemsetAsync(dst, value, size, be->stream) == hipSuccess ? 0 : TTS_STATUS_FAILED;
+    if (hipMemsetAsync(dst, value, size, be->stream) != hipSuccess) return TTS_STATUS_FAILED;
+    tts::conv_pack_written(be, dst, size);
+    return 0;
 }
 
 int tts_hip_synchronize(tts_hip_backend_t be) {
@@ -727,6 +809,7 @@
         case TTS_HIP_OPT_CONV_SPLIT: be->conv_split = value < 0 ? 1 : value; return 0;
         case TTS_HIP_OPT_CONV_VFMA: be->conv_vfma = value < 0 || value > 2 ? 1 : value; return 0;
         case TTS_HIP_OPT_CONV_TILE96: be->conv_tile96 = value != 0; return 0;
+        case TTS_HIP_OPT_CONV_PACK: be->conv_pack = value != 0; return 0;
         case TTS_HIP_OPT_PROFILE_GEMV: be->profile_gemv = value != 0; return 0;
         case TTS_HIP_OPT_GRAPHS: be->use_graphs = value != 0; return 0;
         case TTS_HIP_OPT_CONV_F32ACC:
@@ -839,10 +922,10 @@
 
 extern "C" int tts_hip_counters(tts_hip_backend_t be, int64_t * out, int n) {
     if (!be || !out) return TTS_STATUS_BAD_ARG;
-    const int64_t v[8] = {be->graph_updates, be->graph_instantiations, be->lstm_chains, be->lstm_steps, be->plan_wait_ns,
-                          be->cap_plan_ns, be->cap_launch_ns, be->cap_update_ns};
+    const int64_t v[10] = {be->graph_updates, be->graph_instantiations, be->lstm_chains, be->lstm_steps, be->plan_wait_ns,
+                           be->cap_plan_ns, be->cap_launch_ns, be->cap_update_ns, (int64_t)g_packs_n.load(), (int64_t)g_packs_bytes.load()};
     int k = 0;
-    for (; k < n && k < 8; ++k) out[k] = v[k];
+    for (; k < n && k < 10; ++k) out[k] = v[k];
     return k;
 }
 
diff --git a/tts.cpp_amd/csrc/graph_exec.hip b/tts.cpp_amd/csrc/graph_exec.hip
--- a/tts.cpp_amd/csrc/graph_exec.hip
+++ b/tts.cpp_amd/csrc/graph_exec.hip
@@ -1332,6 +1332,8 @@
     }
 
     static const tts_tensor * through_view(const tts_tensor * t) { return t && t->op == TTS_OP_RESHAPE ? t->src[0] : t; }
+    bool wr_hull = false;
+    const char *wr_lo = nullptr, *wr_hi = nullptr;
     void try_conv(int i) {
         const tts_tensor * col = nodes[i];
         const tts_tensor *kern = col->src[0], *x = col->src[1];
@@ -1424,6 +1426,19 @@
         const size_t wb = tbytes(kern);
         if (xb >= 0x80000000u || wb >= 0x80000000u) return plan_reject("conv", 12);
         a.x_bytes = (uint32_t)xb, a.w_bytes = (uint32_t)wb;
+        a.w_stable = kern->op == TTS_OP_NONE && !(kern->flags & (TTS_FLAG_HOSTDATA | TTS_FLAG_OUTPUT)) && buffer_lookup(kern->data, nullptr, nullptr);
+        if (a.w_stable && !wr_hull) {
+            wr_hull = true;
+            for (int j = 0; j < n; ++j) {
+                if (is_view(nodes[j]->op) || !nodes[j]->data) continue;
+                const char * lo = (const char *)nodes[j]->data;
+                wr_lo = wr_lo ? std::min(wr_lo, lo) : lo;
+                wr_hi = std::max(wr_hi, lo + tbytes(nodes[j]));
+            }
+        }
+        if (a.w_stable && wr_lo && (const char *)kern->data < wr_hi && (const char *)kern->data + wb > wr_lo)
+            for (int j = 0; a.w_stable && j < n; ++j)
+                if (!is_view(nodes[j]->op) && nodes[j]->data && overlap(nodes[j], kern)) a.w_stable = 0;
         Item it;
         it.kind = Item::CONV;
         it.conv = a;
@@ -2655,15 +2670,35 @@
     return true;
 }
 
+namespace tts {
+static void plan_setup(Planner & pl, const tts_hip_backend * be);
+}
+static void conv_pack_prepare(tts_hip_backend * be, tts_tensor * const * nodes, int n_nodes) {
+    if (!be->conv_pack || !(be->fusion & TTS_FUSE_CONV)) return;
+    bool any = false;
+    for (int i = 0; i < n_nodes && !any; ++i) any = nodes[i]->op == TTS_OP_IM2COL;
+    if (!any) return;
+    Planner pl;
+    plan_setup(pl, be);
+    pl.build(nodes, n_nodes);
+    for (const Item & it : pl.items) {
+        ConvPackKey k;
+        if (it.kind == Item::CONV && conv1d_pack_key(be, it.conv, &k)) (void)conv_pack_get(be, k);
+    }
+}
+
 static int capture_into(tts_hip_backend * be, tts_tensor * const * nodes, int n_nodes, hipGraphExec_t & ex) {
+    conv_pack_prepare(be, nodes, n_nodes);
     hipStream_t run = be->stream;
     be->stream = be->cap_stream;
+    be->capturing = true;
     const auto t0 = std::chrono::steady_clock::now();
     TTS_HIP_CHECK(hipStreamBeginCapture(be->stream, hipStreamCaptureModeThreadLocal));
     const int st = graph_compute_launches(be, nodes, n_nodes);
     hipGraph_t graph = nullptr;
     TTS_HIP_CHECK(hipStreamEndCapture(be->stream, &graph));
     be->stream = run;
+    be->capturing = false;
     const auto t1 = std::chrono::steady_clock::now();
     be->cap_launch_ns += std::chrono::duration_cast<std::chrono::nanoseconds>(t1 - t0).count();
     if (st != 0) {
diff --git a/tts.cpp_amd/csrc/hip_internal.h b/tts.cpp_amd/csrc/hip_internal.h
--- a/tts.cpp_amd/csrc/hip_internal.h
+++ b/tts.cpp_amd/csrc/hip_internal.h
@@ -428,6 +428,8 @@
     size_t conv_part_doubles = 0;
     int conv_vfma = 1;
     int conv_tile96 = 1;
+    int conv_pack = 1;
+    bool capturing = false;
     int conv_split = 1;
     int fusion = 0x3FFF;
     bool profile_gemv = false;
@@ -547,6 +549,8 @@
     uint32_t x_bytes = 0, w_bytes = 0;
     double * part = nullptr;
     int ic_per_split = 0;
+    int w_stable = 0;
+    const float * wimg = nullptr;
 };
 constexpr int CONV1D_XN = 16, CONV1D_WN = 16;
 inline int conv1d_icc(int64_t IC, int K, int xw) {
@@ -562,6 +566,28 @@
     return best;
 }
 bool conv1d_fused_ok(int64_t IC, int K, int s, int d, size_t * lds);
+__host__ __device__ inline int64_t conv1d_pack_index(int nchunk, int oct, int rp, int ct, int chunk, int row, int r) {
+    const int lane = (r & 3) * 16 + (row & 15);
+    return (int64_t)(ct * nchunk + chunk) * oct * rp + ((((row >> 4) * (rp >> 4) + (r >> 4)) * 64 + lane) * 4 + ((r >> 2) & 3));
+}
+struct ConvPackKey {
+    const tts_hip_backend * be;
+    const void * w;
+    int w16, K, oct, icc, rp;
+    int64_t IC, OC, wk, wic, woc;
+    bool operator<(const ConvPackKey & o) const {
+        return std::tie(be, w, w16, K, oct, icc, rp, IC, OC, wk, wic, woc) <
+               std::tie(o.be, o.w, o.w16, o.K, o.oct, o.icc, o.rp, o.IC, o.OC, o.wk, o.wic, o.woc);
+    }
+    int nchunk() const { return (int)((IC + icc - 1) / icc); }
+    int ntile() const { return (int)((OC + oct - 1) / oct); }
+    size_t floats() const { return (size_t)ntile() * nchunk() * oct * rp; }
+};
+void launch_conv1d_pack(hipStream_t stream, const ConvPackKey & k, float * img);
+const float * conv_pack_get(tts_hip_backend * be, const ConvPackKey & k);
+void conv_pack_written(tts_hip_backend * be, const void * p, size_t n);
+void conv_pack_freed(const tts_hip_backend * be, const void * p, size_t n);
+bool conv1d_pack_key(const tts_hip_backend * be, const Conv1dArgs & a, ConvPackKey * k);
 struct AdainArgs {
     const float * x = nullptr;
     int64_t xcs = 0;
diff --git a/tts.cpp_amd/csrc/k_conv.hip b/tts.cpp_amd/csrc/k_conv.hip
--- a/tts.cpp_amd/csrc/k_conv.hip
+++ b/tts.cpp_amd/csrc/k_conv.hip
@@ -251,6 +251,52 @@
     return v;
 }
 
+template <bool BIAS, bool RES, bool H32, int MT>
+__device__ __forceinline__ void conv1d_store(const Conv1dArgs & a, const f64x4_t (&acc)[MT][2], int64_t ol0, int oc0, int wr0, int wc0, int c16,
+                                             int kq) {
+    if (a.part) {
+#pragma unroll
+        for (int tj = 0; tj < 2; ++tj) {
+            const int64_t ol = ol0 + wc0 + 16 * tj + c16;
+            if (ol >= a.OL) continue;
+#pragma unroll
+            for (int ti = 0; ti < MT; ++ti)
+#pragma unroll
+                for (int e = 0; e < 4; ++e) {
+                    const int oc = oc0 + wr0 + 16 * ti + (H32 ? 4 * kq + e : kq + 4 * e);
+                    if (oc < a.OC) a.part[((int64_t)blockIdx.z * a.OC + oc) * a.OL + ol] = acc[ti][tj][e];
+                }
+        }
+        return;
+    }
+    float bv[MT][4], rv[2][MT][4];
+#pragma unroll
+    for (int ti = 0; ti < MT; ++ti)
+#pragma unroll
+        for (int e = 0; e < 4; ++e) {
+            const int oc = min(oc0 + wr0 + 16 * ti + (H32 ? 4 * kq + e : kq + 4 * e), (int)a.OC - 1);
+            bv[ti][e] = BIAS ? a.bias[(int64_t)oc * a.bcs] : 0.f;
+#pragma unroll
+            for (int tj = 0; tj < 2; ++tj) {
+                const int64_t ol = min(ol0 + wc0 + 16 * tj + c16, a.OL - 1);
+                rv[tj][ti][e] = RES ? a.res[ol + (int64_t)oc * a.rcs] : 0.f;
+            }
+        }
+#pragma unroll
+    for (int tj = 0; tj < 2; ++tj) {
+        const int64_t ol = ol0 + wc0 + 16 * tj + c16;
+        if (ol >= a.OL) continue;
+#pragma unroll
+        for (int ti = 0; ti < MT; ++ti)
+#pragma unroll
+            for (int e = 0; e < 4; ++e) {
+                const int oc = oc0 + wr0 + 16 * ti + (H32 ? 4 * kq + e : kq + 4 * e);
+                if (oc >= a.OC) continue;
+                a.y[ol + (int64_t)oc * a.ycs] = conv1d_epilogue<BIAS, RES>(acc[ti][tj][e], bv[ti][e], rv[tj][ti][e]);
+            }
+    }
+}
+
 template <bool W16, bool BIAS, bool RES, bool H32 = false, int MT = 2>
 __global__ __launch_bounds__(256) __attribute__((amdgpu_waves_per_eu(MT == 2 ? 1 : 2))) void k_conv1d_f64(Conv1dArgs a) {
     constexpr int OCT = 32 * MT, WN = CONV1D_WN * MT / 2;
@@ -383,47 +429,134 @@
         }
         __syncthreads();
     }
-    if (a.part) {
-#pragma unroll
-        for (int tj = 0; tj < 2; ++tj) {
-            const int64_t ol = ol0 + wc0 + 16 * tj + c16;
-            if (ol >= a.OL) continue;
-#pragma unroll
-            for (int ti = 0; ti < MT; ++ti)
-#pragma unroll
-                for (int e = 0; e < 4; ++e) {
-                    const int oc = oc0 + wr0 + 16 * ti + (H32 ? 4 * kq + e : kq + 4 * e);
-                    if (oc < a.OC) a.part[((int64_t)blockIdx.z * a.OC + oc) * a.OL + ol] = acc[ti][tj][e];
+    conv1d_store<BIAS, RES, H32, MT>(a, acc, ol0, oc0, wr0, wc0, c16, kq);
+}
+
+__global__ __launch_bounds__(256) void k_conv1d_pack(ConvPackKey k, float * __restrict__ img, int nchunk, int64_t n) {
+    const int64_t e = (int64_t)blockIdx.x * 256 + threadIdx.x;
+    if (e >= n) return;
+    const int per = k.oct * k.rp;
+    const int slice = (int)(e / per), w = (int)(e - (int64_t)slice * per);
+    const int ct = slice / nchunk, chunk = slice - ct * nchunk;
+    const int row = w / k.rp, r = w - row * k.rp;
+    const int icl = r / k.K, tap = r - icl * k.K;
+    const int64_t oc = (int64_t)ct * k.oct + row, ic = (int64_t)chunk * k.icc + icl;
+    float v = 0.f;
+    if (icl < k.icc && ic < k.IC && oc < k.OC) {
+        const int64_t o = oc * k.woc + (int64_t)tap * k.wk + ic * k.wic;
+        v = k.w16 ? __half2float(((const __half *)k.w)[o]) : __half2float(__float2half_rn(((const float *)k.w)[o]));
+    }
+    img[conv1d_pack_index(nchunk, k.oct, k.rp, ct, chunk, row, r)] = v;
+}
+
+void launch_conv1d_pack(hipStream_t stream, const ConvPackKey & k, float * img) {
+    const int64_t n = (int64_t)k.floats();
+    hipLaunchKernelGGL(k_conv1d_pack, dim3((unsigned)((n + 255) / 256)), dim3(256), 0, stream, k, img, k.nchunk(), n);
+    TTS_HIP_CHECK(hipGetLastError());
+}
+
+template <bool BIAS, bool RES, int MT>
+__global__ __launch_bounds__(256) __attribute__((amdgpu_waves_per_eu(MT == 2 ? 1 : 2))) void k_conv1d_f64p(Conv1dArgs a) {
+    constexpr int OCT = 32 * MT, WQ = 2 * MT;
+    extern __shared__ float sm[];
+    __shared__ int xoff[CONV1D_MAX_R];
+    const int tid = threadIdx.x, lane = tid & 63, wave = tid >> 6;
+    const int c16 = lane & 15, kq = lane >> 4;
+    const int64_t ol0 = (int64_t)blockIdx.x * 64;
+    const int oc0 = blockIdx.y * OCT;
+    const int K = a.K, s = a.s, icc = a.icc, xw = a.xw;
+    const int R = icc * K, Rp = (R + 31) & ~31;
+    f32x4_t * ws4 = (f32x4_t *)sm;
+    float * xs = sm + OCT * Rp;
+    const int zslot = icc * xw;
+    for (int r = tid; r < Rp; r += 256) {
+        const int ic = r / K, k = r - ic * K;
+        xoff[r] = r < R ? ic * xw + k * a.d : zslot;
+    }
+    if (tid == 0) xs[zslot] = 0.f;
+    __syncthreads();
+    const int wr0 = (wave >> 1) * 16 * MT, wc0 = (wave & 1) * 32;
+    const bool wave_live = oc0 + wr0 < a.OC && ol0 + wc0 < a.OL;
+    f64x4_t acc[MT][2] = {};
+    const int64_t base = ol0 * s - a.p;
+    const int EX = icc * xw;
+    const int nx = (EX + 255) >> 8;
+    const int nw = Rp == 64 ? WQ : WQ / 2;
+    const int G = Rp >> 4;
+    const uint32_t OOB = 0x80000000u;
+    const auto xr = __builtin_amdgcn_make_buffer_rsrc(a.x.data, 0, a.x_bytes, 0x00020000);
+    uint32_t xrel[CONV1D_XN];
+#pragma unroll
+    for (int u = 0; u < CONV1D_XN; ++u) {
+        const int e = tid + 256 * u;
+        const int ic = e / xw, q = e - ic * xw;
+        const int64_t pos = base + q;
+        const bool ok = e < EX && pos >= 0 && pos < a.L;
+        xrel[u] = ok ? (uint32_t)(pos * a.x.nb[0] + (int64_t)ic * a.x.nb[1]) : OOB;
+    }
+    const int nchunk = (int)((a.IC + icc - 1) / icc);
+    const int slice4 = OCT * Rp / 4;
+    const f32x4_t * wp = (const f32x4_t *)a.wimg + (int64_t)blockIdx.y * nchunk * slice4 + tid;
+    float xv[CONV1D_XN];
+    f32x4_t wv[WQ];
+    auto fetch = [&](int ic0) {
+        const int nic = min(icc, (int)(a.IC - ic0));
+        const uint32_t xc = (uint32_t)((int64_t)ic0 * a.x.nb[1]);
+#pragma unroll
+        for (int u = 0; u < CONV1D_XN; ++u)
+            if (u < nx) {
+                const uint32_t off = (xrel[u] == OOB || tid + 256 * u >= nic * xw) ? OOB : xrel[u] + xc;
+                xv[u] = __builtin_bit_cast(float, __builtin_amdgcn_raw_buffer_load_b32(xr, off, 0, 0));
+            }
+#pragma unroll
+        for (int u = 0; u < WQ; ++u)
+            if (u < nw) wv[u] = wp[256 * u];
+        wp += slice4;
+    };
+    fetch(0);
+    for (int ic0 = 0; ic0 < a.IC; ic0 += icc) {
+#pragma unroll
+        for (int u = 0; u < CONV1D_XN; ++u)
+            if (u < nx && tid + 256 * u < EX) xs[tid + 256 * u] = __half2float(__float2half_rn(xv[u]));
+#pragma unroll
+        for (int u = 0; u < WQ; ++u)
+            if (u < nw) ws4[tid + 256 * u] = wv[u];
+        __syncthreads();
+        if (ic0 + icc < a.IC) fetch(ic0 + icc);
+        if (!wave_live) {
+            __syncthreads();
+            continue;
+        }
+        for (int r0 = 0; r0 < Rp; r0 += 32) {
+            int xo[8];
+#pragma unroll
+            for (int u = 0; u < 8; ++u) xo[u] = xoff[r0 + 4 * u + kq];
+            float af[8][MT], bf[8][2];
+#pragma unroll
+            for (int h = 0; h < 2; ++h)
+#pragma unroll
+                for (int t = 0; t < MT; ++t) {
+                    const f32x4_t v = ws4[(((wr0 >> 4) + t) * G + (r0 >> 4) + h) * 64 + lane];
+#pragma unroll
+                    for (int j = 0; j < 4; ++j) af[4 * h + j][t] = v[j];
                 }
-        }
-        return;
-    }
-    float bv[MT][4], rv[2][MT][4];
-#pragma unroll
-    for (int ti = 0; ti < MT; ++ti)
-#pragma unroll
-        for (int e = 0; e < 4; ++e) {
-            const int oc = min(oc0 + wr0 + 16 * ti + (H32 ? 4 * kq + e : kq + 4 * e), (int)a.OC - 1);
-            bv[ti][e] = BIAS ? a.bias[(int64_t)oc * a.bcs] : 0.f;
-#pragma unroll
-            for (int tj = 0; tj < 2; ++tj) {
-                const int64_t ol = min(ol0 + wc0 + 16 * tj + c16, a.OL - 1);
-                rv[tj][ti][e] = RES ? a.res[ol + (int64_t)oc * a.rcs] : 0.f;
-            }
-        }
-#pragma unroll
-    for (int tj = 0; tj < 2; ++tj) {
-        const int64_t ol = ol0 + wc0 + 16 * tj + c16;
-        if (ol >= a.OL) continue;
-#pragma unroll
-        for (int ti = 0; ti < MT; ++ti)
-#pragma unroll
-            for (int e = 0; e < 4; ++e) {
-                const int oc = oc0 + wr0 + 16 * ti + (H32 ? 4 * kq + e : kq + 4 * e);
-                if (oc >= a.OC) continue;
-                a.y[ol + (int64_t)oc * a.ycs] = conv1d_epilogue<BIAS, RES>(acc[ti][tj][e], bv[ti][e], rv[tj][ti][e]);
-            }
-    }
+#pragma unroll
+            for (int u = 0; u < 8; ++u) {
+                const bool z = xo[u] == zslot;
+#pragma unroll
+                for (int t = 0; t < 2; ++t) bf[u][t] = xs[z ? zslot : xo[u] + (wc0 + 16 * t + c16) * s];
+            }
+#pragma unroll
+            for (int u = 0; u < 8; ++u)
+#pragma unroll
+                for (int ti = 0; ti < MT; ++ti)
+#pragma unroll
+                    for (int tj = 0; tj < 2; ++tj)
+                        acc[ti][tj] = __builtin_amdgcn_mfma_f64_16x16x4f64((double)af[u][ti], (double)bf[u][tj], acc[ti][tj], 0, 0, 0);
+        }
+        __syncthreads();
+    }
+    conv1d_store<BIAS, RES, false, MT>(a, acc, ol0, oc0, wr0, wc0, c16, kq);
 }
 
 constexpr int CONV1DV_NP = 4;
@@ -520,7 +653,27 @@
     return bytes <= 64 * 1024;
 }
 
+bool conv1d_pack_key(const tts_hip_backend * be, const Conv1dArgs & a0, ConvPackKey * k) {
+    if (!be->conv_pack || !a0.w_stable || be->conv_acc_mode == 2) return false;
+    Conv1dArgs a = a0;
+    a.xw = 63 * a.s + (a.K - 1) * a.d + 1;
+    a.icc = conv1d_icc(a.IC, a.K, a.xw);
+    if (a.icc < 1) return false;
+    const int64_t tiles = ((a.OL + 63) / 64) * ((a.OC + 63) / 64), nchunk = (a.IC + a.icc - 1) / a.icc;
+    if (split_count(be, tiles, nchunk, 2, a.OL * a.OC) > 1) return false;
+    int vxw = 0, vicc = 0;
+    size_t vlds = 0;
+    if (be->conv_vfma && (be->conv_vfma == 2 || a.OC < 8) && conv1d_vfma_geometry(a, &vxw, &vicc, &vlds)) return false;
+    k->be = be, k->w = a.w, k->w16 = a.w16, k->K = a.K;
+    k->oct = be->conv_tile96 && a.OC % 96 == 0 ? 96 : 64;
+    k->icc = a.icc, k->rp = (a.icc * a.K + 31) & ~31;
+    k->IC = a.IC, k->OC = a.OC, k->wk = a.wk, k->wic = a.wic, k->woc = a.woc;
+    return true;
+}
+
 void launch_conv1d_fused(tts_hip_backend * be, Conv1dArgs a) {
+    ConvPackKey pk;
+    a.wimg = conv1d_pack_key(be, a, &pk) ? conv_pack_get(be, pk) : nullptr;
     a.xw = 63 * a.s + (a.K - 1) * a.d + 1;
     a.icc = conv1d_icc(a.IC, a.K, a.xw);
     a.rs = ((a.icc * a.K + 31) & ~31) + 1;
@@ -559,6 +712,20 @@
         a.xw = vxw, a.icc = vicc;
         const dim3 vgrid((unsigned)((a.OL + 256 * CONV1DV_NP - 1) / (256 * CONV1DV_NP)), (unsigned)a.OC);
         TTS_CONV1D_SEL(k_conv1d_f64v, vgrid, vlds)
+    } else if (a.wimg) {
+        const size_t plds = ((size_t)pk.oct * pk.rp + (size_t)a.icc * a.xw + 1) * 4;
+        grid.y = (unsigned)pk.ntile();
+        const int psel = (pk.oct == 96 ? 4 : 0) | (a.bias ? 2 : 0) | (a.res ? 1 : 0);
+        switch (psel) {
+            case 0: hipLaunchKernelGGL((k_conv1d_f64p<false, false, 2>), grid, dim3(256), plds, be->stream, a); break;
+            case 1: hipLaunchKernelGGL((k_conv1d_f64p<false, true, 2>), grid, dim3(256), plds, be->stream, a); break;
+            case 2: hipLaunchKernelGGL((k_conv1d_f64p<true, false, 2>), grid, dim3(256), plds, be->stream, a); break;
+            case 3: hipLaunchKernelGGL((k_conv1d_f64p<true, true, 2>), grid, dim3(256), plds, be->stream, a); break;
+            case 4: hipLaunchKernelGGL((k_conv1d_f64p<false, false, 3>), grid, dim3(256), plds, be->stream, a); break;
+            case 5: hipLaunchKernelGGL((k_conv1d_f64p<false, true, 3>), grid, dim3(256), plds, be->stream, a); break;
+            case 6: hipLaunchKernelGGL((k_conv1d_f64p<true, false, 3>), grid, dim3(256), plds, be->stream, a); break;
+            default: hipLaunchKernelGGL((k_conv1d_f64p<true, true, 3>), grid, dim3(256), plds, be->stream, a); break;
+        }
     } else if (nz == 1 && be->conv_acc_mode != 2 && be->conv_tile96 && a.OC % 96 == 0) {
         grid.y = (unsigned)(a.OC / 96);
         lds += 32 * (size_t)a.rs * 4;
diff --git a/tts.cpp_amd/ttship/__init__.py b/tts.cpp_amd/ttship/__init__.py
--- a/tts.cpp_amd/ttship/__init__.py
+++ b/tts.cpp_amd/ttship/__init__.py
@@ -19,7 +19,7 @@
 FUSE_ALL = sum(FUSE.values())
 UNARY = {"ABS": 0, "NEG": 1, "TANH": 2, "RELU": 3, "SIGMOID": 4, "GELU": 5, "SILU": 6, "EXP": 7}
 
-OPT = {"FUSION": 0, "PROFILE_GEMV": 1, "GRAPHS": 2, "CONV_F32ACC": 3, "CONVT_LDS": 4, "ATTN_SPLIT": 5, "KV_PREFETCH": 6, "KV_PREFETCH_BLOCKS": 7, "Q4K_TILE_BYTES": 8, "GEMV_DEBUG": 10, "GEMV_UNIQUE": 11, "CONV_SPLIT": 12, "GEMV_KS": 13, "ATTN_FUSED": 14, "ATTN_PV16": 15, "Q4K_DUAL_BYTES": 16, "GEMV_RSPLIT": 17, "GEMM_Q8": 18, "BGEMM_F32": 19, "CU_PARTITION": 20, "GEMV_PREQUANT": 21, "GEMV_KRELAY": 22, "ATTN_KS": 23, "ATTN_PV8": 24, "GEMV_NW_MIN": 25, "GEMV_KRELAY_LOOP": 26, "GEMV_Q80_PRO": 27, "GEMV_Q80_SLAB": 28, "GEMV_Q80_RW": 29, "GEMM_Q8_STAGED": 30, "GEMV_KR_INKERNEL": 31, "GEMV_F32_WIDE": 32, "ATTN_PV_MP": 33, "GEMM_KR_NW": 34, "GEMM_KR_INKERNEL": 35, "GEMM_KR_CT2": 36, "COALESCE": 37, "GEMM_KR_XCD": 38, "GEMM_KR_CP": 39, "GEMM_KR_WALK": 40, "GEMM_PF": 41, "GEMM_PF_NW": 42, "ATTN_ONE": 43, "GEMV_KR_TAIL": 44, "GEMV_Q50_SLAB": 45, "GEMV_Q50_RW": 46, "GEMM_Q5": 47, "GEMM_Q5_STAGED": 48, "GEMV_Q40_SLAB": 49, "GEMV_Q40_RW": 50, "GEMM_Q4_0": 51, "GEMM_Q4_0_STAGED": 52, "CONV_VFMA": 53, "CONV_TILE96": 54}
+OPT = {"FUSION": 0, "PROFILE_GEMV": 1, "GRAPHS": 2, "CONV_F32ACC": 3, "CONVT_LDS": 4, "ATTN_SPLIT": 5, "KV_PREFETCH": 6, "KV_PREFETCH_BLOCKS": 7, "Q4K_TILE_BYTES": 8, "GEMV_DEBUG": 10, "GEMV_UNIQUE": 11, "CONV_SPLIT": 12, "GEMV_KS": 13, "ATTN_FUSED": 14, "ATTN_PV16": 15, "Q4K_DUAL_BYTES": 16, "GEMV_RSPLIT": 17, "GEMM_Q8": 18, "BGEMM_F32": 19, "CU_PARTITION": 20, "GEMV_PREQUANT": 21, "GEMV_KRELAY": 22, "ATTN_KS": 23, "ATTN_PV8": 24, "GEMV_NW_MIN": 25, "GEMV_KRELAY_LOOP": 26, "GEMV_Q80_PRO": 27, "GEMV_Q80_SLAB": 28, "GEMV_Q80_RW": 29, "GEMM_Q8_STAGED": 30, "GEMV_KR_INKERNEL": 31, "GEMV_F32_WIDE": 32, "ATTN_PV_MP": 33, "GEMM_KR_NW": 34, "GEMM_KR_INKERNEL": 35, "GEMM_KR_CT2": 36, "COALESCE": 37, "GEMM_KR_XCD": 38, "GEMM_KR_CP": 39, "GEMM_KR_WALK": 40, "GEMM_PF": 41, "GEMM_PF_NW": 42, "ATTN_ONE": 43, "GEMV_KR_TAIL": 44, "GEMV_Q50_SLAB": 45, "GEMV_Q50_RW": 46, "GEMM_Q5": 47, "GEMM_Q5_STAGED": 48, "GEMV_Q40_SLAB": 49, "GEMV_Q40_RW": 50, "GEMM_Q4_0": 51, "GEMM_Q4_0_STAGED": 52, "CONV_VFMA": 53, "CONV_TILE96": 54, "CONV_PACK": 55}
 ATTN_SPLIT_DEFAULT = 128
 ATTN_ONE_DEFAULT = 1
 GEMV_KR_TAIL_DEFAULT = 1
@@ -634,10 +634,10 @@
         return ms.value, n.value, b.value
 
     def counters(self):
-        out = (ctypes.c_int64 * 8)()
-        n = self.L.tts_hip_counters(self.ptr, out, 8)
+        out = (ctypes.c_int64 * 10)()
+        n = self.L.tts_hip_counters(self.ptr, out, 10)
         keys = ("graph_updates", "graph_instantiations", "lstm_chains", "lstm_steps", "plan_wait_ns",
-                "cap_plan_ns", "cap_launch_ns", "cap_update_ns")
+                "cap_plan_ns", "cap_launch_ns", "cap_update_ns", "conv_pack_images", "conv_pack_bytes")
         return {keys[i]: int(out[i]) for i in range(n)}
 
     def close(self):
```

After: 122.5 (median of 6 runs). +6.6%, better.
